# Edenzzzz/Stable-Diffusion-for-book-cover-generation

Measured on NVIDIA B200. Metric: unet_denoise_it_per_s, higher is better.
Workload: dtype bf16

## Files before the change

include/b200sd.h:

```cpp
#ifndef B200SD_H_
#define B200SD_H_

#include <stddef.h>
#include <stdint.h>

#ifdef __cplusplus
extern "C" {
#endif

#define B200SD_OK 0
#define B200SD_ERR_INVALID 1
#define B200SD_ERR_CUDA 2
#define B200SD_ERR_UNSUPPORTED 3

#define B200SD_F32 0
#define B200SD_BF16 1

typedef void* b200sd_stream_t;

const char* b200sd_last_error(void);
int b200sd_version(void);
int64_t b200sd_launch_count(void);

void b200sd_debug_set(int key, int value);
int b200sd_timer_reserve(int n);
int b200sd_timer_record(int i, b200sd_stream_t stream);
int b200sd_timer_elapsed_ms(int i, int j, float* ms);


int b200sd_cfg_ddim_step(const void* eps_u, const void* eps_c, const void* x, void* out, void* eps_out,
                         int64_t n, float guidance, float sa_t, float sb_t, float sa_p, float sb_p,
                         int eps_dtype, int x_dtype, b200sd_stream_t stream);

int b200sd_sampler_advance(const float* timesteps, int n_steps, int* cursor, float* in_t, int n_t, b200sd_stream_t stream);
int b200sd_cfg_ddim_step_table(const void* eps_u, const void* eps_c, const void* x, void* out, void* eps_out,
                               int64_t n, float guidance, const float* coef_table, const int* cursor,
                               int eps_dtype, int x_dtype, b200sd_stream_t stream);

int b200sd_cfg_plms_step_table(const float* eps_u, const float* eps_c, float* x, float* saved, float* ring, int64_t n,
                               float guidance, const float* table, const int* cursor, b200sd_stream_t stream);

int b200sd_cfg_plms_step(const void* eps_u, const void* eps_c, const void* x, void* out, void* eps_out,
                         const void* hist0, const void* hist1, const void* hist2, const void* hist3,
                         int nhist, const float* w_host5, int64_t n, float guidance, float cx, float ce,
                         int eps_dtype, int x_dtype, b200sd_stream_t stream);

int b200sd_add_noise(const void* x0, const void* noise, const int64_t* timesteps, const float* sa_table,
                     const float* sb_table, void* out, int batch, int64_t per_sample, int num_train_timesteps,
                     int dtype, b200sd_stream_t stream);

int b200sd_mse_workspace_floats(void);
int b200sd_mse_loss_fwd(const void* pred, const void* target, float* loss_out, float* workspace, int64_t n,
                        int pred_dtype, int target_dtype, b200sd_stream_t stream);
int b200sd_mse_loss_bwd(const void* pred, const void* target, const float* grad_loss, void* grad_pred, int64_t n,
                        int pred_dtype, int target_dtype, b200sd_stream_t stream);


int b200sd_timestep_embedding(const float* timesteps, float* out, int batch, int dim, b200sd_stream_t stream);

int b200sd_small_linear(const float* in, const void* w_bf16, const float* bias, float* out, int batch, int N, int K,
                        int silu_in, int silu_out, b200sd_stream_t stream);

#define B200SD_EPI_LINEAR 0
#define B200SD_EPI_GEGLU 1

typedef struct b200sd_gemm_args {
    const void* a0;
    const void* a1;
    const void* w;
    const float* bias;
    const float* rowbias;
    const void* residual;
    void* out;
    int M, N, K;
    int C0, C1;
    int lda0, lda1;
    int ldc, ldr;
    int ldrb;
    int conv_taps;
    int batch, H, W;
    int rows_per_image;
    int epilogue;
    int out_dtype;
    int residual_dtype;
    int block_n;
    int split_k;
    void* workspace;
    size_t workspace_bytes;
    int pair;
    float* gn_part;
} b200sd_gemm_args;

size_t b200sd_gemm_workspace_bytes(void);
int b200sd_geglu_tile(int N);
int b200sd_gemm(const b200sd_gemm_args* args, b200sd_stream_t stream);
int b200sd_gemm_gn_layout(const b200sd_gemm_args* args, int hw, int* parts_per_image, int* total_parts);

typedef struct b200sd_dgrad_args {
    const void* dy;
    const void* w;
    const void* residual;
    void* out;
    int M, Cout, Cin;
    int conv_taps;
    int batch, H, W;
    int ldy, ldc, ldr;
    int out_dtype, residual_dtype;
    int block_n;
    int pair;
} b200sd_dgrad_args;
int b200sd_gemm_dgrad(const b200sd_dgrad_args* args, b200sd_stream_t stream);

typedef struct b200sd_wgrad_args {
    const void* dy;
    const void* x;
    float* dw;
    int rows, Cout, Cin;
    int conv_taps;
    int batch, H, W;
    int ldy, ldx, lddw;
    int block_n, split_k;
} b200sd_wgrad_args;
int b200sd_gemm_wgrad(const b200sd_wgrad_args* args, b200sd_stream_t stream);

int b200sd_conv_in(const float* x_nchw, const float* w, const float* bias, void* out_nhwc, int batch, int Cin,
                   int Cout, int H, int W, int out_dtype, b200sd_stream_t stream);
int b200sd_conv_out(const void* x_nhwc, const float* w, const float* bias, float* out_nchw, int batch, int Cin,
                    int Cout, int H, int W, b200sd_stream_t stream);
int b200sd_nhwc_bias_to_nchw(const float* x, const float* bias, float* out_nchw, int batch, int C, int hw, int ld,
                             b200sd_stream_t stream);

int b200sd_groupnorm_silu(const void* x0, const void* x1, int C0, int C1, const float* gamma, const float* beta,
                          void* out, void* raw_out, float* stats_ws, int batch, int hw, int groups, float eps,
                          int silu, int in_dtype, b200sd_stream_t stream);

int b200sd_groupnorm_silu_stats(const void* x0, const void* x1, int C0, int C1, const float* gamma, const float* beta,
                                void* out, void* raw_out, float* stats_ws, float* stats_out, int batch, int hw, int groups,
                                float eps, int silu, int in_dtype, b200sd_stream_t stream);

int b200sd_groupnorm_silu_parts(const void* x0, const void* x1, int C0, int C1, const float* part0, int ppi0, int ld0,
                                const float* part1, int ppi1, int ld1, const float* gamma, const float* beta, void* out,
                                void* raw_out, float* stats_out, int batch, int hw, int groups, float eps, int silu,
                                int in_dtype, b200sd_stream_t stream);

int b200sd_groupnorm_workspace_floats(int batch);
int b200sd_layernorm(const void* x, const float* gamma, const float* beta, void* out, int rows, int C, float eps,
                     int in_dtype, b200sd_stream_t stream);

size_t b200sd_attention_workspace_bytes(int batch, int heads, int Skv, int d);
int b200sd_attention(const void* q, const void* k, const void* v, void* out, int batch, int heads, int Sq, int Skv,
                     int d, int ldq, int ldk, int ldv, int ldo, float scale, void* workspace, size_t workspace_bytes,
                     b200sd_stream_t stream);

int b200sd_attention_lse(const void* q, const void* k, const void* v, void* out, float* lse, int batch, int heads, int Sq,
                         int Skv, int d, int ldq, int ldk, int ldv, int ldo, float scale, void* workspace,
                         size_t workspace_bytes, b200sd_stream_t stream);

size_t b200sd_attention_bwd_workspace_bytes(int batch, int heads, int Sq);
int b200sd_attention_bwd(const void* q, const void* k, const void* v, const void* out, const void* dout,
                         const float* lse, void* dq, void* dk, void* dv, int batch, int heads, int Sq, int Skv, int d,
                         int ldq, int ldk, int ldv, int ldo, int lddo, int lddq, int lddk, int lddv, float scale,
                         void* workspace, size_t workspace_bytes, b200sd_stream_t stream);


int b200sd_clip_embed(const int64_t* ids, const float* tok, const float* pos, float* out, int batch, int S, int C, int vocab,
                      b200sd_stream_t stream);
int b200sd_clip_embed_bwd(const int64_t* ids, const float* dx, float* dtok, float* dpos, int batch, int S, int C, int vocab,
                          b200sd_stream_t stream);
int b200sd_quick_gelu_fwd(const void* u, void* out, int64_t n, b200sd_stream_t stream);
int b200sd_quick_gelu_bwd(const void* u, const void* dg, void* du, int64_t n, b200sd_stream_t stream);
int b200sd_layernorm_f32out(const float* x, const float* gamma, const float* beta, float* out, int rows, int C, float eps,
                            b200sd_stream_t stream);
int b200sd_causal_attention(const void* qkv, void* out, int batch, int heads, int S, int d, int ld, int ldo, int q_off,
                            int k_off, int v_off, float scale, b200sd_stream_t stream);
int b200sd_causal_attention_bwd(const void* qkv, const void* dout, void* dqkv, int batch, int heads, int S, int d, int ld,
                                int lddo, int ldd, int q_off, int k_off, int v_off, float scale, b200sd_stream_t stream);


int b200sd_im2col_s2_pad(const void* x, void* out, int batch, int H, int W, int C, int in_dtype, int pad,
                         b200sd_stream_t stream);
int b200sd_softmax_rows(const float* x, void* out_bf16, int rows, int L, int ldx, int ldo, float scale, b200sd_stream_t stream);
int b200sd_conv1x1_small(const float* x_nchw, const float* w, const float* bias, float* out_nchw, int batch, int Cin, int Cout,
                         int hw, b200sd_stream_t stream);
int b200sd_gaussian_sample(const float* moments, const float* noise, float* out, int batch, int C, int hw, float out_scale,
                           b200sd_stream_t stream);


int b200sd_grad_prep(const void* in, int in_dtype, void* out_bf16, float* colsum, int rows, int N, int ld,
                     int rows_per_image, int ldcs, b200sd_stream_t stream);

int b200sd_groupnorm_bwd_workspace_floats(int batch);
int b200sd_groupnorm_silu_bwd(const void* x0, const void* x1, int C0, int C1, int in_dtype, const float* gamma,
                              const float* beta, const void* dy, const float* add_src, void* out0, void* out1,
                              int out_dtype, int accumulate0, int accumulate1, float* dgamma, float* dbeta,
                              const float* mean_rstd, float* workspace, int batch, int hw, int groups, float eps, int silu,
                              b200sd_stream_t stream);

int b200sd_layernorm_bwd(const void* x, int in_dtype, const float* gamma, const void* dy, float* dres, float* dgamma,
                         float* dbeta, int rows, int C, float eps, b200sd_stream_t stream);

int b200sd_geglu_fwd(const void* u, void* out, int64_t rows, int C_half, b200sd_stream_t stream);
int b200sd_geglu_bwd(const void* u, const void* dff, void* du, int64_t rows, int C_half, b200sd_stream_t stream);

int b200sd_upsample2x_bwd(const void* dy, float* dx, int batch, int H, int W, int C, int accumulate, b200sd_stream_t stream);
int b200sd_col2im_s2(const void* dcol, float* dx, int batch, int H, int W, int C, int accumulate, b200sd_stream_t stream);

int b200sd_conv_out_bwd(const float* dout_nchw, const void* x_nhwc, const float* w, void* dx_nhwc, float* dw,
                        float* dbias, int batch, int Cin, int Cout, int H, int W, b200sd_stream_t stream);
int b200sd_conv_in_wgrad(const void* dy_nhwc, int dy_dtype, const float* x_nchw, float* dw, int batch, int Cin, int Cout,
                         int H, int W, b200sd_stream_t stream);

int b200sd_cast_act(const float* in, void* out_bf16, int64_t n, int silu, b200sd_stream_t stream);
int b200sd_silu_bwd_mul(const float* pre, float* grad, int64_t n, b200sd_stream_t stream);

int b200sd_split_hi_lo(const float* x, void* hi_bf16, void* lo_bf16, int64_t n, b200sd_stream_t stream);
int b200sd_groupnorm_silu_split(const void* x0, const void* x1, int C0, int C1, const float* gamma, const float* beta,
                                void* out, void* out_lo, void* raw_out, void* raw_lo, float* stats_ws, float* stats_out,
                                int batch, int hw, int groups, float eps, int silu, int in_dtype, b200sd_stream_t stream);
int b200sd_layernorm_split(const void* x, const float* gamma, const float* beta, void* out, void* out_lo, int rows, int C,
                           float eps, int in_dtype, b200sd_stream_t stream);
int b200sd_geglu_f32(const float* u, void* hi_bf16, void* lo_bf16, int64_t rows, int C_half, b200sd_stream_t stream);
int b200sd_attention_f32(const float* q, const float* k, const float* v, float* out, int batch, int heads, int Sq, int Skv,
                         int d, int ldq, int ldk, int ldv, int ldo, float scale, b200sd_stream_t stream);
int b200sd_small_linear_f32(const float* in, const float* w, const float* bias, float* out, int batch, int N, int K,
                            int silu_in, int silu_out, b200sd_stream_t stream);

int b200sd_cast_flat(const float* in, void* out_bf16, int64_t n, b200sd_stream_t stream);
int b200sd_adamw_step(float* param, float* grad, float* exp_avg, float* exp_avg_sq, void* weights_bf16, int64_t n,
                      float lr, float beta1, float beta2, float eps, float weight_decay, int step, float grad_scale,
                      int zero_grad, b200sd_stream_t stream);

int b200sd_adamw8bit_step(float* param, float* grad, uint8_t* state1, uint8_t* state2, float* absmax1, float* absmax2,
                          const float* qmap1, const float* qmap2, const int32_t* chunk_mode, float* small_exp_avg,
                          float* small_exp_avg_sq, void* weights_bf16, int64_t n, float lr, float beta1, float beta2, float eps,
                          float weight_decay, int step, float grad_scale, int zero_grad, b200sd_stream_t stream);

int b200sd_upsample2x(const void* x, void* out, int batch, int H, int W, int C, int in_dtype, b200sd_stream_t stream);
int b200sd_im2col_s2(const void* x, void* out, int batch, int H, int W, int C, int in_dtype, b200sd_stream_t stream);

#ifdef __cplusplus
}
#endif
#endif
```

stable-diffusion-for-book-cover-generation_b200/_lib.py:

```python
from __future__ import annotations

import ctypes as C
import os

_HERE = os.path.dirname(os.path.abspath(__file__))
LIB_PATH = os.path.join(_HERE, "libb200sd.so")

_lib = None


class B200SDError(RuntimeError):
    pass


class GemmArgs(C.Structure):
    _fields_ = [
        ("a0", C.c_void_p), ("a1", C.c_void_p), ("w", C.c_void_p), ("bias", C.c_void_p), ("rowbias", C.c_void_p),
        ("residual", C.c_void_p), ("out", C.c_void_p),
        ("M", C.c_int), ("N", C.c_int), ("K", C.c_int), ("C0", C.c_int), ("C1", C.c_int),
        ("lda0", C.c_int), ("lda1", C.c_int), ("ldc", C.c_int), ("ldr", C.c_int), ("ldrb", C.c_int), ("conv_taps", C.c_int),
        ("batch", C.c_int), ("H", C.c_int), ("W", C.c_int), ("rows_per_image", C.c_int), ("epilogue", C.c_int),
        ("out_dtype", C.c_int), ("residual_dtype", C.c_int), ("block_n", C.c_int), ("split_k", C.c_int),
        ("workspace", C.c_void_p), ("workspace_bytes", C.c_size_t), ("pair", C.c_int), ("gn_part", C.c_void_p),
    ]


class DgradArgs(C.Structure):
    _fields_ = [
        ("dy", C.c_void_p), ("w", C.c_void_p), ("residual", C.c_void_p), ("out", C.c_void_p),
        ("M", C.c_int), ("Cout", C.c_int), ("Cin", C.c_int), ("conv_taps", C.c_int),
        ("batch", C.c_int), ("H", C.c_int), ("W", C.c_int), ("ldy", C.c_int), ("ldc", C.c_int), ("ldr", C.c_int),
        ("out_dtype", C.c_int), ("residual_dtype", C.c_int), ("block_n", C.c_int), ("pair", C.c_int),
    ]


class WgradArgs(C.Structure):
    _fields_ = [
        ("dy", C.c_void_p), ("x", C.c_void_p), ("dw", C.c_void_p),
        ("rows", C.c_int), ("Cout", C.c_int), ("Cin", C.c_int), ("conv_taps", C.c_int),
        ("batch", C.c_int), ("H", C.c_int), ("W", C.c_int), ("ldy", C.c_int), ("ldx", C.c_int), ("lddw", C.c_int),
        ("block_n", C.c_int), ("split_k", C.c_int),
    ]


_vp, _i, _i64, _f, _sz = C.c_void_p, C.c_int, C.c_int64, C.c_float, C.c_size_t

SIGNATURES = {
    "b200sd_last_error": (C.c_char_p, []),
    "b200sd_version": (_i, []),
    "b200sd_launch_count": (_i64, []),
    "b200sd_debug_set": (None, [_i, _i]),
    "b200sd_timer_reserve": (_i, [_i]),
    "b200sd_timer_record": (_i, [_i, _vp]),
    "b200sd_timer_elapsed_ms": (_i, [_i, _i, C.POINTER(C.c_float)]),
    "b200sd_cfg_ddim_step": (_i, [_vp, _vp, _vp, _vp, _vp, _i64, _f, _f, _f, _f, _f, _i, _i, _vp]),
    "b200sd_clip_embed": (_i, [_vp, _vp, _vp, _vp, _i, _i, _i, _i, _vp]),
    "b200sd_clip_embed_bwd": (_i, [_vp, _vp, _vp, _vp, _i, _i, _i, _i, _vp]),
    "b200sd_quick_gelu_fwd": (_i, [_vp, _vp, _i64, _vp]),
    "b200sd_quick_gelu_bwd": (_i, [_vp, _vp, _vp, _i64, _vp]),
    "b200sd_layernorm_f32out": (_i, [_vp, _vp, _vp, _vp, _i, _i, _f, _vp]),
    "b200sd_causal_attention": (_i, [_vp, _vp, _i, _i, _i, _i, _i, _i, _i, _i, _i, _f, _vp]),
    "b200sd_causal_attention_bwd": (_i, [_vp, _vp, _vp, _i, _i, _i, _i, _i, _i, _i, _i, _i, _i, _f, _vp]),
    "b200sd_im2col_s2_pad": (_i, [_vp, _vp, _i, _i, _i, _i, _i, _i, _vp]),
    "b200sd_softmax_rows": (_i, [_vp, _vp, _i, _i, _i, _i, _f, _vp]),
    "b200sd_conv1x1_small": (_i, [_vp, _vp, _vp, _vp, _i, _i, _i, _i, _vp]),
    "b200sd_gaussian_sample": (_i, [_vp, _vp, _vp, _i, _i, _i, _f, _vp]),
    "b200sd_sampler_advance": (_i, [_vp, _i, _vp, _vp, _i, _vp]),
    "b200sd_cfg_plms_step_table": (_i, [_vp, _vp, _vp, _vp, _vp, _i64, _f, _vp, _vp, _vp]),
    "b200sd_cfg_ddim_step_table": (_i, [_vp, _vp, _vp, _vp, _vp, _i64, _f, _vp, _vp, _i, _i, _vp]),
    "b200sd_cfg_plms_step": (_i, [_vp, _vp, _vp, _vp, _vp, _vp, _vp, _vp, _vp, _i, C.POINTER(C.c_float), _i64, _f, _f,
                                  _f, _i, _i, _vp]),
    "b200sd_add_noise": (_i, [_vp, _vp, _vp, _vp, _vp, _vp, _i, _i64, _i, _i, _vp]),
    "b200sd_mse_workspace_floats": (_i, []),
    "b200sd_mse_loss_fwd": (_i, [_vp, _vp, _vp, _vp, _i64, _i, _i, _vp]),
    "b200sd_mse_loss_bwd": (_i, [_vp, _vp, _vp, _vp, _i64, _i, _i, _vp]),
    "b200sd_timestep_embedding": (_i, [_vp, _vp, _i, _i, _vp]),
    "b200sd_small_linear": (_i, [_vp, _vp, _vp, _vp, _i, _i, _i, _i, _i, _vp]),
    "b200sd_gemm_workspace_bytes": (_sz, []),
    "b200sd_geglu_tile": (_i, [_i]),
    "b200sd_gemm": (_i, [C.POINTER(GemmArgs), _vp]),
    "b200sd_gemm_gn_layout": (_i, [C.POINTER(GemmArgs), _i, C.POINTER(C.c_int), C.POINTER(C.c_int)]),
    "b200sd_groupnorm_silu_parts": (_i, [_vp, _vp, _i, _i, _vp, _i, _i, _vp, _i, _i, _vp, _vp, _vp, _vp, _vp, _i, _i, _i, _f, _i,
                                         _i, _vp]),
    "b200sd_gemm_dgrad": (_i, [C.POINTER(DgradArgs), _vp]),
    "b200sd_gemm_wgrad": (_i, [C.POINTER(WgradArgs), _vp]),
    "b200sd_conv_in": (_i, [_vp, _vp, _vp, _vp, _i, _i, _i, _i, _i, _i, _vp]),
    "b200sd_conv_out": (_i, [_vp, _vp, _vp, _vp, _i, _i, _i, _i, _i, _vp]),
    "b200sd_nhwc_bias_to_nchw": (_i, [_vp, _vp, _vp, _i, _i, _i, _i, _vp]),
    "b200sd_groupnorm_silu": (_i, [_vp, _vp, _i, _i, _vp, _vp, _vp, _vp, _vp, _i, _i, _i, _f, _i, _i, _vp]),
    "b200sd_groupnorm_silu_stats": (_i, [_vp, _vp, _i, _i, _vp, _vp, _vp, _vp, _vp, _vp, _i, _i, _i, _f, _i, _i, _vp]),
    "b200sd_groupnorm_workspace_floats": (_i, [_i]),
    "b200sd_layernorm": (_i, [_vp, _vp, _vp, _vp, _i, _i, _f, _i, _vp]),
    "b200sd_attention_workspace_bytes": (_sz, [_i, _i, _i, _i]),
    "b200sd_attention": (_i, [_vp, _vp, _vp, _vp, _i, _i, _i, _i, _i, _i, _i, _i, _i, _f, _vp, _sz, _vp]),
    "b200sd_attention_lse": (_i, [_vp, _vp, _vp, _vp, _vp, _i, _i, _i, _i, _i, _i, _i, _i, _i, _f, _vp, _sz, _vp]),
    "b200sd_attention_bwd_workspace_bytes": (_sz, [_i, _i, _i]),
    "b200sd_attention_bwd": (_i, [_vp] * 9 + [_i] * 13 + [_f, _vp, _sz, _vp]),
    "b200sd_grad_prep": (_i, [_vp, _i, _vp, _vp, _i, _i, _i, _i, _i, _vp]),
    "b200sd_groupnorm_bwd_workspace_floats": (_i, [_i]),
    "b200sd_groupnorm_silu_bwd": (_i, [_vp, _vp, _i, _i, _i, _vp, _vp, _vp, _vp, _vp, _vp, _i, _i, _i, _vp, _vp, _vp, _vp, _i,
                                       _i, _i, _f, _i, _vp]),
    "b200sd_layernorm_bwd": (_i, [_vp, _i, _vp, _vp, _vp, _vp, _vp, _i, _i, _f, _vp]),
    "b200sd_geglu_fwd": (_i, [_vp, _vp, _i64, _i, _vp]),
    "b200sd_geglu_bwd": (_i, [_vp, _vp, _vp, _i64, _i, _vp]),
    "b200sd_upsample2x_bwd": (_i, [_vp, _vp, _i, _i, _i, _i, _i, _vp]),
    "b200sd_col2im_s2": (_i, [_vp, _vp, _i, _i, _i, _i, _i, _vp]),
    "b200sd_conv_out_bwd": (_i, [_vp, _vp, _vp, _vp, _vp, _vp, _i, _i, _i, _i, _i, _vp]),
    "b200sd_conv_in_wgrad": (_i, [_vp, _i, _vp, _vp, _i, _i, _i, _i, _i, _vp]),
    "b200sd_cast_act": (_i, [_vp, _vp, _i64, _i, _vp]),
    "b200sd_silu_bwd_mul": (_i, [_vp, _vp, _i64, _vp]),
    "b200sd_split_hi_lo": (_i, [_vp, _vp, _vp, _i64, _vp]),
    "b200sd_groupnorm_silu_split": (_i, [_vp, _vp, _i, _i, _vp, _vp, _vp, _vp, _vp, _vp, _vp, _vp, _i, _i, _i, _f, _i, _i, _vp]),
    "b200sd_layernorm_split": (_i, [_vp, _vp, _vp, _vp, _vp, _i, _i, _f, _i, _vp]),
    "b200sd_geglu_f32": (_i, [_vp, _vp, _vp, _i64, _i, _vp]),
    "b200sd_attention_f32": (_i, [_vp, _vp, _vp, _vp, _i, _i, _i, _i, _i, _i, _i, _i, _i, _f, _vp]),
    "b200sd_small_linear_f32": (_i, [_vp, _vp, _vp, _vp, _i, _i, _i, _i, _i, _vp]),
    "b200sd_cast_flat": (_i, [_vp, _vp, _i64, _vp]),
    "b200sd_adamw_step": (_i, [_vp, _vp, _vp, _vp, _vp, _i64, _f, _f, _f, _f, _f, _i, _f, _i, _vp]),
    "b200sd_adamw8bit_step": (_i, [_vp] * 12 + [_i64, _f, _f, _f, _f, _f, _i, _f, _i, _vp]),
    "b200sd_upsample2x": (_i, [_vp, _vp, _i, _i, _i, _i, _i, _vp]),
    "b200sd_im2col_s2": (_i, [_vp, _vp, _i, _i, _i, _i, _i, _vp]),
}


def lib() -> C.CDLL:
    global _lib
    if _lib is None:
        if not os.path.exists(LIB_PATH):
            raise B200SDError(
                f"{LIB_PATH} is missing: build it with `python -c 'import __graft_entry__ as g; g.build()'` "
                "(b200sd has no CPU / eager fallback)")
        L = C.CDLL(LIB_PATH)
        for name, (res, args) in SIGNATURES.items():
            fn = getattr(L, name)
            fn.restype = res
            fn.argtypes = args
        _lib = L
    return _lib


def check(rc: int, what: str = "") -> None:
    if rc != 0:
        msg = lib().b200sd_last_error().decode("utf-8", "replace")
        raise B200SDError(f"{what or 'b200sd call'} failed (code {rc}): {msg}")
```

stable-diffusion-for-book-cover-generation_b200/csrc/api.cu:

```cuda
#include <atomic>
#include <cstdarg>
#include <cstdio>
#include <mutex>

#include "common.cuh"

static thread_local char g_err[512] = "";
std::atomic<long long> g_b200sd_launches{0};

void b200sd_set_error(const char* fmt, ...) {
    va_list ap;
    va_start(ap, fmt);
    vsnprintf(g_err, sizeof(g_err), fmt, ap);
    va_end(ap);
}

extern "C" const char* b200sd_last_error(void) { return g_err; }

#include <map>
#include <utility>
cudaError_t b200sd_opt_in_smem_impl(const void* kernel, int bytes, bool max_carveout) {
    static std::mutex mu;
    static std::map<std::pair<const void*, int>, int> configured;
    int dev = 0;
    cudaError_t e = cudaGetDevice(&dev);
    if (e != cudaSuccess) return e;
    std::lock_guard<std::mutex> lock(mu);
    auto key = std::make_pair(kernel, dev);
    auto it = configured.find(key);
    if (it != configured.end() && it->second >= bytes) return cudaSuccess;
    e = cudaFuncSetAttribute(kernel, cudaFuncAttributeMaxDynamicSharedMemorySize, bytes);
    if (e != cudaSuccess) return e;
    if (max_carveout) {
        e = cudaFuncSetAttribute(kernel, cudaFuncAttributePreferredSharedMemoryCarveout, 100);
        if (e != cudaSuccess) return e;
    }
    configured[key] = bytes;
    return cudaSuccess;
}
extern "C" int b200sd_version(void) { return 101; }
extern "C" int64_t b200sd_launch_count(void) { return g_b200sd_launches.load(); }

#include <vector>
static std::vector<cudaEvent_t> g_timers;
extern "C" int b200sd_timer_reserve(int n) {
    B200SD_REQUIRE(n >= 0 && n <= (1 << 20), "timer_reserve: bad count %d", n);
    while ((int)g_timers.size() < n) {
        cudaEvent_t e;
        B200SD_CUDA(cudaEventCreate(&e));
        g_timers.push_back(e);
    }
    return B200SD_OK;
}
extern "C" int b200sd_timer_record(int i, b200sd_stream_t stream) {
    B200SD_REQUIRE(i >= 0 && i < (int)g_timers.size(), "timer_record: index %d not reserved", i);
    cudaStream_t s = static_cast<cudaStream_t>(stream);
    cudaStreamCaptureStatus st = cudaStreamCaptureStatusNone;
    B200SD_CUDA(cudaStreamIsCapturing(s, &st));
    B200SD_CUDA(cudaEventRecordWithFlags(g_timers[i], s, st == cudaStreamCaptureStatusActive ? cudaEventRecordExternal : cudaEventRecordDefault));
    return B200SD_OK;
}
extern "C" int b200sd_timer_elapsed_ms(int i, int j, float* ms) {
    B200SD_REQUIRE(ms && i >= 0 && j >= 0 && i < (int)g_timers.size() && j < (int)g_timers.size(), "timer_elapsed: bad index");
    B200SD_CUDA(cudaEventElapsedTime(ms, g_timers[i], g_timers[j]));
    return B200SD_OK;
}

int b200sd_num_sms() {
    static int sms = 0;
    if (sms == 0) {
        int dev = 0;
        if (cudaGetDevice(&dev) != cudaSuccess) return 148;
        if (cudaDeviceGetAttribute(&sms, cudaDevAttrMultiProcessorCount, dev) != cudaSuccess || sms <= 0) sms = 148;
    }
    return sms;
}

typedef CUresult (*encode_tiled_fn)(CUtensorMap*, CUtensorMapDataType, cuuint32_t, void*, const cuuint64_t*,
                                    const cuuint64_t*, const cuuint32_t*, const cuuint32_t*, CUtensorMapInterleave,
                                    CUtensorMapSwizzle, CUtensorMapL2promotion, CUtensorMapFloatOOBfill);

static encode_tiled_fn get_encode_fn() {
    static encode_tiled_fn fn = nullptr;
    static std::once_flag once;
    std::call_once(once, [] {
        void* p = nullptr;
        cudaDriverEntryPointQueryResult q;
        if (cudaGetDriverEntryPoint("cuTensorMapEncodeTiled", &p, cudaEnableDefault, &q) == cudaSuccess &&
            q == cudaDriverEntryPointSuccess)
            fn = reinterpret_cast<encode_tiled_fn>(p);
    });
    return fn;
}

int b200sd_make_tmap(CUtensorMap* out, const void* base, int rank, const uint64_t* dims,
                     const uint64_t* strides_bytes, const uint32_t* box, CUtensorMapSwizzle swizzle,
                     CUtensorMapDataType dtype) {
    encode_tiled_fn fn = get_encode_fn();
    B200SD_REQUIRE(fn != nullptr, "cuTensorMapEncodeTiled driver entry point unavailable");
    cuuint64_t gdim[5];
    cuuint64_t gstr[5];
    cuuint32_t bdim[5];
    cuuint32_t estr[5];
    for (int i = 0; i < rank; ++i) {
        gdim[i] = dims[i];
        bdim[i] = box[i];
        estr[i] = 1;
        if (i > 0) gstr[i - 1] = strides_bytes[i];
    }
    CUresult r = fn(out, dtype, (cuuint32_t)rank, const_cast<void*>(base), gdim, gstr, bdim, estr,
                    CU_TENSOR_MAP_INTERLEAVE_NONE, swizzle, CU_TENSOR_MAP_L2_PROMOTION_L2_256B,
                    CU_TENSOR_MAP_FLOAT_OOB_FILL_NONE);
    B200SD_REQUIRE(r == CUDA_SUCCESS,
                   "cuTensorMapEncodeTiled failed (%d): rank %d dims [%llu %llu %llu %llu] box [%u %u %u %u] base %p",
                   (int)r, rank, (unsigned long long)dims[0], (unsigned long long)(rank > 1 ? dims[1] : 0),
                   (unsigned long long)(rank > 2 ? dims[2] : 0), (unsigned long long)(rank > 3 ? dims[3] : 0), box[0],
                   rank > 1 ? box[1] : 0, rank > 2 ? box[2] : 0, rank > 3 ? box[3] : 0, base);
    return B200SD_OK;
}
```

stable-diffusion-for-book-cover-generation_b200/csrc/common.cuh:

```cuda
#pragma once

#include <cuda.h>
#include <cuda_bf16.h>
#include <cuda_runtime.h>
#include <stdint.h>
#include <stdio.h>

#include "../../include/b200sd.h"

typedef __nv_bfloat16 bf16;

void b200sd_set_error(const char* fmt, ...);

#define B200SD_REQUIRE(cond, ...)                       \
    do {                                                \
        if (!(cond)) {                                  \
            b200sd_set_error(__VA_ARGS__);              \
            return B200SD_ERR_INVALID;                  \
        }                                               \
    } while (0)

#define B200SD_CUDA(call)                                                                   \
    do {                                                                                    \
        cudaError_t e__ = (call);                                                           \
        if (e__ != cudaSuccess) {                                                           \
            b200sd_set_error("%s:%d CUDA error %s", __FILE__, __LINE__, cudaGetErrorString(e__)); \
            return B200SD_ERR_CUDA;                                                         \
        }                                                                                   \
    } while (0)

#define B200SD_LAUNCH_CHECK() B200SD_CUDA(cudaGetLastError())

static inline int ceil_div(int a, int b) { return (a + b - 1) / b; }

int b200sd_num_sms();

int b200sd_make_tmap(CUtensorMap* out, const void* base, int rank, const uint64_t* dims,
                     const uint64_t* strides_bytes, const uint32_t* box, CUtensorMapSwizzle swizzle,
                     CUtensorMapDataType dtype = CU_TENSOR_MAP_DATA_TYPE_BFLOAT16);

#ifdef __CUDACC__
cudaError_t b200sd_opt_in_smem_impl(const void* kernel, int bytes, bool max_carveout);
template <typename K>
static inline cudaError_t b200sd_opt_in_smem(K kernel, int bytes, bool max_carveout = false) {
    return b200sd_opt_in_smem_impl(reinterpret_cast<const void*>(kernel), bytes, max_carveout);
}

namespace ptx {

__device__ __forceinline__ uint32_t smem_u32(const void* p) {
    return static_cast<uint32_t>(__cvta_generic_to_shared(p));
}

__device__ __forceinline__ bool elect_one() {
    uint32_t pred;
    asm volatile(
        "{\n\t.reg .pred p;\n\t"
        "elect.sync _|p, 0xffffffff;\n\t"
        "selp.u32 %0, 1, 0, p;\n\t}\n"
        : "=r"(pred));
    return pred != 0;
}

__device__ __forceinline__ void mbar_init(uint64_t* bar, uint32_t count) {
    asm volatile("mbarrier.init.shared::cta.b64 [%0], %1;" ::"r"(smem_u32(bar)), "r"(count));
}
__device__ __forceinline__ void fence_barrier_init() {
    asm volatile("fence.mbarrier_init.release.cluster;" ::: "memory");
}
__device__ __forceinline__ void fence_proxy_async() {
    asm volatile("fence.proxy.async.shared::cta;" ::: "memory");
}
__device__ __forceinline__ void fence_proxy_async_global() {
    asm volatile("fence.proxy.async.global;" ::: "memory");
}
__device__ __forceinline__ void mbar_expect_tx(uint64_t* bar, uint32_t bytes) {
    asm volatile("mbarrier.arrive.expect_tx.shared::cta.b64 _, [%0], %1;" ::"r"(smem_u32(bar)), "r"(bytes)
                 : "memory");
}
__device__ __forceinline__ void mbar_arrive(uint64_t* bar) {
    asm volatile("mbarrier.arrive.shared::cta.b64 _, [%0];" ::"r"(smem_u32(bar)) : "memory");
}
__device__ __forceinline__ bool mbar_try_wait(uint64_t* bar, uint32_t parity) {
    uint32_t ok;
    asm volatile(
        "{\n\t.reg .pred p;\n\t"
        "mbarrier.try_wait.parity.shared::cta.b64 p, [%1], %2;\n\t"
        "selp.u32 %0, 1, 0, p;\n\t}\n"
        : "=r"(ok)
        : "r"(smem_u32(bar)), "r"(parity)
        : "memory");
    return ok != 0;
}
__device__ __forceinline__ void mbar_wait(uint64_t* bar, uint32_t parity) {
    if (mbar_try_wait(bar, parity)) return;
    long long t0 = clock64();
    while (!mbar_try_wait(bar, parity)) {
        if (clock64() - t0 > 4000000000LL) {
            printf("b200sd: mbarrier wait timed out (block %d,%d thread %d)\n", blockIdx.x, blockIdx.y,
                   threadIdx.x);
            __trap();
        }
    }
}

__device__ __forceinline__ void prefetch_tmap(const CUtensorMap* m) {
    asm volatile("prefetch.tensormap [%0];" ::"l"(reinterpret_cast<uint64_t>(m)) : "memory");
}
__device__ __forceinline__ void tma_load_2d(void* dst, const CUtensorMap* m, uint64_t* bar, int c0, int c1) {
    asm volatile(
        "cp.async.bulk.tensor.2d.shared::cluster.global.mbarrier::complete_tx::bytes [%0], [%1, {%3, %4}], [%2];"
        ::"r"(smem_u32(dst)), "l"(reinterpret_cast<uint64_t>(m)), "r"(smem_u32(bar)), "r"(c0), "r"(c1)
        : "memory");
}
__device__ __forceinline__ void tma_load_3d(void* dst, const CUtensorMap* m, uint64_t* bar, int c0, int c1, int c2) {
    asm volatile(
        "cp.async.bulk.tensor.3d.shared::cluster.global.mbarrier::complete_tx::bytes [%0], [%1, {%3, %4, %5}], [%2];"
        ::"r"(smem_u32(dst)), "l"(reinterpret_cast<uint64_t>(m)), "r"(smem_u32(bar)), "r"(c0), "r"(c1), "r"(c2)
        : "memory");
}
__device__ __forceinline__ void tma_load_4d(void* dst, const CUtensorMap* m, uint64_t* bar, int c0, int c1, int c2,
                                            int c3) {
    asm volatile(
        "cp.async.bulk.tensor.4d.shared::cluster.global.mbarrier::complete_tx::bytes [%0], [%1, {%3, %4, %5, %6}], "
        "[%2];" ::"r"(smem_u32(dst)),
        "l"(reinterpret_cast<uint64_t>(m)), "r"(smem_u32(bar)), "r"(c0), "r"(c1), "r"(c2), "r"(c3)
        : "memory");
}

__device__ __forceinline__ void tma_store_2d(const CUtensorMap* m, const void* src, int c0, int c1) {
    asm volatile("cp.async.bulk.tensor.2d.global.shared::cta.bulk_group [%0, {%2, %3}], [%1];" ::"l"(reinterpret_cast<uint64_t>(m)),
                 "r"(smem_u32(src)), "r"(c0), "r"(c1)
                 : "memory");
}
__device__ __forceinline__ void tma_store_commit() { asm volatile("cp.async.bulk.commit_group;" ::: "memory"); }
template <int N>
__device__ __forceinline__ void tma_store_wait_read() { asm volatile("cp.async.bulk.wait_group.read %0;" ::"n"(N) : "memory"); }
template <int N>
__device__ __forceinline__ void tma_store_wait() { asm volatile("cp.async.bulk.wait_group %0;" ::"n"(N) : "memory"); }

__device__ __forceinline__ uint32_t mapa_u32(uint32_t local_smem_addr, uint32_t cta_rank) {
    uint32_t r;
    asm volatile("mapa.shared::cluster.u32 %0, %1, %2;" : "=r"(r) : "r"(local_smem_addr), "r"(cta_rank));
    return r;
}
__device__ __forceinline__ void tma_load_2d_cg2(void* dst, const CUtensorMap* m, uint32_t bar_cluster_addr, int c0, int c1) {
    asm volatile(
        "cp.async.bulk.tensor.2d.cta_group::2.shared::cluster.global.mbarrier::complete_tx::bytes [%0], [%1, {%3, %4}], [%2];"
        ::"r"(smem_u32(dst)), "l"(reinterpret_cast<uint64_t>(m)), "r"(bar_cluster_addr), "r"(c0), "r"(c1)
        : "memory");
}
__device__ __forceinline__ void tma_load_3d_cg2(void* dst, const CUtensorMap* m, uint32_t bar_cluster_addr, int c0, int c1, int c2) {
    asm volatile(
        "cp.async.bulk.tensor.3d.cta_group::2.shared::cluster.global.mbarrier::complete_tx::bytes [%0], [%1, {%3, %4, %5}], [%2];"
        ::"r"(smem_u32(dst)), "l"(reinterpret_cast<uint64_t>(m)), "r"(bar_cluster_addr), "r"(c0), "r"(c1), "r"(c2)
        : "memory");
}
__device__ __forceinline__ void tma_load_4d_cg2(void* dst, const CUtensorMap* m, uint32_t bar_cluster_addr, int c0, int c1, int c2,
                                                int c3) {
    asm volatile(
        "cp.async.bulk.tensor.4d.cta_group::2.shared::cluster.global.mbarrier::complete_tx::bytes [%0], [%1, {%3, %4, %5, %6}], "
        "[%2];" ::"r"(smem_u32(dst)),
        "l"(reinterpret_cast<uint64_t>(m)), "r"(bar_cluster_addr), "r"(c0), "r"(c1), "r"(c2), "r"(c3)
        : "memory");
}
__device__ __forceinline__ void tmem_alloc_cg2(uint32_t* dst_smem, uint32_t ncols) {
    asm volatile("tcgen05.alloc.cta_group::2.sync.aligned.shared::cta.b32 [%0], %1;" ::"r"(smem_u32(dst_smem)), "r"(ncols) : "memory");
}
__device__ __forceinline__ void tmem_relinquish_cg2() {
    asm volatile("tcgen05.relinquish_alloc_permit.cta_group::2.sync.aligned;" ::: "memory");
}
__device__ __forceinline__ void tmem_dealloc_cg2(uint32_t taddr, uint32_t ncols) {
    asm volatile("tcgen05.dealloc.cta_group::2.sync.aligned.b32 %0, %1;" ::"r"(taddr), "r"(ncols) : "memory");
}
__device__ __forceinline__ void umma_bf16_ss_cg2(uint32_t tmem_d, uint64_t desc_a, uint64_t desc_b, uint32_t idesc,
                                                 uint32_t accumulate) {
    asm volatile(
        "{\n\t.reg .pred p;\n\t"
        "setp.ne.b32 p, %4, 0;\n\t"
        "tcgen05.mma.cta_group::2.kind::f16 [%0], %1, %2, %3, p;\n\t}\n" ::"r"(tmem_d),
        "l"(desc_a), "l"(desc_b), "r"(idesc), "r"(accumulate)
        : "memory");
}
__device__ __forceinline__ void umma_commit_cg2(uint64_t* bar, uint16_t cta_mask) {
    asm volatile("tcgen05.commit.cta_group::2.mbarrier::arrive::one.shared::cluster.multicast::cluster.b64 [%0], %1;" ::"r"(smem_u32(bar)),
                 "h"(cta_mask)
                 : "memory");
}
// ... 156 lines not shown
```

stable-diffusion-for-book-cover-generation_b200/csrc/gemm_tcgen05.cu:

```cuda
#include <atomic>
#include <cstring>
#include <mutex>
#include <cstdio>

#include "common.cuh"

extern std::atomic<long long> g_b200sd_launches;

static int g_persist = -1;
extern "C" void b200sd_debug_set(int key, int value) { if (key == 0) g_persist = value; }

namespace {

constexpr int BLOCK_M = 128;
constexpr size_t kWsPartialBytes = (size_t)160 * 128 * 256 * sizeof(float);
constexpr size_t kWsCounterBytes = 4096;
constexpr int BLOCK_K = 64;
constexpr int UMMA_K = 16;
constexpr int kNumThreads = 192;
constexpr int kMaxStages = 8;
constexpr int kABytes = BLOCK_M * BLOCK_K * 2;


struct KParams {
    CUtensorMap tmA0, tmA1, tmB;
    const float* bias;
    const float* rowbias;
    const void* residual;
    void* out;
    int M, N;
    int num_k_blocks;
    int kb_per_split;
    int split_k;
    int block_n;
    int stages;
    int conv;
    int cblocks0;
    int cblocks;
    int tile_w, tile_h, tile_n;
    int tiles_y;
    int tiles_x;
    int rows_valid;
    int a_bytes;
    int ldc, ldr, ldrb;
    int rows_per_image;
    int epilogue;
    int out_f32;
    int res_f32;
    uint32_t tmem_cols;
    int a_mn;
    int b_mode;
    int conv_sign;
    int n_valid;
    int tiles_per_tap;
    int atomic_out;
    int pair;
    int persist;
    int psplit;
    float* gn_part;
};

__device__ __forceinline__ void cluster_sync_all() {
    asm volatile("barrier.cluster.arrive.release.aligned;\n\tbarrier.cluster.wait.acquire.aligned;" ::: "memory");
}
__device__ __forceinline__ uint32_t cluster_ctarank() {
    uint32_t r;
    asm volatile("mov.u32 %0, %%cluster_ctarank;" : "=r"(r));
    return r;
}
__device__ __forceinline__ float4 ld_dsmem_v4(uint32_t local_smem_addr, uint32_t cta_rank) {
    uint32_t raddr;
    asm volatile("mapa.shared::cluster.u32 %0, %1, %2;" : "=r"(raddr) : "r"(local_smem_addr), "r"(cta_rank));
    float4 v;
    asm volatile("ld.shared::cluster.v4.f32 {%0, %1, %2, %3}, [%4];" : "=f"(v.x), "=f"(v.y), "=f"(v.z), "=f"(v.w) : "r"(raddr) : "memory");
    return v;
}

__device__ __forceinline__ void red_add_v4(float* dst, float a, float b, float c, float d) {
    asm volatile("red.global.add.v4.f32 [%0], {%1, %2, %3, %4};" ::"l"(dst), "f"(a), "f"(b), "f"(c), "f"(d) : "memory");
}

struct EpiCtx {
    uint32_t stage_u32;
    int pitch_f, row_end, R, cb, half, m0, col_out, img0, n0cb;
    const float* s_rb;
    bool multi_img, rb_smem;
};
__device__ __forceinline__ void lds8(uint32_t addr, float (&v)[8]) {
    asm volatile("ld.shared.v4.f32 {%0, %1, %2, %3}, [%4];" : "=f"(v[0]), "=f"(v[1]), "=f"(v[2]), "=f"(v[3]) : "r"(addr));
    asm volatile("ld.shared.v4.f32 {%0, %1, %2, %3}, [%4];" : "=f"(v[4]), "=f"(v[5]), "=f"(v[6]), "=f"(v[7]) : "r"(addr + 16));
}
template <int OUT, int RES, bool SPLIT, bool GEGLU, bool STATS = false>
__device__ __forceinline__ void epilogue_rows(const KParams& p, const EpiCtx& e, int row0, const float (&b)[8], const float (&bg)[8],
                                              float* cs = nullptr, float* cq = nullptr) {
    constexpr int U = 4;
    for (int row = row0; row < e.row_end; row += e.R * U) {
        float v[U][8], r[U][8];
#pragma unroll
        for (int u = 0; u < U; ++u) {
            const int rl = min(row + u * e.R, e.row_end - 1);
            const uint32_t addr = e.stage_u32 + (uint32_t)(rl * e.pitch_f + e.cb) * 4u;
            if constexpr (SPLIT) {
#pragma unroll
                for (int i = 0; i < 8; ++i) v[u][i] = 0.f;
                for (int sp = 0; sp < p.split_k; ++sp) {
                    const float4 a0 = ld_dsmem_v4(addr, sp), a1 = ld_dsmem_v4(addr + 16, sp);
                    v[u][0] += a0.x; v[u][1] += a0.y; v[u][2] += a0.z; v[u][3] += a0.w;
                    v[u][4] += a1.x; v[u][5] += a1.y; v[u][6] += a1.z; v[u][7] += a1.w;
                }
            } else {
                lds8(addr, v[u]);
            }
            if constexpr (GEGLU) lds8(addr + (uint32_t)e.half * 4u, r[u]);
            else if constexpr (RES == 2) ld8<B200SD_F32>(p.residual, (size_t)(e.m0 + rl) * p.ldr + e.col_out, r[u]);
            else if constexpr (RES == 1) ld8<B200SD_BF16>(p.residual, (size_t)(e.m0 + rl) * p.ldr + e.col_out, r[u]);
        }
#pragma unroll
        for (int u = 0; u < U; ++u) {
            const int rl = row + u * e.R;
            if (rl >= e.row_end) break;
            const int grow = e.m0 + rl;
            float o[8];
            if constexpr (GEGLU) {
#pragma unroll
                for (int i = 0; i < 8; ++i) o[i] = (v[u][i] + b[i]) * gelu_erf_f(r[u][i] + bg[i]);
                st8<B200SD_BF16>(p.out, (size_t)grow * p.ldc + e.col_out, o);
            } else {
#pragma unroll
                for (int i = 0; i < 8; ++i) o[i] = v[u][i] + b[i];
                if constexpr (RES != 0) {
#pragma unroll
                    for (int i = 0; i < 8; ++i) o[i] += r[u][i];
                }
                if (e.multi_img) {
                    const int img = grow / p.rows_per_image;
                    if (e.rb_smem) {
                        const float* rb = e.s_rb + (img == e.img0 ? 0 : 256) + e.cb;
#pragma unroll
                        for (int i = 0; i < 8; ++i) o[i] += rb[i];
                    } else {
                        float t[8];
                        ld8<B200SD_F32>(p.rowbias, (size_t)img * p.ldrb + e.n0cb, t);
#pragma unroll
                        for (int i = 0; i < 8; ++i) o[i] += t[i];
                    }
                }
                if constexpr (STATS) {
#pragma unroll
                    for (int i = 0; i < 8; ++i) { cs[i] += o[i]; cq[i] = fmaf(o[i], o[i], cq[i]); }
                }
                if constexpr (OUT == 2) {
                    float* dst = static_cast<float*>(p.out) + (size_t)grow * p.ldc + e.col_out;
                    red_add_v4(dst, o[0], o[1], o[2], o[3]);
                    red_add_v4(dst + 4, o[4], o[5], o[6], o[7]);
                } else if constexpr (OUT == 1) st8<B200SD_F32>(p.out, (size_t)grow * p.ldc + e.col_out, o);
                else st8<B200SD_BF16>(p.out, (size_t)grow * p.ldc + e.col_out, o);
            }
        }
    }
}

template <bool PAIR, int OP>
__global__ void __launch_bounds__(kNumThreads, 1) gemm_tcgen05_kernel(const __grid_constant__ KParams p) {
    constexpr bool a_mn = OP >= 2;
    constexpr int b_mode = OP;
    extern __shared__ uint8_t smem_raw[];
    uint8_t* smem = reinterpret_cast<uint8_t*>((reinterpret_cast<uintptr_t>(smem_raw) + 1023) & ~uintptr_t(1023));
    constexpr bool pair = PAIR;
    const uint32_t crank = pair ? cluster_ctarank() : 0;
    const int b_bytes = (p.block_n * BLOCK_K * 2) >> (pair ? 1 : 0);
    uint8_t* smem_a = smem;
    uint8_t* smem_b = smem + (size_t)p.stages * kABytes;
    uint64_t* bars = reinterpret_cast<uint64_t*>(smem_b + (size_t)p.stages * b_bytes);
    uint64_t* full_bar = bars;
    uint64_t* empty_bar = bars + kMaxStages;
    uint64_t* tmem_full_bar = bars + 2 * kMaxStages;
    uint32_t* tmem_slot = reinterpret_cast<uint32_t*>(bars + 2 * kMaxStages + 1);

    const int warp = threadIdx.x >> 5;
    const int lane = threadIdx.x & 31;
    const int m_tile = blockIdx.x;
    const int n_tile = blockIdx.y;
    const int split = blockIdx.z;
    const int kb_begin = split * p.kb_per_split;
    const int kb_end = min(kb_begin + p.kb_per_split, p.num_k_blocks);
    const int w_tap = b_mode == 3 ? n_tile / p.tiles_per_tap : 0;
    const int n0 = (b_mode == 3 ? n_tile - w_tap * p.tiles_per_tap : n_tile) * p.block_n;
    const int col_base = w_tap * p.n_valid + n0;
    const int col_valid = min(p.block_n, p.n_valid - n0);
    const int m0 = m_tile * p.rows_valid;

    if (warp == 0 && lane == 0) {
        ptx::prefetch_tmap(&p.tmA0);
        ptx::prefetch_tmap(&p.tmB);
        if (p.cblocks0 != p.cblocks) ptx::prefetch_tmap(&p.tmA1);
        for (int s = 0; s < p.stages; ++s) {
            ptx::mbar_init(&full_bar[s], 1);
            ptx::mbar_init(&empty_bar[s], 1);
        }
        ptx::mbar_init(tmem_full_bar, 1);
        ptx::fence_barrier_init();
    }
    if (warp == 1) {
        if constexpr (pair) { ptx::tmem_alloc_cg2(tmem_slot, p.tmem_cols); ptx::tmem_relinquish_cg2(); }
        else { ptx::tmem_alloc(tmem_slot, p.tmem_cols); ptx::tmem_relinquish(); }
    }
    ptx::tc_fence_before();
    __syncthreads();
    if constexpr (pair) cluster_sync_all();
    ptx::tc_fence_after();
    const uint32_t tmem_base = *tmem_slot;

    const int epi_tid = threadIdx.x - 64;
    const int pitch_f = p.block_n + 4;
    float* stage = reinterpret_cast<float*>(smem);
    float* s_bias = reinterpret_cast<float*>(bars + 32);
    float* s_rb = s_bias + 256;
    int img0 = 0, img1 = 0;
    bool rb_smem = false;
    if (p.rowbias && m0 < p.M) {
        img0 = m0 / p.rows_per_image;
        img1 = (min(m0 + p.rows_valid, p.M) - 1) / p.rows_per_image;
        rb_smem = (img1 - img0) <= 1;
    }

    if (warp == 0) {
        if (ptx::elect_one()) {
            int stage = 0;
            uint32_t phase = 0;
            int img = 0, y0 = 0, x0 = 0;
            if (p.conv) {
                if (p.tile_n > 1) { img = m_tile * p.tile_n; y0 = 0; }
                else {
                    int mt = m_tile;
                    if (p.tiles_x > 1) { x0 = (mt % p.tiles_x) * p.tile_w; mt /= p.tiles_x; }
                    img = mt / p.tiles_y; y0 = (mt % p.tiles_y) * p.tile_h;
                }
            }
            const int nbox_live = (b_mode != 0 && !pair) ? (col_valid + 63) >> 6 : (p.block_n >> 6);
            const int nboxb = nbox_live >> (pair ? 1 : 0);
            const int nb0 = n0 + (pair ? (int)crank * (p.block_n >> 1) : 0);
            const uint32_t stage_tx = (b_mode != 0 && !pair) ? (uint32_t)(p.a_bytes + nbox_live * 8192)
                                                             : ((uint32_t)(p.a_bytes + b_bytes) << (pair ? 1 : 0));
            for (int kb = kb_begin; kb < kb_end; ++kb) {
                ptx::mbar_wait(&empty_bar[stage], phase ^ 1);
                if (!pair || crank == 0) ptx::mbar_expect_tx(&full_bar[stage], stage_tx);
                uint8_t* dst_a = smem_a + (size_t)stage * kABytes;
                uint8_t* dst_b = smem_b + (size_t)stage * b_bytes;
                uint64_t* fb = &full_bar[stage];
                const uint32_t fbc = pair ? ptx::mapa_u32(ptx::smem_u32(fb), 0) : 0;
#define LD2(dst, tm, c0, c1) do { if constexpr (pair) ptx::tma_load_2d_cg2(dst, tm, fbc, c0, c1); else ptx::tma_load_2d(dst, tm, fb, c0, c1); } while (0)
#define LD3(dst, tm, c0, c1, c2) do { if constexpr (pair) ptx::tma_load_3d_cg2(dst, tm, fbc, c0, c1, c2); else ptx::tma_load_3d(dst, tm, fb, c0, c1, c2); } while (0)
#define LD4(dst, tm, c0, c1, c2, c3) do { if constexpr (pair) ptx::tma_load_4d_cg2(dst, tm, fbc, c0, c1, c2, c3); else ptx::tma_load_4d(dst, tm, fb, c0, c1, c2, c3); } while (0)
                if (a_mn) {
                    LD2(dst_a, &p.tmA0, m0, kb * BLOCK_K);
                    LD2(dst_a + kABytes / 2, &p.tmA0, m0 + 64, kb * BLOCK_K);
                } else if (!p.conv) {
                    if (kb < p.cblocks0) LD2(dst_a, &p.tmA0, kb * BLOCK_K, m0);
                    else LD2(dst_a, &p.tmA1, (kb - p.cblocks0) * BLOCK_K, m0);
                } else {
                    const int tap = kb / p.cblocks;
                    const int cb = kb - tap * p.cblocks;
                    const int dy = (tap / 3 - 1) * p.conv_sign, dx = (tap % 3 - 1) * p.conv_sign;
                    if (cb < p.cblocks0) LD4(dst_a, &p.tmA0, cb * BLOCK_K, x0 + dx, y0 + dy, img);
                    else LD4(dst_a, &p.tmA1, (cb - p.cblocks0) * BLOCK_K, x0 + dx, y0 + dy, img);
                }
                if (b_mode == 0) {
                    LD2(dst_b, &p.tmB, kb * BLOCK_K, nb0);
                } else if (b_mode == 1) {
                    if (!p.conv) {
                        for (int j = 0; j < nboxb; ++j) LD2(dst_b + j * 8192, &p.tmB, nb0 + j * 64, kb * BLOCK_K);
                    } else {
                        const int tap = kb / p.cblocks;
                        const int cb = kb - tap * p.cblocks;
                        for (int j = 0; j < nboxb; ++j) LD3(dst_b + j * 8192, &p.tmB, nb0 + j * 64, tap, cb * BLOCK_K);
                    }
                } else if (b_mode == 2) {
                    for (int j = 0; j < nboxb; ++j) LD2(dst_b + j * 8192, &p.tmB, nb0 + j * 64, kb * BLOCK_K);
                } else {
                    int bimg, by0;
                    if (p.tile_n > 1) { bimg = kb * p.tile_n; by0 = 0; }
                    else { bimg = kb / p.tiles_y; by0 = (kb - bimg * p.tiles_y) * p.tile_h; }
                    const int dy = w_tap / 3 - 1, dx = w_tap % 3 - 1;
                    for (int j = 0; j < nboxb; ++j) LD4(dst_b + j * 8192, &p.tmB, nb0 + j * 64, dx, by0 + dy, bimg);
                }
#undef LD2
#undef LD3
#undef LD4
                if (++stage == p.stages) { stage = 0; phase ^= 1; }
            }
        }
    } else if (warp == 1) {
        if ((!pair || crank == 0) && ptx::elect_one()) {
            const uint32_t b_mn = b_mode != 0;
            const uint32_t mma_n = (b_mode != 0 && !pair) ? (uint32_t)(((col_valid + 63) >> 6) << 6) : (uint32_t)p.block_n;
            const uint32_t idesc = ptx::umma_idesc_bf16(pair ? 2 * BLOCK_M : BLOCK_M, mma_n) | ((uint32_t)a_mn << 15) | (b_mn << 16);
            const uint32_t a_step = a_mn ? (2048 >> 4) : 2, b_step = b_mn ? (2048 >> 4) : 2;
            int stage = 0;
            uint32_t phase = 0;
            for (int kb = kb_begin; kb < kb_end; ++kb) {
                ptx::mbar_wait(&full_bar[stage], phase);
                ptx::tc_fence_after();
                const uint32_t sa = ptx::smem_u32(smem_a + (size_t)stage * kABytes), sb = ptx::smem_u32(smem_b + (size_t)stage * b_bytes);
                const uint64_t da = a_mn ? ptx::umma_desc_mn_sw128(sa, 8192) : ptx::umma_desc_k_sw128(sa);
                const uint64_t db = b_mn ? ptx::umma_desc_mn_sw128(sb, 8192) : ptx::umma_desc_k_sw128(sb);
#pragma unroll
                for (int k = 0; k < BLOCK_K / UMMA_K; ++k) {
                    const uint32_t accum = (kb > kb_begin || k > 0) ? 1u : 0u;
                    if constexpr (pair) ptx::umma_bf16_ss_cg2(tmem_base, da + a_step * k, db + b_step * k, idesc, accum);
                    else ptx::umma_bf16_ss(tmem_base, da + a_step * k, db + b_step * k, idesc, accum);
                }
                if constexpr (pair) ptx::umma_commit_cg2(&empty_bar[stage], 3); else ptx::umma_commit(&empty_bar[stage]);
                if (++stage == p.stages) { stage = 0; phase ^= 1; }
            }
            if constexpr (pair) ptx::umma_commit_cg2(tmem_full_bar, 3); else ptx::umma_commit(tmem_full_bar);
        }
    } else {
        const int q = warp & 3;
        const int r_in_tile = q * 32 + lane;
        const uint32_t taddr = tmem_base + ((uint32_t)(q * 32) << 16);
        for (int c = epi_tid; c < p.block_n; c += 128) {
            s_bias[c] = (p.bias && c < col_valid) ? __ldg(p.bias + n0 + c) : 0.f;
            if (rb_smem) {
                s_rb[c] = __ldg(p.rowbias + (size_t)img0 * p.ldrb + n0 + c);
                s_rb[256 + c] = __ldg(p.rowbias + (size_t)img1 * p.ldrb + n0 + c);
            }
        }
        ptx::mbar_wait(tmem_full_bar, 0);
        ptx::tc_fence_after();
        {
            float4* my_row = reinterpret_cast<float4*>(stage + (size_t)r_in_tile * pitch_f);
            for (int c = 0; c < p.block_n; c += 32) {
                uint32_t r0[16], r1[16];
                const bool two = (c + 16 < p.block_n);
                ptx::tmem_ld_32x32b_x16(taddr + c, r0);
                if (two) ptx::tmem_ld_32x32b_x16(taddr + c + 16, r1);
                ptx::tmem_ld_wait();
#pragma unroll
                for (int i = 0; i < 4; ++i)
                    my_row[c / 4 + i] = make_float4(__uint_as_float(r0[4 * i]), __uint_as_float(r0[4 * i + 1]),
                                                    __uint_as_float(r0[4 * i + 2]), __uint_as_float(r0[4 * i + 3]));
                if (two) {
#pragma unroll
                    for (int i = 0; i < 4; ++i)
                        my_row[c / 4 + 4 + i] = make_float4(__uint_as_float(r1[4 * i]), __uint_as_float(r1[4 * i + 1]),
                                                            __uint_as_float(r1[4 * i + 2]), __uint_as_float(r1[4 * i + 3]));
                }
            }
        }
        ptx::tc_fence_before();
        ptx::named_bar_sync(1, 128);
    }

    if (p.split_k > 1) cluster_sync_all(); else __syncthreads();

    {
        const int rank = p.split_k > 1 ? (int)cluster_ctarank() : 0;
        const int rows_per_cta = BLOCK_M / p.split_k;
        const int row_begin = rank * rows_per_cta;
        int valid = min(p.rows_valid, p.M - m0) - row_begin;
        valid = max(0, min(valid, rows_per_cta));
        const bool geglu = p.epilogue == B200SD_EPI_GEGLU;
        const int half = p.block_n / 2;
        const int groups = (geglu ? half : p.block_n) / 8;
        const int R = kNumThreads / groups;
        const int tid = threadIdx.x;
        float cs[8], cq[8];
#pragma unroll
        for (int i = 0; i < 8; ++i) { cs[i] = 0.f; cq[i] = 0.f; }
        if (tid < R * groups && valid > 0) {
            const int c8 = tid % groups, r0 = tid / groups;
            const int cb = c8 * 8;
            if (geglu || cb < col_valid) {
                float b[8], bg[8];
#pragma unroll
                for (int i = 0; i < 8; ++i) { b[i] = s_bias[cb + i]; bg[i] = geglu ? s_bias[half + cb + i] : 0.f; }
                const bool multi_img = p.rowbias != nullptr && img1 != img0;
                if (p.rowbias != nullptr && !multi_img) {
#pragma unroll
                    for (int i = 0; i < 8; ++i) b[i] += s_rb[cb + i];
                }
                EpiCtx e;
                e.stage_u32 = ptx::smem_u32(stage);
                e.pitch_f = pitch_f; e.row_end = row_begin + valid; e.R = R; e.cb = cb; e.half = half; e.m0 = m0;
                e.col_out = geglu ? n_tile * half + cb : col_base + cb;
                e.s_rb = s_rb; e.img0 = img0; e.multi_img = multi_img; e.rb_smem = rb_smem; e.n0cb = n0 + cb;
                const int row0 = row_begin + r0;
                const int ok = p.atomic_out ? 2 : (p.out_f32 ? 1 : 0);
                const int rk = p.residual ? (p.res_f32 ? 2 : 1) : 0;
                if (geglu) epilogue_rows<0, 0, false, true>(p, e, row0, b, bg);
                else if (p.split_k > 1) {
                    if (ok == 1 && p.gn_part) { if (rk == 2) epilogue_rows<1, 2, true, false, true>(p, e, row0, b, bg, cs, cq); else epilogue_rows<1, 0, true, false, true>(p, e, row0, b, bg, cs, cq); }
                    else if (ok == 1) { if (rk == 2) epilogue_rows<1, 2, true, false>(p, e, row0, b, bg); else if (rk == 1) epilogue_rows<1, 1, true, false>(p, e, row0, b, bg); else epilogue_rows<1, 0, true, false>(p, e, row0, b, bg); }
                    else { if (rk == 2) epilogue_rows<0, 2, true, false>(p, e, row0, b, bg); else if (rk == 1) epilogue_rows<0, 1, true, false>(p, e, row0, b, bg); else epilogue_rows<0, 0, true, false>(p, e, row0, b, bg); }
                } else if (ok == 2) epilogue_rows<2, 0, false, false>(p, e, row0, b, bg);
                else if (ok == 1 && p.gn_part) { if (rk == 2) epilogue_rows<1, 2, false, false, true>(p, e, row0, b, bg, cs, cq); else epilogue_rows<1, 0, false, false, true>(p, e, row0, b, bg, cs, cq); }
                else if (ok == 1) { if (rk == 2) epilogue_rows<1, 2, false, false>(p, e, row0, b, bg); else if (rk == 1) epilogue_rows<1, 1, false, false>(p, e, row0, b, bg); else epilogue_rows<1, 0, false, false>(p, e, row0, b, bg); }
                else { if (rk == 2) epilogue_rows<0, 2, false, false>(p, e, row0, b, bg); else if (rk == 1) epilogue_rows<0, 1, false, false>(p, e, row0, b, bg); else epilogue_rows<0, 0, false, false>(p, e, row0, b, bg); }
            }
        }
        if (p.gn_part != nullptr) {
            if (p.split_k > 1) cluster_sync_all(); else __syncthreads();
            float* s_gn = reinterpret_cast<float*>(stage);
#pragma unroll
            for (int i = 0; i < 8; ++i) { s_gn[tid * 16 + i] = cs[i]; s_gn[tid * 16 + 8 + i] = cq[i]; }
            __syncthreads();
            float* dst = p.gn_part + (size_t)(m_tile * p.split_k + rank) * 2 * p.N;
            for (int idx = tid; idx < groups * 16; idx += kNumThreads) {
                const int c8 = idx >> 4, k = idx & 15, col = c8 * 8 + (k & 7);
                float a = 0.f;
                for (int r = 0; r < R; ++r) a += s_gn[(r * groups + c8) * 16 + k];
                if (col < col_valid) dst[(size_t)(k >> 3) * p.N + n0 + col] = a;
            }
        }
    }
    if (p.split_k > 1 && p.gn_part == nullptr) cluster_sync_all();

    ptx::tc_fence_before();
    __syncthreads();
    if constexpr (pair) cluster_sync_all();
    if (warp == 1) {
        ptx::tc_fence_after();
        if constexpr (pair) ptx::tmem_dealloc_cg2(tmem_base, p.tmem_cols); else ptx::tmem_dealloc(tmem_base, p.tmem_cols);
    }
}

constexpr int kEpiWarps = 8;
constexpr int kPersistThreads = 64 + 32 * kEpiWarps + 32;
constexpr int kMaxDepth = 3;

struct PParams {
    CUtensorMap tmA0, tmA1, tmB, tmOut, tmRes;
    const float* bias;
    const float* rowbias;
    float* gn_part;
    int M, N;
    int num_k_blocks, block_n, stages;
    int conv, cblocks0, cblocks, tile_h, tile_n, tiles_y;
    int tile_w, tiles_x;
    int n_tiles, num_tiles;
    int ldrb, rows_per_image;
    int geglu, out_f32, res_kind;
    int depth;
    int chunk_bytes;
    uint32_t tmem_cols, acc_stride;
    uint32_t off_b, off_epi, off_bias, off_stat, off_bars;
    int split, kb_per_split;
    CUtensorMap tmWs;
    float* ws;
    int* cnt;
    const void* residual;
    void* out;
    int ldc, ldr;
};

template <bool OUT_F32, int RES, bool GEGLU, bool STATS>
__device__ __forceinline__ void persist_chunk(const PParams& p, uint32_t taddr, int ch, const float* sbv, const float* sbg, uint8_t* cb,
                                              int lane, bool last_chunk, uint64_t* tempty_bar, uint64_t* rfull_bar, uint32_t rparity,
                                              float* gn_dst, int nrows) {
    uint32_t r0[16], r1[16], g0[16], g1[16];
    ptx::tmem_ld_32x32b_x16(taddr + ch * 32, r0);
    ptx::tmem_ld_32x32b_x16(taddr + ch * 32 + 16, r1);
    const int half = p.block_n >> 1;
    if constexpr (GEGLU) {
        ptx::tmem_ld_32x32b_x16(taddr + half + ch * 32, g0);
        ptx::tmem_ld_32x32b_x16(taddr + half + ch * 32 + 16, g1);
    }
    if constexpr (RES != 0) ptx::mbar_wait(rfull_bar, rparity);
    ptx::tmem_ld_wait();
    if (last_chunk) {
        ptx::tc_fence_before();
        __syncwarp();
        if (lane == 0) ptx::mbar_arrive(tempty_bar);
    }
    float v[32];
    const float4* sb4 = reinterpret_cast<const float4*>(sbv);
#pragma unroll
    for (int j = 0; j < 8; ++j) {
        const float4 b = sb4[j];
        const uint32_t* r = j < 4 ? r0 : r1;
        const int o = (j & 3) * 4;
        v[4 * j + 0] = __uint_as_float(r[o + 0]) + b.x;
        v[4 * j + 1] = __uint_as_float(r[o + 1]) + b.y;
        v[4 * j + 2] = __uint_as_float(r[o + 2]) + b.z;
        v[4 * j + 3] = __uint_as_float(r[o + 3]) + b.w;
    }
    if constexpr (GEGLU) {
        const float4* sg4 = reinterpret_cast<const float4*>(sbg);
#pragma unroll
        for (int j = 0; j < 8; ++j) {
            const float4 b = sg4[j];
            const uint32_t* r = j < 4 ? g0 : g1;
            const int o = (j & 3) * 4;
            v[4 * j + 0] *= gelu_erf_fast(__uint_as_float(r[o + 0]) + b.x);
            v[4 * j + 1] *= gelu_erf_fast(__uint_as_float(r[o + 1]) + b.y);
            v[4 * j + 2] *= gelu_erf_fast(__uint_as_float(r[o + 2]) + b.z);
            v[4 * j + 3] *= gelu_erf_fast(__uint_as_float(r[o + 3]) + b.w);
        }
    }
    uint8_t* row128 = cb + lane * 128;
    uint8_t* row64 = cb + lane * 64;
    const int x128 = lane & 7, x64 = (lane >> 1) & 3;
    if constexpr (RES == 2) {
#pragma unroll
        for (int j = 0; j < 8; ++j) {
            const float4 t = *reinterpret_cast<const float4*>(row128 + ((j ^ x128) << 4));
            v[4 * j + 0] += t.x; v[4 * j + 1] += t.y; v[4 * j + 2] += t.z; v[4 * j + 3] += t.w;
        }
    } else if constexpr (RES == 1) {
#pragma unroll
        for (int j = 0; j < 4; ++j) {
            const uint4 u = *reinterpret_cast<const uint4*>(row64 + ((j ^ x64) << 4));
            float2 f;
            f = unpack_bf16x2(u.x); v[8 * j + 0] += f.x; v[8 * j + 1] += f.y;
            f = unpack_bf16x2(u.y); v[8 * j + 2] += f.x; v[8 * j + 3] += f.y;
            f = unpack_bf16x2(u.z); v[8 * j + 4] += f.x; v[8 * j + 5] += f.y;
            f = unpack_bf16x2(u.w); v[8 * j + 6] += f.x; v[8 * j + 7] += f.y;
        }
    }
    if constexpr (RES != 0 && ((RES == 2) != OUT_F32)) __syncwarp();
    if constexpr (OUT_F32) {
#pragma unroll
        for (int j = 0; j < 8; ++j)
            *reinterpret_cast<float4*>(row128 + ((j ^ x128) << 4)) = make_float4(v[4 * j], v[4 * j + 1], v[4 * j + 2], v[4 * j + 3]);
    } else {
#pragma unroll
        for (int j = 0; j < 4; ++j) {
            uint4 u;
            u.x = pack_bf16x2(v[8 * j + 0], v[8 * j + 1]);
            u.y = pack_bf16x2(v[8 * j + 2], v[8 * j + 3]);
            u.z = pack_bf16x2(v[8 * j + 4], v[8 * j + 5]);
            u.w = pack_bf16x2(v[8 * j + 6], v[8 * j + 7]);
            *reinterpret_cast<uint4*>(row64 + ((j ^ x64) << 4)) = u;
        }
    }
    if constexpr (STATS) {
        __syncwarp();
        float s = 0.f, ss = 0.f;
        const uint8_t* colp = cb + ((lane & 3) << 2);
        const int piece = lane >> 2;
        for (int r = 0; r < nrows; ++r) {
            const float x = *reinterpret_cast<const float*>(colp + r * 128 + ((piece ^ (r & 7)) << 4));
            s += x;
            ss = fmaf(x, x, ss);
        }
        gn_dst[ch * 32 + lane] = s;
        gn_dst[256 + ch * 32 + lane] = ss;
    }
}

template <bool OUT_F32, int RES, bool GEGLU, bool STATS>
__device__ __forceinline__ void persist_epilogue(const PParams& p, uint8_t* smem, uint32_t tmem_base, int warp, int lane) {
    const int ew = warp - 2;
    const int q = warp & 3;
    const int h = ew >> 2;
    const int D = p.depth;
    const int kChunkBytes = p.chunk_bytes;
    uint8_t* my = smem + p.off_epi + (size_t)ew * D * kChunkBytes;
    float* sb = reinterpret_cast<float*>(smem + p.off_bias) + ew * 256;
    uint64_t* bars = reinterpret_cast<uint64_t*>(smem + p.off_bars);
    uint64_t* tfull = bars + 16;
    uint64_t* tempty = bars + 18;
    uint64_t* rfull = bars + 20 + ew * kMaxDepth;
    const int half = p.block_n >> 1;
    const int nch = (GEGLU ? half : p.block_n) >> 5;
    const int nl = nch > h ? (nch - h + 1) >> 1 : 0;
    const int my_tiles = ((int)blockIdx.x < p.num_tiles) ? (p.num_tiles - 1 - (int)blockIdx.x) / (int)gridDim.x + 1 : 0;
    const int total = my_tiles * nl;
    const int out_n = GEGLU ? half : p.block_n;

    auto issue_res = [&](int g) {
        const int itl = g / nl, ch = h + 2 * (g - itl * nl);
        const int tile = (int)blockIdx.x + itl * (int)gridDim.x;
        const int m_tile = tile / p.n_tiles, n_tile = tile - m_tile * p.n_tiles;
        const int buf = g % D;
        ptx::mbar_expect_tx(&rfull[buf], RES == 2 ? 4096u : 2048u);
        ptx::tma_load_2d(my + buf * kChunkBytes, &p.tmRes, &rfull[buf], n_tile * p.block_n + ch * 32, m_tile * BLOCK_M + q * 32);
    };
    if constexpr (RES != 0) {
        if (lane == 0)
            for (int g = 0; g < D && g < total; ++g) issue_res(g);
    }

    int g = 0;
    for (int it = 0; it < my_tiles; ++it) {
        const int tile = (int)blockIdx.x + it * (int)gridDim.x;
        const int m_tile = tile / p.n_tiles, n_tile = tile - m_tile * p.n_tiles;
        const int n0 = n_tile * p.block_n;
        const int row0 = m_tile * BLOCK_M + q * 32;
        __syncwarp();
        {
            const int img = p.rowbias ? min(row0, p.M - 1) / p.rows_per_image : 0;
            for (int l = 0; l < nl; ++l) {
                const int c = (h + 2 * l) * 32 + lane;
                float b = p.bias ? __ldg(p.bias + n0 + c) : 0.f;
                if (p.rowbias) b += __ldg(p.rowbias + (size_t)img * p.ldrb + n0 + c);
                sb[l * 32 + lane] = b;
                if constexpr (GEGLU) sb[128 + l * 32 + lane] = p.bias ? __ldg(p.bias + n0 + half + c) : 0.f;
            }
        }
        __syncwarp();
        const int acc = it & 1;
        ptx::mbar_wait(&tfull[acc], (uint32_t)(it >> 1) & 1u);
        ptx::tc_fence_after();
        const uint32_t taddr = tmem_base + (uint32_t)acc * p.acc_stride + ((uint32_t)(q * 32) << 16);
        const int nrows = max(0, min(32, p.M - row0));
        float* sstat = reinterpret_cast<float*>(smem + p.off_stat);
        float* gn_dst = STATS ? sstat + q * 512 : nullptr;
        if (nl == 0) {
            ptx::tc_fence_before();
            __syncwarp();
            if (lane == 0) ptx::mbar_arrive(&tempty[acc]);
        }
        for (int l = 0; l < nl; ++l, ++g) {
            const int ch = h + 2 * l;
            const int buf = g % D;
            uint8_t* cb = my + buf * kChunkBytes;
            if constexpr (RES == 0) {
                if (lane == 0) ptx::tma_store_wait_read<1>();
                __syncwarp();
            }
            persist_chunk<OUT_F32, RES, GEGLU, STATS>(p, taddr, ch, sb + l * 32, sb + 128 + l * 32, cb, lane, l == nl - 1, &tempty[acc],
                                                     &rfull[buf], (uint32_t)(g / D) & 1u, gn_dst, nrows);
            ptx::fence_proxy_async();
            __syncwarp();
            if (lane == 0) {
                ptx::tma_store_2d(&p.tmOut, cb, n_tile * out_n + ch * 32, row0);
                ptx::tma_store_commit();
                if constexpr (RES != 0) {
                    if (g >= 1 && g - 1 + D < total) {
                        ptx::tma_store_wait_read<1>();
                        issue_res(g - 1 + D);
                    }
                }
            }
        }
        if constexpr (STATS) {
            ptx::named_bar_sync(1, kEpiWarps * 32);
            const int te = ew * 32 + lane;
            if (te < p.block_n) {
                float s0 = 0.f, s1 = 0.f;
#pragma unroll
                for (int qq = 0; qq < 4; ++qq) { s0 += sstat[qq * 512 + te]; s1 += sstat[qq * 512 + 256 + te]; }
                float* dst = p.gn_part + (size_t)m_tile * 2 * p.N + n0 + te;
                dst[0] = s0;
                dst[p.N] = s1;
            }
            ptx::named_bar_sync(1, kEpiWarps * 32);
        }
    }
    if (lane == 0) ptx::tma_store_wait<0>();
    __syncwarp();
}

template <bool OUT_F32, int RES, bool STATS>
__device__ __forceinline__ void persist_epilogue_split(const PParams& p, uint8_t* smem, uint32_t tmem_base, int warp, int lane) {
    const int ew = warp - 2, q = warp & 3, h = ew >> 2;
    const int kChunkBytes = 4096;
    uint8_t* my = smem + p.off_epi + (size_t)ew * 2 * kChunkBytes;
    uint64_t* bars = reinterpret_cast<uint64_t*>(smem + p.off_bars);
    uint64_t* tfull = bars + 16;
    uint64_t* tempty = bars + 18;
    const int unit = blockIdx.x, tile = unit / p.split, s = unit - tile * p.split;
    const int m_tile = tile / p.n_tiles, n_tile = tile - m_tile * p.n_tiles;
    const int n0 = n_tile * p.block_n, m0 = m_tile * BLOCK_M;
    const int nch = p.block_n >> 5;
    const int nl = nch > h ? (nch - h + 1) >> 1 : 0;
    ptx::mbar_wait(&tfull[0], 0);
    ptx::tc_fence_after();
    const uint32_t taddr = tmem_base + ((uint32_t)(q * 32) << 16);
    for (int l = 0; l < nl; ++l) {
        const int ch = h + 2 * l;
        uint8_t* cb = my + (l & 1) * kChunkBytes;
        if (lane == 0) ptx::tma_store_wait_read<1>();
        __syncwarp();
        uint32_t r0[16], r1[16];
        ptx::tmem_ld_32x32b_x16(taddr + ch * 32, r0);
        ptx::tmem_ld_32x32b_x16(taddr + ch * 32 + 16, r1);
        ptx::tmem_ld_wait();
        uint8_t* row128 = cb + lane * 128;
        const int x128 = lane & 7;
#pragma unroll
        for (int j = 0; j < 8; ++j) {
            const uint32_t* r = j < 4 ? r0 : r1;
            const int o = (j & 3) * 4;
            *reinterpret_cast<uint4*>(row128 + ((j ^ x128) << 4)) = make_uint4(r[o], r[o + 1], r[o + 2], r[o + 3]);
        }
        ptx::fence_proxy_async();
        __syncwarp();
        if (lane == 0) {
            ptx::tma_store_2d(&p.tmWs, cb, ch * 32, unit * BLOCK_M + q * 32);
            ptx::tma_store_commit();
        }
    }
    ptx::tc_fence_before();
    __syncwarp();
    if (lane == 0) {
        ptx::mbar_arrive(&tempty[0]);
        ptx::tma_store_wait<0>();
        ptx::fence_proxy_async_global();
        __threadfence();
    }
    ptx::named_bar_sync(1, kEpiWarps * 32);
    const int te = ew * 32 + lane;
    int* cnt_in = p.cnt + tile;
    int* cnt_out = p.cnt + p.num_tiles + tile;
    if (te == 0) {
        atomicAdd(cnt_in, 1);
        int seen;
        long long t0 = clock64();
        do {
            asm volatile("ld.acquire.gpu.global.s32 %0, [%1];" : "=r"(seen) : "l"(cnt_in) : "memory");
            if (clock64() - t0 > 4000000000LL) { printf("b200sd: split-K arrival wait timed out (unit %d)\n", unit); __trap(); }
        } while (seen < p.split);
        __threadfence();
    }
    ptx::named_bar_sync(1, kEpiWarps * 32);
    const int rpc = BLOCK_M / p.split;
    const int groups = p.block_n >> 2;
    const int rslots = (kEpiWarps * 32) / groups < 4 ? (kEpiWarps * 32) / groups : 4;
    const int c4 = te % groups, rslot = te / groups;
    float* sstat = reinterpret_cast<float*>(smem + p.off_stat);
    float cs[4] = {0.f, 0.f, 0.f, 0.f}, cq[4] = {0.f, 0.f, 0.f, 0.f};
    if (rslot < rslots) {
        const int col = n0 + c4 * 4;
        float4 b4 = p.bias ? __ldg(reinterpret_cast<const float4*>(p.bias + col)) : make_float4(0.f, 0.f, 0.f, 0.f);
        for (int r = rslot; r < rpc; r += rslots) {
            const int trow = s * rpc + r;
            const int grow = m0 + trow;
            if (grow >= p.M) break;
            float4 v = make_float4(0.f, 0.f, 0.f, 0.f);
            const float* src = p.ws + ((size_t)(tile * p.split) * BLOCK_M + trow) * p.block_n + c4 * 4;
            for (int j = 0; j < p.split; ++j) {
                const float4 t = __ldcg(reinterpret_cast<const float4*>(src + (size_t)j * BLOCK_M * p.block_n));
                v.x += t.x; v.y += t.y; v.z += t.z; v.w += t.w;
            }
            v.x += b4.x; v.y += b4.y; v.z += b4.z; v.w += b4.w;
            if (p.rowbias) {
                const float4 t = __ldg(reinterpret_cast<const float4*>(p.rowbias + (size_t)(grow / p.rows_per_image) * p.ldrb + col));
                v.x += t.x; v.y += t.y; v.z += t.z; v.w += t.w;
            }
            if constexpr (RES == 2) {
                const float4 t = __ldcg(reinterpret_cast<const float4*>(static_cast<const float*>(p.residual) + (size_t)grow * p.ldr + col));
                v.x += t.x; v.y += t.y; v.z += t.z; v.w += t.w;
            } else if constexpr (RES == 1) {
                const uint2 u = __ldcg(reinterpret_cast<const uint2*>(static_cast<const bf16*>(p.residual) + (size_t)grow * p.ldr + col));
                const float2 f0 = unpack_bf16x2(u.x), f1 = unpack_bf16x2(u.y);
                v.x += f0.x; v.y += f0.y; v.z += f1.x; v.w += f1.y;
            }
            if constexpr (STATS) {
                cs[0] += v.x; cs[1] += v.y; cs[2] += v.z; cs[3] += v.w;
                cq[0] = fmaf(v.x, v.x, cq[0]); cq[1] = fmaf(v.y, v.y, cq[1]); cq[2] = fmaf(v.z, v.z, cq[2]); cq[3] = fmaf(v.w, v.w, cq[3]);
            }
            if constexpr (OUT_F32) {
                *reinterpret_cast<float4*>(static_cast<float*>(p.out) + (size_t)grow * p.ldc + col) = v;
            } else {
                uint2 u;
                u.x = pack_bf16x2(v.x, v.y);
                u.y = pack_bf16x2(v.z, v.w);
                *reinterpret_cast<uint2*>(static_cast<bf16*>(p.out) + (size_t)grow * p.ldc + col) = u;
            }
        }
    }
    if constexpr (STATS) {
        if (rslot < 4) {
#pragma unroll
            for (int i = 0; i < 4; ++i) { sstat[rslot * 512 + c4 * 4 + i] = cs[i]; sstat[rslot * 512 + 256 + c4 * 4 + i] = cq[i]; }
        }
        ptx::named_bar_sync(1, kEpiWarps * 32);
        if (te < p.block_n) {
            float s0 = 0.f, s1 = 0.f;
            for (int rs = 0; rs < rslots; ++rs) { s0 += sstat[rs * 512 + te]; s1 += sstat[rs * 512 + 256 + te]; }
            float* dst = p.gn_part + (size_t)(m_tile * p.split + s) * 2 * p.N + n0 + te;
            dst[0] = s0;
            dst[p.N] = s1;
        }
    }
    ptx::named_bar_sync(1, kEpiWarps * 32);
    if (te == 0) {
        __threadfence();
        if (atomicAdd(cnt_out, 1) == p.split - 1) {
            *cnt_out = 0;
            *cnt_in = 0;
            __threadfence();
        }
    }
}

__global__ void __launch_bounds__(kPersistThreads, 1) gemm_persist_kernel(const __grid_constant__ PParams p) {
    extern __shared__ uint8_t smem_raw[];
    uint8_t* smem = reinterpret_cast<uint8_t*>((reinterpret_cast<uintptr_t>(smem_raw) + 1023) & ~uintptr_t(1023));
    uint8_t* smem_a = smem;
    uint8_t* smem_b = smem + p.off_b;
    uint64_t* bars = reinterpret_cast<uint64_t*>(smem + p.off_bars);
    uint64_t* full_bar = bars;
    uint64_t* empty_bar = bars + 8;
    uint64_t* tfull = bars + 16;
    uint64_t* tempty = bars + 18;
    uint64_t* rfull = bars + 20;
    uint32_t* tmem_slot = reinterpret_cast<uint32_t*>(bars + 20 + kEpiWarps * kMaxDepth);
    const int warp = threadIdx.x >> 5;
    const int lane = threadIdx.x & 31;
    const int b_bytes = p.block_n * BLOCK_K * 2;

    const bool splitk = p.split > 1;
    const int sk_tile = splitk ? (int)blockIdx.x / p.split : 0, sk_s = splitk ? (int)blockIdx.x - sk_tile * p.split : 0;
    const int sk_kb0 = splitk ? (sk_s * p.num_k_blocks) / p.split : 0;
    const int sk_kb1 = splitk ? ((sk_s + 1) * p.num_k_blocks) / p.split : p.num_k_blocks;
    int pr_stage = 0, pr_tile = splitk ? sk_tile : (int)blockIdx.x, pr_kb = sk_kb0, pr_m0 = 0, pr_n0 = 0, pr_img = 0, pr_y0 = 0, pr_x0 = 0, pr_tap = 0,
        pr_cb = 0;
    bool pr_new = true;
    uint32_t pr_phase = 0;
    auto produce = [&](int limit, const int what) {
        const bool load_a = what & 1, load_b = what & 2;
        while (limit > 0 && pr_tile < p.num_tiles) {
            if (pr_new) {
                pr_new = false;
                const int m_tile = pr_tile / p.n_tiles, n_tile = pr_tile - m_tile * p.n_tiles;
                pr_m0 = m_tile * BLOCK_M;
                pr_n0 = n_tile * p.block_n;
                if (p.conv) {
                    if (p.tile_n > 1) { pr_img = m_tile * p.tile_n; pr_y0 = 0; }
                    else {
                        int mt = m_tile;
                        if (p.tiles_x > 1) { pr_x0 = (mt % p.tiles_x) * p.tile_w; mt /= p.tiles_x; }
                        pr_img = mt / p.tiles_y; pr_y0 = (mt - pr_img * p.tiles_y) * p.tile_h;
                    }
                }
                pr_tap = pr_kb / p.cblocks;
                pr_cb = pr_kb - pr_tap * p.cblocks;
            }
            uint64_t* fb = &full_bar[pr_stage];
            if (what) ptx::mbar_wait(&empty_bar[pr_stage], pr_phase ^ 1);
            if (load_a) {
                ptx::mbar_expect_tx(fb, (uint32_t)kABytes);

                uint8_t* dst_a = smem_a + (size_t)pr_stage * kABytes;
                if (!p.conv) {
                    if (pr_kb < p.cblocks0) ptx::tma_load_2d(dst_a, &p.tmA0, fb, pr_kb * BLOCK_K, pr_m0);
                    else ptx::tma_load_2d(dst_a, &p.tmA1, fb, (pr_kb - p.cblocks0) * BLOCK_K, pr_m0);
                } else {
                    const int dy = pr_tap / 3 - 1, dx = pr_tap - (pr_tap / 3) * 3 - 1;
                    if (pr_cb < p.cblocks0) ptx::tma_load_4d(dst_a, &p.tmA0, fb, pr_cb * BLOCK_K, pr_x0 + dx, pr_y0 + dy, pr_img);
                    else ptx::tma_load_4d(dst_a, &p.tmA1, fb, (pr_cb - p.cblocks0) * BLOCK_K, pr_x0 + dx, pr_y0 + dy, pr_img);
                }
            }
            if (load_b) {
                ptx::mbar_expect_tx(fb, (uint32_t)b_bytes);
                ptx::tma_load_2d(smem_b + (size_t)pr_stage * b_bytes, &p.tmB, fb, pr_kb * BLOCK_K, pr_n0);
            }
            if (++pr_stage == p.stages) { pr_stage = 0; pr_phase ^= 1; }
            if (++pr_cb == p.cblocks) { pr_cb = 0; ++pr_tap; }
            if (++pr_kb == sk_kb1) { pr_kb = 0; pr_new = true; pr_tile = splitk ? p.num_tiles : pr_tile + (int)gridDim.x; }
            --limit;
        }
    };
    const bool is_prod_a = threadIdx.x == 0, is_prod_b = threadIdx.x == kPersistThreads - 32;

    if (warp == 0 && lane == 0) {
        ptx::prefetch_tmap(&p.tmA0);
        ptx::prefetch_tmap(&p.tmB);
        ptx::prefetch_tmap(&p.tmOut);
        if (p.cblocks0 != p.cblocks) ptx::prefetch_tmap(&p.tmA1);
        if (p.res_kind) ptx::prefetch_tmap(&p.tmRes);
        for (int s = 0; s < p.stages; ++s) {
            ptx::mbar_init(&full_bar[s], 2);
            ptx::mbar_init(&empty_bar[s], 1);
        }
        for (int s = 0; s < 2; ++s) {
            ptx::mbar_init(&tfull[s], 1);
            ptx::mbar_init(&tempty[s], kEpiWarps);
        }
        for (int s = 0; s < kEpiWarps * kMaxDepth; ++s) ptx::mbar_init(&rfull[s], 1);
        ptx::fence_barrier_init();
        produce(p.stages, 3);
    }
    if (warp == 1) {
        ptx::tmem_alloc(tmem_slot, p.tmem_cols);
        ptx::tmem_relinquish();
    }
    ptx::tc_fence_before();
    __syncthreads();
    ptx::tc_fence_after();
    const uint32_t tmem_base = *tmem_slot;

    if (warp == 0) {
        if (is_prod_a) produce(0x7fffffff, 1);
    } else if (warp == kPersistThreads / 32 - 1) {
        if (is_prod_b) {
            produce(p.stages, 0);
            produce(0x7fffffff, 2);
        }
    } else if (warp == 1) {
        if (ptx::elect_one()) {
            const uint32_t idesc = ptx::umma_idesc_bf16(BLOCK_M, (uint32_t)p.block_n);
            int stage = 0;
            uint32_t phase = 0;
            int it = 0;
            const int nkb = sk_kb1 - sk_kb0;
            for (int tile = splitk ? sk_tile : (int)blockIdx.x; tile < p.num_tiles; tile = splitk ? p.num_tiles : tile + (int)gridDim.x, ++it) {
                const int acc = it & 1;
                ptx::mbar_wait(&tempty[acc], ((uint32_t)(it >> 1) & 1u) ^ 1u);
                ptx::tc_fence_after();
                const uint32_t d_tmem = tmem_base + (uint32_t)acc * p.acc_stride;
                for (int kb = 0; kb < nkb; ++kb) {
                    ptx::mbar_wait(&full_bar[stage], phase);
                    ptx::tc_fence_after();
                    const uint64_t da = ptx::umma_desc_k_sw128(ptx::smem_u32(smem_a + (size_t)stage * kABytes));
                    const uint64_t db = ptx::umma_desc_k_sw128(ptx::smem_u32(smem_b + (size_t)stage * b_bytes));
#pragma unroll
                    for (int k = 0; k < BLOCK_K / UMMA_K; ++k)
                        ptx::umma_bf16_ss(d_tmem, da + 2 * k, db + 2 * k, idesc, (kb > 0 || k > 0) ? 1u : 0u);
                    ptx::umma_commit(&empty_bar[stage]);
                    if (++stage == p.stages) { stage = 0; phase ^= 1; }
                }
                ptx::umma_commit(&tfull[acc]);
            }
        }
    } else {
        const int variant = (p.geglu ? 100 : 0) + (p.out_f32 ? 10 : 0) + p.res_kind + (p.gn_part ? 1000 : 0);
        if (splitk) {
            switch (variant) {
                case 0: persist_epilogue_split<false, 0, false>(p, smem, tmem_base, warp, lane); break;
                case 1: persist_epilogue_split<false, 1, false>(p, smem, tmem_base, warp, lane); break;
                case 2: persist_epilogue_split<false, 2, false>(p, smem, tmem_base, warp, lane); break;
                case 10: persist_epilogue_split<true, 0, false>(p, smem, tmem_base, warp, lane); break;
                case 11: persist_epilogue_split<true, 1, false>(p, smem, tmem_base, warp, lane); break;
                case 12: persist_epilogue_split<true, 2, false>(p, smem, tmem_base, warp, lane); break;
                case 1010: persist_epilogue_split<true, 0, true>(p, smem, tmem_base, warp, lane); break;
                case 1012: persist_epilogue_split<true, 2, true>(p, smem, tmem_base, warp, lane); break;
                default: break;
            }
        } else
        switch (variant) {
            case 100: persist_epilogue<false, 0, true, false>(p, smem, tmem_base, warp, lane); break;
            case 0: persist_epilogue<false, 0, false, false>(p, smem, tmem_base, warp, lane); break;
            case 1: persist_epilogue<false, 1, false, false>(p, smem, tmem_base, warp, lane); break;
            case 2: persist_epilogue<false, 2, false, false>(p, smem, tmem_base, warp, lane); break;
            case 10: persist_epilogue<true, 0, false, false>(p, smem, tmem_base, warp, lane); break;
// ... 28 lines not shown
        for (int bn = 256; bn >= step; bn -= step)
            if (N % bn == 0) { best = bn; break; }
        return best;
    }
    if (epilogue == B200SD_EPI_LINEAR && !can_split && (long)m_tiles * (N / best) * 2 <= sms) {
        for (int bn = 80; bn < best; bn += step)
            if (N % bn == 0 && (long)m_tiles * (N / bn) <= sms) { best = bn; break; }
    }
    return best;
}


typedef void (*gemm_kernel_t)(const KParams);
gemm_kernel_t gemm_entry(int pair, int op) {
    switch ((op << 1) | (pair ? 1 : 0)) {
        case 0: return gemm_tcgen05_kernel<false, 0>;
        case 1: return gemm_tcgen05_kernel<true, 0>;
        case 2: return gemm_tcgen05_kernel<false, 1>;
        case 3: return gemm_tcgen05_kernel<true, 1>;
        case 4: return gemm_tcgen05_kernel<false, 2>;
        case 5: return gemm_tcgen05_kernel<true, 2>;
        case 6: return gemm_tcgen05_kernel<false, 3>;
        default: return gemm_tcgen05_kernel<true, 3>;
    }
}

int configure_gemm_kernels() {
    static std::mutex mu;
    static bool configured[64] = {};
    int dev = 0;
    B200SD_CUDA(cudaGetDevice(&dev));
    std::lock_guard<std::mutex> lock(mu);
    if (dev < 0 || dev >= 64 || configured[dev]) return B200SD_OK;
    for (int i = 0; i < 8; ++i) {
        B200SD_CUDA(cudaFuncSetAttribute(gemm_entry(i & 1, i >> 1), cudaFuncAttributeMaxDynamicSharedMemorySize, (int)(227 * 1024)));
        B200SD_CUDA(cudaFuncSetAttribute(gemm_entry(i & 1, i >> 1), cudaFuncAttributePreferredSharedMemoryCarveout, 100));
    }
    B200SD_CUDA(cudaFuncSetAttribute(gemm_persist_kernel, cudaFuncAttributeMaxDynamicSharedMemorySize, (int)(227 * 1024)));
    B200SD_CUDA(cudaFuncSetAttribute(gemm_persist_kernel, cudaFuncAttributePreferredSharedMemoryCarveout, 100));
    configured[dev] = true;
    return B200SD_OK;
}

bool persist_enabled() { return g_persist != 0; }
int pick_block_n_persist(int N, int m_tiles, bool geglu) {
    const int sms = b200sd_num_sms();
    const int step = geglu ? 64 : 32;
    long best_cost = 0;
    int best = 0;
    for (int bn = step; bn <= 256; bn += step) {
        if (N % bn) continue;
        const long tiles = (long)m_tiles * (N / bn);
        const long cost = ((tiles + sms - 1) / sms) * (BLOCK_M + bn);
        if (best == 0 || cost < best_cost || (cost == best_cost && bn > best)) { best = bn; best_cost = cost; }
    }
    return best;
}

int launch_persist(const b200sd_gemm_args* a, const KParams& k, int m_tiles, b200sd_stream_t stream) {
    PParams p;
    memset(&p, 0, sizeof(p));
    p.tmA0 = k.tmA0; p.tmA1 = k.tmA1; p.tmB = k.tmB;
    p.bias = k.bias; p.rowbias = k.rowbias; p.gn_part = k.gn_part;
    p.M = k.M; p.N = k.N;
    p.num_k_blocks = k.num_k_blocks; p.block_n = k.block_n;
    p.conv = k.conv; p.cblocks0 = k.cblocks0; p.cblocks = k.cblocks;
    p.tile_h = k.tile_h; p.tile_n = k.tile_n; p.tiles_y = k.tiles_y;
    p.tile_w = k.tile_w; p.tiles_x = k.tiles_x;
    p.n_tiles = k.N / k.block_n;
    p.num_tiles = m_tiles * p.n_tiles;
    p.ldrb = k.ldrb; p.rows_per_image = k.rows_per_image;
    p.geglu = k.epilogue == B200SD_EPI_GEGLU;
    p.out_f32 = k.out_f32;
    p.res_kind = k.residual ? (k.res_f32 ? 2 : 1) : 0;
    p.depth = p.res_kind ? kMaxDepth : 2;
    p.split = k.psplit > 1 ? k.psplit : 1;
    p.kb_per_split = ceil_div(k.num_k_blocks, p.split);
    p.residual = k.residual; p.out = k.out; p.ldc = k.ldc; p.ldr = k.ldr;
    const int units = p.num_tiles * p.split;
    if (p.split > 1) {
        B200SD_REQUIRE(k.num_k_blocks >= p.split, "gemm(split-K): fewer K blocks (%d) than slices (%d)", k.num_k_blocks, p.split);
        B200SD_REQUIRE(units <= b200sd_num_sms() && (size_t)units * BLOCK_M * k.block_n * sizeof(float) <= kWsPartialBytes &&
                           (size_t)2 * p.num_tiles * sizeof(int) <= kWsCounterBytes,
                       "gemm(split-K): %d units do not fit the workspace / the machine", units);
        p.depth = 2;
        p.ws = static_cast<float*>(a->workspace);
        p.cnt = reinterpret_cast<int*>(static_cast<char*>(a->workspace) + kWsPartialBytes);
        const uint64_t dims[2] = {(uint64_t)k.block_n, (uint64_t)units * BLOCK_M};
        const uint64_t str[2] = {0, (uint64_t)k.block_n * 4};
        const uint32_t box[2] = {32, 32};
        const int rc = b200sd_make_tmap(&p.tmWs, a->workspace, 2, dims, str, box, CU_TENSOR_MAP_SWIZZLE_128B, CU_TENSOR_MAP_DATA_TYPE_FLOAT32);
        if (rc) return rc;
    }
    const int bn = k.block_n;
    p.acc_stride = bn <= 128 ? 128 : 256;
    p.tmem_cols = 2 * p.acc_stride;
    const int out_cols = p.geglu ? k.N / 2 : k.N;
    {
        const uint64_t dims[2] = {(uint64_t)out_cols, (uint64_t)k.M};
        const uint64_t str[2] = {0, (uint64_t)k.ldc * (k.out_f32 ? 4 : 2)};
        const uint32_t box[2] = {32, 32};
        const int rc = b200sd_make_tmap(&p.tmOut, k.out, 2, dims, str, box, k.out_f32 ? CU_TENSOR_MAP_SWIZZLE_128B : CU_TENSOR_MAP_SWIZZLE_64B,
                                        k.out_f32 ? CU_TENSOR_MAP_DATA_TYPE_FLOAT32 : CU_TENSOR_MAP_DATA_TYPE_BFLOAT16);
        if (rc) return rc;
    }
    if (p.res_kind) {
        const uint64_t dims[2] = {(uint64_t)k.N, (uint64_t)k.M};
        const uint64_t str[2] = {0, (uint64_t)k.ldr * (k.res_f32 ? 4 : 2)};
        const uint32_t box[2] = {32, 32};
        const int rc = b200sd_make_tmap(&p.tmRes, k.residual, 2, dims, str, box, k.res_f32 ? CU_TENSOR_MAP_SWIZZLE_128B : CU_TENSOR_MAP_SWIZZLE_64B,
                                        k.res_f32 ? CU_TENSOR_MAP_DATA_TYPE_FLOAT32 : CU_TENSOR_MAP_DATA_TYPE_BFLOAT16);
        if (rc) return rc;
    }
    const int stage_bytes = kABytes + bn * BLOCK_K * 2;
    p.chunk_bytes = (p.out_f32 || p.res_kind == 2 || k.psplit > 1) ? 4096 : 2048;
    const int epi_bytes = kEpiWarps * p.depth * p.chunk_bytes;
    const int bias_bytes = kEpiWarps * 256 * (int)sizeof(float);
    const int stat_bytes = k.gn_part ? 4 * 2 * 256 * (int)sizeof(float) : 0;
    const int bars_bytes = 512;
    const int budget = 227 * 1024 - 1024;
    int stages = (budget - epi_bytes - bias_bytes - stat_bytes - bars_bytes) / stage_bytes;
    if (stages > kMaxStages) stages = kMaxStages;
    B200SD_REQUIRE(stages >= 2, "gemm(persistent): smem budget leaves %d stages for block_n %d", stages, bn);
    p.stages = stages;
    p.off_b = (uint32_t)stages * kABytes;
    p.off_epi = (uint32_t)stages * stage_bytes;
    p.off_bias = p.off_epi + epi_bytes;
    p.off_stat = p.off_bias + bias_bytes;
    p.off_bars = p.off_stat + stat_bytes;
    const size_t smem_bytes = (size_t)p.off_bars + bars_bytes + 1024;
    {
        const int rc = configure_gemm_kernels();
        if (rc) return rc;
    }
    const int sms = b200sd_num_sms();
    cudaLaunchConfig_t cfg = {};
    cfg.gridDim = dim3(p.split > 1 ? units : (p.num_tiles < sms ? p.num_tiles : sms));
    cfg.blockDim = dim3(kPersistThreads);
    cfg.dynamicSmemBytes = smem_bytes;
    cfg.stream = static_cast<cudaStream_t>(stream);
    cudaLaunchAttribute attr[1];
    if (p.split > 1) {
        attr[0].id = cudaLaunchAttributeCooperative;
        attr[0].val.cooperative = 1;
        cfg.attrs = attr;
        cfg.numAttrs = 1;
    }
    B200SD_CUDA(cudaLaunchKernelEx(&cfg, gemm_persist_kernel, p));
    g_b200sd_launches.fetch_add(1, std::memory_order_relaxed);
    B200SD_LAUNCH_CHECK();
    return B200SD_OK;
}

int launch_gemm(KParams& p, int m_tiles, int n_tiles, int grid_z, bool cluster, b200sd_stream_t stream) {
    const int sms = b200sd_num_sms();
    const int bn = p.block_n;
    if (p.pair) m_tiles = (m_tiles + 1) & ~1;
    const int stage_bytes = kABytes + ((bn * BLOCK_K * 2) >> (p.pair ? 1 : 0));
    const long total_ctas = (long)m_tiles * n_tiles * grid_z;
    int stages;
    if (total_ctas <= sms || bn > 160) stages = (200 * 1024) / stage_bytes;
    else stages = (108 * 1024) / stage_bytes;
    if (stages > kMaxStages) stages = kMaxStages;
    if (stages > p.kb_per_split && total_ctas <= sms) stages = p.kb_per_split;
    const int min_stages = ceil_div(BLOCK_M * (bn + 4) * (int)sizeof(float), stage_bytes);
    if (stages < min_stages) stages = min_stages;
    if (stages < 2) stages = 2;
    p.stages = stages;
    B200SD_REQUIRE((size_t)stages * stage_bytes >= (size_t)BLOCK_M * (bn + 4) * sizeof(float), "gemm: smem ring smaller than the epilogue staging tile");
    const size_t smem_bytes = (size_t)stages * stage_bytes + 1024  + 256  + 3072 ;
    B200SD_REQUIRE(smem_bytes <= 227 * 1024, "gemm: smem budget exceeded (%zu B)", smem_bytes);

    {
        const int rc = configure_gemm_kernels();
        if (rc) return rc;
    }
    cudaLaunchConfig_t cfg = {};
    cfg.gridDim = dim3(m_tiles, n_tiles, grid_z);
    cfg.blockDim = dim3(kNumThreads);
    cfg.dynamicSmemBytes = smem_bytes;
    cfg.stream = static_cast<cudaStream_t>(stream);
    cudaLaunchAttribute attr[1];
    if ((cluster && grid_z > 1) || p.pair) {
        attr[0].id = cudaLaunchAttributeClusterDimension;
        attr[0].val.clusterDim.x = p.pair ? 2 : 1;
        attr[0].val.clusterDim.y = 1;
        attr[0].val.clusterDim.z = p.pair ? 1 : grid_z;
        cfg.attrs = attr;
        cfg.numAttrs = 1;
    }
    B200SD_CUDA(cudaLaunchKernelEx(&cfg, gemm_entry(p.pair, p.b_mode), p));
    g_b200sd_launches.fetch_add(1, std::memory_order_relaxed);
    B200SD_LAUNCH_CHECK();
    return B200SD_OK;
}

bool want_pair(int request, int split, int m_tiles, int n_tiles, int k_blocks) {
    if (request < 0 || split != 1) return false;
    if (request > 0) return true;
    return m_tiles >= 2 && k_blocks >= 32 && (long)m_tiles * n_tiles >= b200sd_num_sms();
}

int pick_block_n_mn(int N, int m_tiles, int kind) {
    int best;
    if (N <= 64) best = 64;
    else if (N <= 128) best = 128;
    else if (kind == 1) best = N <= 192 ? 192 : ((N % 192 == 0 || N % 128 != 0) ? 192 : (N % 256 == 0 ? 256 : 128));
    else best = (N % 192 == 0 && N % 128 != 0) ? 192 : 128;
    while (best > 64 && (long)m_tiles * ceil_div(N, best) * 2 <= b200sd_num_sms()) best -= 64;
    return best;
}

int conv_m_tiling(KParams& p, int NB, int H, int W, int M, int* m_tiles) {
    B200SD_REQUIRE(NB > 0 && H > 0 && W > 0 && M == NB * H * W, "gemm(conv): M=%d != batch*H*W", M);
    p.tiles_x = 1;
    if (W > BLOCK_M) {
        B200SD_REQUIRE(W % BLOCK_M == 0, "gemm(conv): W=%d > 128 must be a multiple of 128", W);
        p.tile_w = BLOCK_M; p.tile_h = 1; p.tile_n = 1;
        p.tiles_x = W / BLOCK_M; p.tiles_y = H;
        p.rows_valid = BLOCK_M;
        p.a_bytes = p.rows_valid * BLOCK_K * 2;
        *m_tiles = NB * H * p.tiles_x;
        return B200SD_OK;
    }
    const int max_h = BLOCK_M / W;
    if (H <= max_h) {
        p.tile_h = H;
        p.tile_n = max_h / H;
        if (p.tile_n < 1) p.tile_n = 1;
        if (p.tile_n > NB) p.tile_n = NB;
    } else {
        p.tile_n = 1;
        p.tile_h = 1;
        for (int h = max_h; h >= 1; --h)
            if (H % h == 0) { p.tile_h = h; break; }
    }
    p.tile_w = W;
    p.tiles_y = H / p.tile_h;
    p.rows_valid = p.tile_w * p.tile_h * p.tile_n;
    p.a_bytes = p.rows_valid * BLOCK_K * 2;
    *m_tiles = (p.tile_n > 1) ? ceil_div(NB, p.tile_n) : NB * p.tiles_y;
    return B200SD_OK;
}

}

extern "C" size_t b200sd_gemm_workspace_bytes(void) { return kWsPartialBytes + kWsCounterBytes; }

extern "C" int b200sd_geglu_tile(int N) {
    if (persist_enabled() && N < 10240) {
        if (N % 256 == 0) return 256;
        if (N % 128 == 0) return 128;
        if (N % 64 == 0) return 64;
    }
    return pick_block_n(N, 1, B200SD_EPI_GEGLU);
}

static int gemm_tiling(const b200sd_gemm_args* a, KParams& p, int* m_tiles_out, int* n_tiles_out) {
    const int C0 = a->C0, C1 = a->a1 ? a->C1 : 0, C = C0 + C1;
    (void)C;
    if (!p.conv) {
        p.rows_valid = BLOCK_M;
        p.a_bytes = kABytes;
        p.tile_w = p.tile_h = p.tile_n = 1;
        p.tiles_x = 1;
        p.tiles_y = 1;
        *m_tiles_out = ceil_div(a->M, BLOCK_M);
    } else {
        const int rc = conv_m_tiling(p, a->batch, a->H, a->W, a->M, m_tiles_out);
        if (rc) return rc;
    }

    const int m_tiles = *m_tiles_out;

    const bool can_split = a->split_k <= 0 && a->epilogue == B200SD_EPI_LINEAR && p.num_k_blocks >= 16;
    int bn = a->block_n > 0 ? a->block_n : pick_block_n(a->N, m_tiles, a->epilogue, can_split);
    B200SD_REQUIRE(bn >= 16 && bn <= 256 && bn % 16 == 0 && a->N % bn == 0, "gemm: bad block_n %d for N=%d", bn, a->N);
    B200SD_REQUIRE(a->epilogue != B200SD_EPI_GEGLU || bn % 32 == 0, "gemm: GEGLU needs block_n %% 32 == 0");
    p.block_n = bn;
    int n_tiles = a->N / bn;
    p.tmem_cols = pow2_cols(bn);

    const int sms = b200sd_num_sms();
    int split = a->split_k;
    if (split <= 0) {
        split = 1;
        const int tiles = m_tiles * n_tiles;
        if (a->epilogue == B200SD_EPI_LINEAR && tiles * 2 <= sms && p.num_k_blocks >= 16) {
            while (split < 8 && tiles * split * 2 <= sms && p.num_k_blocks / (split * 2) >= 8) split *= 2;
        }
    }
    int n_tiles_f = n_tiles;
    if (a->split_k <= 0 && a->block_n <= 0 && can_split) {
        const int tiles = m_tiles * n_tiles;
        if (split == 8 && tiles > 8) split = 4;
        if (split <= 4 && tiles * split * 2 <= sms && bn % 32 == 0 && bn / 2 >= 80) {
            bn /= 2;
            p.block_n = bn;
            n_tiles_f = a->N / bn;
            p.tmem_cols = pow2_cols(bn);
        }
    }
    B200SD_REQUIRE(split == 1 || a->epilogue == B200SD_EPI_LINEAR, "gemm: split-K only with the linear epilogue");
    B200SD_REQUIRE(split == 1 || split == 2 || split == 4 || split == 8, "gemm: split_k must be 1, 2, 4 or 8 (cluster size)");
    p.kb_per_split = ceil_div(p.num_k_blocks, split);
    B200SD_REQUIRE((split - 1) * p.kb_per_split < p.num_k_blocks, "gemm: split_k=%d leaves an empty split for K=%d", split, a->K);
    *n_tiles_out = n_tiles_f;
    p.split_k = split;
    p.pair = want_pair(a->pair, split, m_tiles, n_tiles_f, p.num_k_blocks) && bn % 32 == 0;
    p.persist = 0;
    p.psplit = 0;
    const bool geglu = a->epilogue == B200SD_EPI_GEGLU;
    if (persist_enabled() && a->split_k <= 0 && a->block_n <= 0 && split > 1 && !geglu && p.rows_valid == BLOCK_M &&
        a->N % 32 == 0 && a->workspace != nullptr && a->workspace_bytes >= kWsPartialBytes + kWsCounterBytes &&
        (reinterpret_cast<uintptr_t>(a->workspace) & 127) == 0 && a->ldc % 4 == 0 && (!a->residual || a->ldr % 4 == 0)) {
        int bnp = 0;
        for (int cand : {160, 128, 256, 192, 96, 64, 32})
            if (a->N % cand == 0) { bnp = cand; break; }
        const int sms_s = b200sd_num_sms();
        const long tiles = bnp ? (long)m_tiles * (a->N / bnp) : sms_s + 1;
        int S = 1;
        while (S < 16 && tiles * (S * 2) <= sms_s && p.num_k_blocks / (S * 2) >= 4) S *= 2;
        if (S == 16 && p.num_k_blocks >= 128) {
            p.persist = 1;
            p.psplit = S;
            p.block_n = bnp;
            p.split_k = 1;
            p.pair = 0;
            *n_tiles_out = a->N / bnp;
            return B200SD_OK;
        }
    }
    if (persist_enabled() && split == 1 && !p.pair && p.rows_valid == BLOCK_M && a->N % 32 == 0 &&
        (!a->rowbias || (a->rows_per_image > 0 && a->rows_per_image % 32 == 0)) &&
        !(a->residual && a->residual == a->out && a->residual_dtype != a->out_dtype)) {
        const int bnp = a->block_n > 0 ? a->block_n : pick_block_n_persist(a->N, m_tiles, geglu);
        const long ptiles = bnp > 0 ? (long)m_tiles * (a->N / bnp) : 0;
        const bool multi = ptiles >= 2L * b200sd_num_sms();
        if (bnp > 0 && bnp <= 256 && bnp % (geglu ? 64 : 32) == 0 && a->N % bnp == 0 && (multi || g_persist > 0)) {
            p.persist = 1;
            p.block_n = bnp;
            *n_tiles_out = a->N / bnp;
        }
    }
    return B200SD_OK;
}

extern "C" int b200sd_gemm(const b200sd_gemm_args* a, b200sd_stream_t stream) {
    B200SD_REQUIRE(a != nullptr, "gemm: null args");
    B200SD_REQUIRE(a->a0 && a->w && a->out, "gemm: null operand pointer");
    B200SD_REQUIRE(a->M > 0 && a->N > 0 && a->K > 0, "gemm: non-positive dims M=%d N=%d K=%d", a->M, a->N, a->K);
    B200SD_REQUIRE(a->conv_taps == 1 || a->conv_taps == 9, "gemm: conv_taps must be 1 or 9");
    const int C0 = a->C0, C1 = a->a1 ? a->C1 : 0, C = C0 + C1;
    B200SD_REQUIRE(C0 > 0 && C0 % BLOCK_K == 0 && C1 % BLOCK_K == 0, "gemm: channel counts must be multiples of 64 (C0=%d C1=%d)", C0, C1);
    B200SD_REQUIRE(a->K == a->conv_taps * C, "gemm: K=%d != taps*C=%d", a->K, a->conv_taps * C);
    B200SD_REQUIRE(a->N % 16 == 0, "gemm: N=%d must be a multiple of 16", a->N);
    B200SD_REQUIRE(a->epilogue == B200SD_EPI_LINEAR || a->epilogue == B200SD_EPI_GEGLU, "gemm: bad epilogue");
    B200SD_REQUIRE(a->epilogue != B200SD_EPI_GEGLU || (a->bias && !a->residual && !a->rowbias && a->out_dtype == B200SD_BF16),
                   "gemm: GEGLU epilogue needs bias, bf16 out and no residual/rowbias");
    B200SD_REQUIRE(a->out_dtype == B200SD_BF16 || a->out_dtype == B200SD_F32, "gemm: bad out dtype");
    B200SD_REQUIRE(a->residual_dtype == B200SD_BF16 || a->residual_dtype == B200SD_F32, "gemm: bad residual dtype");
    B200SD_REQUIRE(a->ldc % 8 == 0 && (!a->residual || a->ldr % 8 == 0), "gemm: ldc/ldr must be multiples of 8");
    B200SD_REQUIRE((reinterpret_cast<uintptr_t>(a->out) & 15) == 0 && (reinterpret_cast<uintptr_t>(a->a0) & 15) == 0 &&
                       (reinterpret_cast<uintptr_t>(a->w) & 15) == 0 && (reinterpret_cast<uintptr_t>(a->a1) & 15) == 0 &&
                       (reinterpret_cast<uintptr_t>(a->residual) & 15) == 0 && (reinterpret_cast<uintptr_t>(a->bias) & 15) == 0 &&
                       (reinterpret_cast<uintptr_t>(a->rowbias) & 15) == 0,
                   "gemm: pointers must be 16-byte aligned");
    B200SD_REQUIRE(!a->rowbias || (a->rows_per_image > 0 && a->ldrb % 4 == 0), "gemm: rowbias needs rows_per_image and ldrb %% 4 == 0");

    KParams p;
    memset(&p, 0, sizeof(p));
    p.M = a->M;
    p.N = a->N;
    p.num_k_blocks = a->K / BLOCK_K;
    p.conv = a->conv_taps == 9;
    p.cblocks0 = C0 / BLOCK_K;
    p.cblocks = C / BLOCK_K;
    p.bias = a->bias;
    p.rowbias = a->rowbias;
    p.residual = a->residual;
    p.res_f32 = a->residual_dtype == B200SD_F32;
    p.out = a->out;
    p.ldc = a->ldc;
    p.ldr = a->ldr;
    p.ldrb = a->ldrb > 0 ? a->ldrb : a->N;
    p.rows_per_image = a->rows_per_image > 0 ? a->rows_per_image : 1;
    p.epilogue = a->epilogue;
    p.out_f32 = a->out_dtype == B200SD_F32;
    p.conv_sign = 1;
    p.n_valid = a->N;
    p.tiles_per_tap = 1;

    int m_tiles = 0, n_tiles = 0;
    {
        const int rc = gemm_tiling(a, p, &m_tiles, &n_tiles);
        if (rc) return rc;
    }
    const int bn = p.block_n, split = p.split_k;
    p.gn_part = a->gn_part;
    B200SD_REQUIRE(!a->gn_part || (a->out_dtype == B200SD_F32 && a->epilogue == B200SD_EPI_LINEAR &&
                                   (!a->residual || a->residual_dtype == B200SD_F32)),
                   "gemm: gn_part needs fp32 output, the linear epilogue and no bf16 residual");

    if (!p.conv) {
        const uint64_t dimsA[2] = {(uint64_t)C0, (uint64_t)a->M};
        const uint64_t strA[2] = {0, (uint64_t)(a->lda0 > 0 ? a->lda0 : C0) * 2};
        const uint32_t boxA[2] = {BLOCK_K, BLOCK_M};
        int rc = b200sd_make_tmap(&p.tmA0, a->a0, 2, dimsA, strA, boxA, CU_TENSOR_MAP_SWIZZLE_128B);
        if (rc) return rc;
        if (C1 > 0) {
            const uint64_t dimsA1[2] = {(uint64_t)C1, (uint64_t)a->M};
            const uint64_t strA1[2] = {0, (uint64_t)(a->lda1 > 0 ? a->lda1 : C1) * 2};
            rc = b200sd_make_tmap(&p.tmA1, a->a1, 2, dimsA1, strA1, boxA, CU_TENSOR_MAP_SWIZZLE_128B);
            if (rc) return rc;
        }
    } else {
        const uint32_t boxA[4] = {BLOCK_K, (uint32_t)p.tile_w, (uint32_t)p.tile_h, (uint32_t)p.tile_n};
        const uint64_t dims0[4] = {(uint64_t)C0, (uint64_t)a->W, (uint64_t)a->H, (uint64_t)a->batch};
        const uint64_t str0[4] = {0, (uint64_t)C0 * 2, (uint64_t)a->W * C0 * 2, (uint64_t)a->H * a->W * C0 * 2};
        int rc = b200sd_make_tmap(&p.tmA0, a->a0, 4, dims0, str0, boxA, CU_TENSOR_MAP_SWIZZLE_128B);
        if (rc) return rc;
        if (C1 > 0) {
            const uint64_t dims1[4] = {(uint64_t)C1, (uint64_t)a->W, (uint64_t)a->H, (uint64_t)a->batch};
            const uint64_t str1[4] = {0, (uint64_t)C1 * 2, (uint64_t)a->W * C1 * 2, (uint64_t)a->H * a->W * C1 * 2};
            rc = b200sd_make_tmap(&p.tmA1, a->a1, 4, dims1, str1, boxA, CU_TENSOR_MAP_SWIZZLE_128B);
            if (rc) return rc;
        }
    }
    {
        const uint64_t dimsB[2] = {(uint64_t)a->K, (uint64_t)a->N};
        const uint64_t strB[2] = {0, (uint64_t)a->K * 2};
        const uint32_t boxB[2] = {BLOCK_K, (uint32_t)(p.pair ? bn / 2 : bn)};
        int rc = b200sd_make_tmap(&p.tmB, a->w, 2, dimsB, strB, boxB, CU_TENSOR_MAP_SWIZZLE_128B);
        if (rc) return rc;
    }

    if (p.persist) return launch_persist(a, p, m_tiles, stream);
    return launch_gemm(p, m_tiles, n_tiles, split, true, stream);
}

extern "C" int b200sd_gemm_gn_layout(const b200sd_gemm_args* a, int hw, int* parts_per_image, int* total_parts) {
    B200SD_REQUIRE(a && parts_per_image && total_parts && hw > 0, "gemm_gn_layout: bad arguments");
    KParams p;
    memset(&p, 0, sizeof(p));
    p.M = a->M;
    p.N = a->N;
    p.num_k_blocks = a->K / BLOCK_K;
    p.conv = a->conv_taps == 9;
    int m_tiles = 0, n_tiles = 0;
    const int rc = gemm_tiling(a, p, &m_tiles, &n_tiles);
    if (rc) return rc;
    *parts_per_image = 0;
    *total_parts = 0;
    if (a->out_dtype != B200SD_F32 || a->epilogue != B200SD_EPI_LINEAR || (a->residual && a->residual_dtype != B200SD_F32)) return B200SD_OK;
    if (p.persist && p.psplit > 1) {
        const int rpc = BLOCK_M / p.psplit;
        if (a->M % hw != 0 || hw % rpc != 0 || (p.conv && a->H * a->W != hw)) return B200SD_OK;
        *parts_per_image = hw / rpc;
        *total_parts = m_tiles * p.psplit;
        return B200SD_OK;
    }
    if (p.persist) {
        if (a->M % hw != 0 || hw % BLOCK_M != 0 || (p.conv && a->H * a->W != hw)) return B200SD_OK;
        *parts_per_image = hw / BLOCK_M;
        *total_parts = m_tiles;
        return B200SD_OK;
    }
    const int rpp = BLOCK_M / p.split_k;
    int ppi;
    if (p.conv) {
        if (a->H * a->W != hw) return B200SD_OK;
        if (p.tile_n == 1) ppi = p.tiles_y * p.tiles_x * p.split_k;
        else if (p.rows_valid == BLOCK_M && hw % rpp == 0) ppi = hw / rpp;
        else return B200SD_OK;
    } else {
        if (a->M % hw != 0 || hw % rpp != 0) return B200SD_OK;
        ppi = hw / rpp;
    }
    if (p.pair) m_tiles = (m_tiles + 1) & ~1;
    *parts_per_image = ppi;
    *total_parts = m_tiles * p.split_k;
    return B200SD_OK;
}

extern "C" int b200sd_gemm_dgrad(const b200sd_dgrad_args* a, b200sd_stream_t stream) {
    B200SD_REQUIRE(a != nullptr && a->dy && a->w && a->out, "dgrad: null pointer");
    B200SD_REQUIRE(a->conv_taps == 1 || a->conv_taps == 9, "dgrad: conv_taps must be 1 or 9");
    B200SD_REQUIRE(a->M > 0 && a->Cout > 0 && a->Cout % BLOCK_K == 0, "dgrad: Cout=%d must be a positive multiple of 64", a->Cout);
    B200SD_REQUIRE(a->Cin > 0 && a->Cin % 8 == 0, "dgrad: Cin=%d must be a multiple of 8", a->Cin);
    B200SD_REQUIRE(a->out_dtype == B200SD_BF16 || a->out_dtype == B200SD_F32, "dgrad: bad out dtype");
    const int ldy = a->ldy > 0 ? a->ldy : a->Cout;
    const int ldc = a->ldc > 0 ? a->ldc : a->Cin;
    const int ldr = a->ldr > 0 ? a->ldr : a->Cin;
    B200SD_REQUIRE(ldc % 8 == 0 && ldr % 8 == 0 && ldy % 8 == 0, "dgrad: pitches must be multiples of 8");
    B200SD_REQUIRE(((reinterpret_cast<uintptr_t>(a->dy) | reinterpret_cast<uintptr_t>(a->w) | reinterpret_cast<uintptr_t>(a->out) |
                     reinterpret_cast<uintptr_t>(a->residual)) & 15) == 0, "dgrad: pointers must be 16-byte aligned");
    KParams p;
    memset(&p, 0, sizeof(p));
    p.M = a->M;
    p.N = a->Cin;
    p.n_valid = a->Cin;
    p.tiles_per_tap = 1;
    p.conv = a->conv_taps == 9;
    p.conv_sign = -1;
    p.b_mode = 1;
    p.cblocks0 = p.cblocks = a->Cout / BLOCK_K;
    p.num_k_blocks = a->conv_taps * p.cblocks;
    p.residual = a->residual;
    p.res_f32 = a->residual_dtype == B200SD_F32;
    p.out = a->out;
    p.ldc = ldc;
    p.ldr = ldr;
    p.ldrb = a->Cin;
    p.rows_per_image = 1;
    p.epilogue = B200SD_EPI_LINEAR;
    p.out_f32 = a->out_dtype == B200SD_F32;
    int m_tiles;
    if (!p.conv) {
        p.rows_valid = BLOCK_M;
        p.a_bytes = kABytes;
        p.tile_w = p.tile_h = p.tile_n = p.tiles_y = 1;
        p.tiles_x = 1;
        m_tiles = ceil_div(a->M, BLOCK_M);
    } else {
        B200SD_REQUIRE(ldy == a->Cout, "dgrad(conv): dy must be dense NHWC");
        const int rc = conv_m_tiling(p, a->batch, a->H, a->W, a->M, &m_tiles);
        if (rc) return rc;
    }
    int bn = a->block_n > 0 ? a->block_n : pick_block_n_mn(a->Cin, m_tiles, 0);
    B200SD_REQUIRE(bn % 64 == 0 && bn >= 64 && bn <= 256, "dgrad: block_n %d must be 64, 128, 192 or 256", bn);
    p.pair = want_pair(a->pair, 1, m_tiles, ceil_div(a->Cin, bn), p.num_k_blocks);
    if (p.pair && bn % 128 != 0) {
        if (a->block_n > 0) p.pair = 0;
        else bn = (ceil_div(a->Cin, 256) * 256 <= ceil_div(a->Cin, 128) * 128) ? 256 : 128;
    }
    p.block_n = bn;
    const int n_tiles = ceil_div(a->Cin, bn);
    p.tmem_cols = pow2_cols(bn);
    int split = 1;
    {
        const int sms = b200sd_num_sms();
        const int tiles = m_tiles * n_tiles;
        if (!p.pair && tiles * 2 <= sms && p.num_k_blocks >= 16) {
            while (split < 8 && tiles * split * 2 <= sms && p.num_k_blocks / (split * 2) >= 8) split *= 2;
            if (split == 8 && tiles > 8) split = 4;
        }
    }
    p.split_k = split;
    p.kb_per_split = ceil_div(p.num_k_blocks, split);
    while (split > 1 && (split - 1) * p.kb_per_split >= p.num_k_blocks) {
        split /= 2;
        p.split_k = split;
        p.kb_per_split = ceil_div(p.num_k_blocks, split);
    }
    int rc;
// ... 105 lines not shown
```

stable-diffusion-for-book-cover-generation_b200/csrc/norm.cu:

```cuda
#include <atomic>

#include <algorithm>


#include "common.cuh"

extern std::atomic<long long> g_b200sd_launches;
#define COUNT_LAUNCH() g_b200sd_launches.fetch_add(1, std::memory_order_relaxed)

namespace {

__device__ __forceinline__ void st8_lo(bf16* lo, size_t i, const float (&y)[8]) {
    float r[8];
#pragma unroll
    for (int j = 0; j < 8; ++j) r[j] = y[j] - __bfloat162float(__float2bfloat16(y[j]));
    st8<B200SD_BF16>(lo, i, r);
}

constexpr int kGnThreads = 256;
constexpr int kMaxSlabs = 128;
constexpr int kCounterFloats = 1024;
constexpr int kMaxGroups = 32;

template <int DT>
// ... 407 lines not shown
                                           int silu, int in_dtype, b200sd_stream_t stream) {
    B200SD_REQUIRE(raw_lo == nullptr || raw_out != nullptr, "groupnorm: raw_lo needs raw_out");
    B200SD_REQUIRE(x0 && gamma && beta && out && stats_ws, "groupnorm: null pointer");
    if (!x1) C1 = 0;
    const int C = C0 + C1;
    B200SD_REQUIRE(batch > 0 && hw > 0 && batch <= kCounterFloats, "groupnorm: bad batch/hw");
    B200SD_REQUIRE(groups > 0 && groups <= kMaxGroups && C % groups == 0 && (C / groups) % 2 == 0,
                   "groupnorm: C=%d groups=%d unsupported (channels per group must be even)", C, groups);
    B200SD_REQUIRE(C0 % 8 == 0 && C1 % 8 == 0, "groupnorm: channel counts must be multiples of 8");
    B200SD_REQUIRE(C * sizeof(float2) <= 48 * 1024, "groupnorm: C=%d too large", C);
    cudaStream_t s = static_cast<cudaStream_t>(stream);
    B200SD_REQUIRE(in_dtype == B200SD_BF16 || in_dtype == B200SD_F32, "groupnorm: bad input dtype");
    {
        const int cpg = C / groups;
        int G = 1;
        while ((G * cpg) % 8 != 0 && G < groups) G *= 2;
        while (G * 2 <= groups && groups % (G * 2) == 0 && G * cpg < 32) G *= 2;
        const int Cg = G * cpg;
        if ((Cg % 8) == 0 && groups % G == 0 && Cg / 8 <= 512 && (long)hw * C <= 3000000L) {
            const int VC = Cg / 8;
            const int sets = groups / G;
            int CL = 1;
            while (CL < 8 && (long)batch * sets * CL < b200sd_num_sms() && hw / (CL * 2) >= 32) CL *= 2;
            const int ppc = ceil_div(hw, CL);
            int R = 256 / VC;
            if (R < 1) R = 1;
            if (R > ppc) R = ppc;
            int threads = ((VC * R + 31) / 32) * 32;
            if (threads < 32) threads = 32;
            const size_t smem = ((size_t)2 * R * Cg + 2 * Cg + threads) * sizeof(float);
            cudaLaunchConfig_t cfg = {};
            cfg.gridDim = dim3(CL, sets, batch);
            cfg.blockDim = dim3(threads);
            cfg.dynamicSmemBytes = smem;
            cfg.stream = s;
            cudaLaunchAttribute attr[1];
            if (CL > 1) {
                attr[0].id = cudaLaunchAttributeClusterDimension;
                attr[0].val.clusterDim.x = CL;
                attr[0].val.clusterDim.y = 1;
                attr[0].val.clusterDim.z = 1;
                cfg.attrs = attr;
                cfg.numAttrs = 1;
            }
            if (in_dtype == B200SD_F32)
                B200SD_CUDA(cudaLaunchKernelEx(&cfg, gn_fused_kernel<B200SD_F32>, x0, x1, C0, C1, gamma, beta, static_cast<bf16*>(out),
                                               static_cast<bf16*>(raw_out), static_cast<bf16*>(out_lo), static_cast<bf16*>(raw_lo), hw, groups, G, CL, ppc, R, eps,
                                               silu, stats_out));
            else
                B200SD_CUDA(cudaLaunchKernelEx(&cfg, gn_fused_kernel<B200SD_BF16>, x0, x1, C0, C1, gamma, beta, static_cast<bf16*>(out),
                                               static_cast<bf16*>(raw_out), static_cast<bf16*>(out_lo), static_cast<bf16*>(raw_lo), hw, groups, G, CL, ppc, R, eps,
                                               silu, stats_out));
            COUNT_LAUNCH();
            B200SD_LAUNCH_CHECK();
            return B200SD_OK;
        }
    }
    const int C8 = C / 8;
    B200SD_REQUIRE(C8 <= 1024, "groupnorm: C=%d too large", C);
    const int rows_per_pass = (C8 >= 256) ? 1 : 256 / C8;
    int threads = ((C8 * rows_per_pass + 31) / 32) * 32;
    if (threads < 256) threads = 256;
    unsigned int* counters = reinterpret_cast<unsigned int*>(stats_ws);
    float* mean_rstd = stats_ws + kCounterFloats;
    float* partial = mean_rstd + 2 * (size_t)batch * kMaxGroups;
    int slabs = ceil_div(b200sd_num_sms() * 2, batch);
    if (slabs > kMaxSlabs) slabs = kMaxSlabs;
    int pps = ceil_div(hw, slabs);
    pps = ceil_div(pps, rows_per_pass) * rows_per_pass;
    slabs = ceil_div(hw, pps);
    const size_t st_smem = (size_t)2 * rows_per_pass * C * sizeof(float);
    if (in_dtype == B200SD_F32)
        gn_stats_kernel<B200SD_F32><<<dim3(slabs, batch), dim3(threads), st_smem, s>>>(x0, x1, C0, C1, partial,
                                  mean_rstd, counters, hw, groups, pps, rows_per_pass, eps);
    else
        gn_stats_kernel<B200SD_BF16><<<dim3(slabs, batch), dim3(threads), st_smem, s>>>(x0, x1, C0, C1, partial,
                                  mean_rstd, counters, hw, groups, pps, rows_per_pass, eps);
    COUNT_LAUNCH();
    B200SD_LAUNCH_CHECK();
    if (stats_out != nullptr)
        B200SD_CUDA(cudaMemcpyAsync(stats_out, mean_rstd, (size_t)2 * batch * groups * sizeof(float), cudaMemcpyDeviceToDevice, s));
    int blocks = ceil_div(b200sd_num_sms() * 4, batch);
    int ppb = ceil_div(hw, blocks);
    const int min_ppb = ceil_div(kGnThreads * 4, C / 8);
    if (ppb < min_ppb) ppb = min_ppb;
    blocks = ceil_div(hw, ppb);
    if (in_dtype == B200SD_F32)
        gn_apply_kernel<B200SD_F32><<<dim3(blocks, batch), dim3(kGnThreads), C * sizeof(float2), s>>>(x0, x1, C0, C1,
                                  gamma, beta, static_cast<bf16*>(out), static_cast<bf16*>(raw_out), static_cast<bf16*>(out_lo), static_cast<bf16*>(raw_lo),
                                  mean_rstd, hw, groups, silu, ppb);
    else
        gn_apply_kernel<B200SD_BF16><<<dim3(blocks, batch), dim3(kGnThreads), C * sizeof(float2), s>>>(x0, x1, C0, C1,
                                  gamma, beta, static_cast<bf16*>(out), static_cast<bf16*>(raw_out), static_cast<bf16*>(out_lo), static_cast<bf16*>(raw_lo),
                                  mean_rstd, hw, groups, silu, ppb);
    COUNT_LAUNCH();
    B200SD_LAUNCH_CHECK();
    return B200SD_OK;
}

extern "C" int b200sd_groupnorm_silu(const void* x0, const void* x1, int C0, int C1, const float* gamma,
                                     const float* beta, void* out, void* raw_out, float* stats_ws, int batch, int hw,
                                     int groups, float eps, int silu, int in_dtype, b200sd_stream_t stream) {
    return b200sd_groupnorm_silu_split(x0, x1, C0, C1, gamma, beta, out, nullptr, raw_out, nullptr, stats_ws, nullptr, batch, hw,
                                       groups, eps, silu, in_dtype, stream);
}

extern "C" int b200sd_groupnorm_silu_stats(const void* x0, const void* x1, int C0, int C1, const float* gamma,
                                           const float* beta, void* out, void* raw_out, float* stats_ws, float* stats_out,
                                           int batch, int hw, int groups, float eps, int silu, int in_dtype,
                                           b200sd_stream_t stream) {
    return b200sd_groupnorm_silu_split(x0, x1, C0, C1, gamma, beta, out, nullptr, raw_out, nullptr, stats_ws, stats_out, batch, hw,
                                       groups, eps, silu, in_dtype, stream);
}

extern "C" int b200sd_groupnorm_workspace_floats(int batch) {
    return kCounterFloats + 2 * batch * kMaxGroups + 2 * batch * kMaxSlabs * kMaxGroups;
}

extern "C" int b200sd_layernorm_split(const void* x, const float* gamma, const float* beta, void* out, void* out_lo, int rows,
                                      int C, float eps, int in_dtype, b200sd_stream_t stream) {
    B200SD_REQUIRE(x && gamma && beta && out, "layernorm: null pointer");
    B200SD_REQUIRE(rows > 0, "layernorm: rows must be positive");
    B200SD_REQUIRE(C % 64 == 0 && C >= 64 && C <= 1280, "layernorm: C=%d unsupported (multiple of 64, <= 1280)", C);
    cudaStream_t s = static_cast<cudaStream_t>(stream);
    const int blocks = ceil_div(rows, 8);
    const void* xi = x;
    B200SD_REQUIRE(in_dtype == B200SD_BF16 || in_dtype == B200SD_F32, "layernorm: bad input dtype");
    bf16* xo = static_cast<bf16*>(out);
    bf16* xl = static_cast<bf16*>(out_lo);
#define LN_CASE(P)                                                                                     \
    case P:                                                                                            \
        if (in_dtype == B200SD_F32)                                                                         \
            layernorm_kernel<P, B200SD_F32><<<dim3(blocks), dim3(256), 0, s>>>(xi, gamma, beta, xo, xl, rows, C, eps); \
        else                                                                                                \
            layernorm_kernel<P, B200SD_BF16><<<dim3(blocks), dim3(256), 0, s>>>(xi, gamma, beta, xo, xl, rows, C, eps); \
        break;
    switch (C / 64) {
        LN_CASE(1) LN_CASE(2) LN_CASE(3) LN_CASE(4) LN_CASE(5) LN_CASE(6) LN_CASE(7) LN_CASE(8) LN_CASE(9) LN_CASE(10)
        LN_CASE(11) LN_CASE(12) LN_CASE(13) LN_CASE(14) LN_CASE(15) LN_CASE(16) LN_CASE(17) LN_CASE(18) LN_CASE(19) LN_CASE(20)
        default:
            B200SD_REQUIRE(false, "layernorm: C=%d unsupported", C);
    }
#undef LN_CASE
    COUNT_LAUNCH();
    B200SD_LAUNCH_CHECK();
    return B200SD_OK;
}

extern "C" int b200sd_layernorm(const void* x, const float* gamma, const float* beta, void* out, int rows, int C,
                                float eps, int in_dtype, b200sd_stream_t stream) {
    return b200sd_layernorm_split(x, gamma, beta, out, nullptr, rows, C, eps, in_dtype, stream);
}

extern "C" int b200sd_groupnorm_silu_parts(const void* x0, const void* x1, int C0, int C1, const float* part0, int ppi0, int ld0,
                                           const float* part1, int ppi1, int ld1, const float* gamma, const float* beta, void* out,
                                           void* raw_out, float* stats_out, int batch, int hw, int groups, float eps, int silu,
                                           int in_dtype, b200sd_stream_t stream) {
    B200SD_REQUIRE(x0 && part0 && gamma && beta && out && ppi0 > 0, "groupnorm_parts: null pointer");
    if (!x1) C1 = 0;
    B200SD_REQUIRE(C1 == 0 || (part1 && ppi1 > 0), "groupnorm_parts: x1 without its statistics");
    const int C = C0 + C1;
    B200SD_REQUIRE(batch > 0 && hw > 0 && groups > 0 && groups <= kMaxGroups && C % groups == 0, "groupnorm_parts: bad shape");
    B200SD_REQUIRE(C0 % 8 == 0 && C1 % 8 == 0, "groupnorm_parts: channel counts must be multiples of 8");
    B200SD_REQUIRE(in_dtype == B200SD_BF16 || in_dtype == B200SD_F32, "groupnorm_parts: bad input dtype");
    const int cpg = C / groups;
    int G = 1;
    while ((G * cpg) % 8 != 0 && G < groups) G *= 2;
    while (G * 2 <= groups && groups % (G * 2) == 0 && G * cpg < 32) G *= 2;
    const int Cg = G * cpg;
    if ((Cg % 8) != 0 || groups % G != 0 || Cg / 8 > 512) return B200SD_ERR_UNSUPPORTED;
    const int VC = Cg / 8, sets = groups / G;
    int slabs = ceil_div(b200sd_num_sms() * 2, batch * sets);
    if (slabs > hw / 32) slabs = hw / 32;
    if (slabs < 1) slabs = 1;
    const int ppc = ceil_div(hw, slabs);
    slabs = ceil_div(hw, ppc);
    int R = 256 / VC;
    if (R < 1) R = 1;
    if (R > ppc) R = ppc;
    int threads = ((VC * R + 31) / 32) * 32;
    if (threads < 64) threads = 64;
    const size_t smem = ((size_t)4 * Cg + (size_t)std::max(threads, 2 * Cg)) * sizeof(float);
    cudaStream_t s = static_cast<cudaStream_t>(stream);
    if (in_dtype == B200SD_F32)
        gn_parts_kernel<B200SD_F32><<<dim3(slabs, sets, batch), dim3(threads), smem, s>>>(x0, x1, C0, C1, part0, ppi0,
                                  ld0, part1, ppi1, ld1, gamma, beta, static_cast<bf16*>(out), static_cast<bf16*>(raw_out), hw, groups, G,
                                  ppc, R, eps, silu, stats_out);
    else
        gn_parts_kernel<B200SD_BF16><<<dim3(slabs, sets, batch), dim3(threads), smem, s>>>(x0, x1, C0, C1, part0, ppi0,
                                  ld0, part1, ppi1, ld1, gamma, beta, static_cast<bf16*>(out), static_cast<bf16*>(raw_out), hw, groups, G,
                                  ppc, R, eps, silu, stats_out);
    COUNT_LAUNCH();
    B200SD_LAUNCH_CHECK();
    return B200SD_OK;
}
```

stable-diffusion-for-book-cover-generation_b200/engine.py:

```python
from __future__ import annotations

import torch

from . import ops
from .plan import Builder, ContextKey, Plan, Pool, capture, profile_plan, run_plan


class Engine(Builder):
    def __init__(self, model, N, H, W, S_ctx, device, io=None):
        super().__init__(device)
        self.model, self.N, self.H, self.W, self.S = model, N, H, W, S_ctx
        self._io = io
        cfg = model.config
        self.heads = cfg.attention_head_dim
        self.ctx_dim = cfg.cross_attention_dim
        self.plan = Plan()
        self.ctx_plan = Plan()
        self.graph = None
        self._ctx_key = ContextKey()
        self.debug = False
        self.debug_out = {}
        with torch.cuda.device(device):
            self._build()

    def _tap(self, name, t, h, w):
        def op():
            if self.debug:
                self.debug_out[name] = t.float().reshape(self.N, h, w, -1).permute(0, 3, 1, 2).clone()
        self.plan.append(op, "tap")

    def _build(self):
        m, Wp, N, dev = self.model, self.model._packed, self.N, self.device
        cfg = m.config
        boc = cfg.block_out_channels
        P, pool = self.plan, Pool(dev)
        self.pool = pool
        f32 = dict(dtype=torch.float32, device=dev)

        if self._io is not None:
            self.in_sample, self.in_t, self.out = self._io
        else:
            self.in_sample = torch.zeros(N, cfg.in_channels, self.H, self.W, **f32)
            self.in_t = torch.zeros(N, **f32)
            self.out = torch.zeros(N, cfg.out_channels, self.H, self.W, **f32)
        self.in_ctx = torch.zeros(N * self.S, self.ctx_dim, dtype=torch.bfloat16, device=dev)

        temb_dim = boc[0] * 4
        t_sin = torch.empty(N, boc[0], **f32)
        t_h = torch.empty(N, temb_dim, **f32)
        t_emb = torch.empty(N, temb_dim, **f32)
        tp_off, n_tp = m._tproj_offsets()
        self.tproj = torch.empty(N, n_tp, **f32)
        te = Wp["temb"]
        P.append(lambda: ops.timestep_embedding(self.in_t, boc[0], out=t_sin), "time_embed")
        P.append(lambda: ops.small_linear(t_sin, te["w1"], te["b1"], silu_out=True, out=t_h), "time_embed")
        P.append(lambda: ops.small_linear(t_h, te["w2"], te["b2"], out=t_emb), "time_embed")
        self.large_batch = N >= 8
        if self.large_batch:
            a16 = torch.empty(N, temb_dim, dtype=torch.bfloat16, device=dev)
            P.append(lambda: ops.cast_act(t_emb, a16, silu=True), "time_embed")
            self.gemm(P, a16, Wp["tproj"]["w"], self.tproj, bias=Wp["tproj"]["b"], kind="time_embed",
                      name="time_emb_proj x22 (tensor cores)")
        else:
            P.append(lambda: ops.small_linear(t_emb, Wp["tproj"]["w"], Wp["tproj"]["b"], silu_in=True, out=self.tproj), "time_embed", 0, "time_emb_proj x22")

        self.attn_ws = torch.empty(ops.attention_workspace_bytes(N, self.heads, self.H * self.W, boc[0] // self.heads) + 256,
                                   dtype=torch.uint8, device=dev)

        h, w = self.H, self.W
        F32 = torch.float32
        x = pool.get(N * h * w, boc[0], F32)
        P.append(lambda x=x: ops.conv_in(self.in_sample, Wp["conv_in"]["w"], Wp["conv_in"]["b"], x), "conv_io", 0, "conv_in")
        self._tap("conv_in", x, h, w)

        def resnet(prefix, r, x, skip, h, w):
            wr = Wp[prefix]
            M = N * h * w
            cin, cout = r.cin, r.cout
            t1 = pool.get(M, cin)
            raw = pool.get(M, cin) if "wsc" in wr else None
            self.groupnorm(P, x, skip, wr["g1"], wr["b1"], t1, N, h * w, cfg.norm_eps, True, raw_out=raw)
            hbuf = pool.get(M, cout, F32)
            rb = (self.tproj.data_ptr() + tp_off[prefix] * 4, n_tp, h * w)
            self.gemm(P, t1, wr["w1"], hbuf, bias=wr["cb1"], conv=(N, h, w), rowbias_ptr=rb, gn_hw=h * w)
            pool.put(t1)
            t2 = pool.get(M, cout)
            self.groupnorm(P, hbuf, None, wr["g2"], wr["b2"], t2, N, h * w, cfg.norm_eps, True)
            pool.put(hbuf)
            if "wsc" in wr:
                sc = pool.get(M, cout, F32)
                self.gemm(P, raw, wr["wsc"], sc, bias=wr["bsc"])
                pool.put(raw)
            else:
                sc = x
            y = pool.get(M, cout, F32)
            self.gemm(P, t2, wr["w2"], y, bias=wr["cb2"], residual=sc, conv=(N, h, w), gn_hw=h * w)
            pool.put(t2)
            if sc is not x:
                pool.put(sc)
            self._tap(prefix, y, h, w)
            return y

        def xformer(prefix, a, x, h, w):
            wa = Wp[prefix]
            Cc = a.ch
            M = N * h * w
            d = Cc // self.heads
            scale = d ** -0.5
            kv = torch.empty(N * self.S, 2 * Cc, dtype=torch.bfloat16, device=dev)
            self.gemm(self.ctx_plan, self.in_ctx, wa["w_kv2"], kv)
            t = pool.get(M, Cc)
            self.groupnorm(P, x, None, wa["gn_g"], wa["gn_b"], t, N, h * w, 1e-6, False)
            hs = pool.get(M, Cc, F32)
            self.gemm(P, t, wa["w_in"], hs, bias=wa["b_in"])
            P.append(lambda: ops.layernorm(hs, wa["ln1_g"], wa["ln1_b"], t), "layernorm")
            qkv = pool.get(M, 3 * Cc)
            self.gemm(P, t, wa["w_qkv"], qkv)
            P.append(lambda: ops.attention(qkv, qkv, qkv, t, N, self.heads, h * w, h * w, d, scale, ldq=3 * Cc,
                                           ldk=3 * Cc, ldv=3 * Cc, ldo=Cc, q_off=0, k_off=Cc, v_off=2 * Cc, ws=self.attn_ws),
                     "attention", 4.0 * N * self.heads * (h * w) * (h * w) * d, f"self-attn S{h * w} d{d}")
            pool.put(qkv)
            self.gemm(P, t, wa["w_o1"], hs, bias=wa["b_o1"], residual=hs)
            P.append(lambda: ops.layernorm(hs, wa["ln2_g"], wa["ln2_b"], t), "layernorm")
            q = pool.get(M, Cc)
            self.gemm(P, t, wa["w_q2"], q)
            P.append(lambda: ops.attention(q, kv, kv, t, N, self.heads, h * w, self.S, d, scale, ldq=Cc, ldk=2 * Cc,
                                           ldv=2 * Cc, ldo=Cc, k_off=0, v_off=Cc, ws=self.attn_ws),
                     "attention", 4.0 * N * self.heads * (h * w) * self.S * d, f"cross-attn S{h * w} d{d}")
            pool.put(q)
            self.gemm(P, t, wa["w_o2"], hs, bias=wa["b_o2"], residual=hs)
            P.append(lambda: ops.layernorm(hs, wa["ln3_g"], wa["ln3_b"], t), "layernorm")
            ff = pool.get(M, 4 * Cc)
            self.gemm(P, t, wa["w_ff1"], ff, bias=wa["b_ff1"], epilogue=ops.EPI_GEGLU, block_n=wa["ff_tile"])
            self.gemm(P, ff, wa["w_ff2"], t, bias=wa["b_ff2"], residual=hs)
            pool.put(ff)
            y = pool.get(M, Cc, F32)
            self.gemm(P, t, wa["w_out"], y, bias=wa["b_out"], residual=x, gn_hw=h * w)
            pool.put(t)
            pool.put(hs)
            self._tap(prefix, y, h, w)
            return y

        def downsample(prefix, _s, x, h, w):
            Cc = x.shape[1]
            col = pool.get(N * (h // 2) * (w // 2), 9 * Cc)
            P.append(lambda x=x, col=col, h=h, w=w: ops.im2col_s2(x, col, N, h, w), "resample", 0, "im2col_s2")
            h, w = h // 2, w // 2
            y = pool.get(N * h * w, Cc, F32)
            self.gemm(P, col, Wp[prefix]["w"], y, bias=Wp[prefix]["b"], gn_hw=h * w)
            pool.put(col)
            self._tap(prefix, y, h, w)
            return y

        def upsample(prefix, _s, x, h, w):
            Cc = x.shape[1]
            up = pool.get(N * 4 * h * w, Cc)
            P.append(lambda x=x, up=up, h=h, w=w: ops.upsample2x(x, up, N, h, w), "resample", 0, "upsample2x")
            h, w = 2 * h, 2 * w
            y = pool.get(N * h * w, Cc, F32)
            self.gemm(P, up, Wp[prefix]["w"], y, bias=Wp[prefix]["b"], conv=(N, h, w), gn_hw=h * w)
            pool.put(up)
            self._tap(prefix, y, h, w)
            return y

        x, h, w = m._walk(x, h, w, resnet=resnet, xformer=xformer, downsample=downsample, upsample=upsample, release=pool.put)

        wo = Wp["conv_out"]
        t = pool.get(N * h * w, boc[0])
        self.groupnorm(P, x, None, wo["g"], wo["beta"], t, N, h * w, cfg.norm_eps, True)
        if self.large_batch and boc[0] % 64 == 0 and cfg.out_channels <= 4:
            tmp = pool.get(N * h * w, 32, F32)
            self.gemm(P, t, wo["w_tc"], tmp, a1=t, conv=(N, h, w), kind="conv_io", name="conv_out (tensor cores)")
            P.append(lambda tmp=tmp: ops.nhwc_bias_to_nchw(tmp, wo["b"], self.out), "conv_io", 0, "conv_out: bias + NCHW")
        else:
            P.append(lambda t=t: ops.conv_out(t, wo["w"], wo["b"], self.out), "conv_io", 0, "conv_out")
        self.activation_bytes = pool.total

    def set_context(self, ctx):
        if self._ctx_key.matches(ctx):
            return
        self.in_ctx.copy_(ctx.reshape(self.N * self.S, self.ctx_dim))
        run_plan(self.ctx_plan)
        self._ctx_key.set(ctx)

    def run(self, sample, timestep, ctx, use_graph=True):
        with torch.cuda.device(self.device):
            self.set_context(ctx)
            self.in_sample.copy_(sample)
            if torch.is_tensor(timestep):
                self.in_t.copy_(timestep.to(device=self.device, dtype=torch.float32).reshape(-1).expand(self.N))
            else:
                self.in_t.fill_(float(timestep))
            if not use_graph:
                run_plan(self.plan)
            elif self.graph is None:
                self.graph, self.kernels_per_graph = capture(self.plan)
            else:
                self.graph.replay()
            return self.out.clone()

    def profile(self, iters=5):
        return profile_plan(self.plan, self.device, iters)
```

stable-diffusion-for-book-cover-generation_b200/ops.py:

```python
from __future__ import annotations

import ctypes as C

import torch

from ._lib import DgradArgs, GemmArgs, WgradArgs, B200SDError, check, lib

F32, BF16 = 0, 1
EPI_LINEAR, EPI_GEGLU = 0, 1


def _up16(*ts):
    had = any(t is not None and t.dtype == torch.float16 for t in ts)
    return tuple(t.float() if (t is not None and t.dtype == torch.float16) else t for t in ts) + (had,)


def _dt(t: torch.Tensor) -> int:
    if t.dtype == torch.float32:
        return F32
    if t.dtype == torch.bfloat16:
        return BF16
    raise B200SDError(f"unsupported dtype {t.dtype} (float32 / bfloat16 only)")


def _chk(*ts):
    for t in ts:
        if t is None:
            continue
        if not t.is_cuda:
            raise B200SDError("b200sd ops need CUDA tensors (there is no CPU fallback)")
        if not t.is_contiguous():
            raise B200SDError("b200sd ops need contiguous tensors")


def _p(t):
    return None if t is None else t.data_ptr()


def _stream():
    return torch.cuda.current_stream().cuda_stream


_ws_cache: dict = {}
_ws_retired: list = []


def _workspace(key, nbytes, device, zero=True):
    k = (key, device.index if device.index is not None else torch.cuda.current_device())
    t = _ws_cache.get(k)
    if t is None or t.numel() < nbytes:
        if t is not None:
            _ws_retired.append(t)
        t = (torch.zeros if zero else torch.empty)(nbytes, dtype=torch.uint8, device=device)
        _ws_cache[k] = t
    return t


def attention_workspace_bytes(batch, heads, Skv, d) -> int:
    return int(lib().b200sd_attention_workspace_bytes(batch, heads, Skv, d))


def attention_bwd_workspace_bytes(batch, heads, Sq) -> int:
    return int(lib().b200sd_attention_bwd_workspace_bytes(batch, heads, Sq))


def launch_count() -> int:
    return int(lib().b200sd_launch_count())


def cfg_ddim_step(eps_u, eps_c, x, guidance, sa_t, sb_t, sa_p, sb_p, out=None, eps_out=None):
    eps_u, eps_c, x, half = _up16(eps_u, eps_c, x)
    if half:
        if eps_out is not None:
            raise B200SDError("cfg_ddim_step: eps_out is not supported with float16 inputs")
        r = cfg_ddim_step(eps_u.contiguous(), None if eps_c is None else eps_c.contiguous(), x.contiguous(), guidance, sa_t, sb_t,
                          sa_p, sb_p).half()
        return r if out is None else out.copy_(r)
    _chk(eps_u, eps_c, x, out, eps_out)
    if out is None:
        out = torch.empty_like(x)
    if eps_c is not None and eps_c.shape != eps_u.shape:
        raise ValueError("eps_u / eps_c shape mismatch")
    if eps_u.numel() != x.numel():
        raise ValueError(f"model_output {tuple(eps_u.shape)} and sample {tuple(x.shape)} sizes differ")
    check(lib().b200sd_cfg_ddim_step(_p(eps_u), _p(eps_c), _p(x), _p(out), _p(eps_out), x.numel(), float(guidance),
                                     float(sa_t), float(sb_t), float(sa_p), float(sb_p), _dt(eps_u), _dt(x), _stream()),
          "cfg_ddim_step")
    return out


def cfg_plms_step(eps_u, eps_c, x, hist, weights, guidance, cx, ce, out=None, eps_out=None):
    eps_u, eps_c, x, half = _up16(eps_u, eps_c, x)
    if half:
        r = cfg_plms_step(eps_u.contiguous(), None if eps_c is None else eps_c.contiguous(), x.contiguous(), hist, weights, guidance,
                          cx, ce, eps_out=eps_out).half()
        return r if out is None else out.copy_(r)
    _chk(eps_u, eps_c, x, out, eps_out, *hist)
    if out is None:
        out = torch.empty_like(x)
    if eps_u.numel() != x.numel():
        raise ValueError(f"model_output {tuple(eps_u.shape)} and sample {tuple(x.shape)} sizes differ")
    w = (C.c_float * 5)(*([float(v) for v in weights] + [0.0] * (5 - len(weights))))
    hp = [_p(h) for h in hist] + [None] * (4 - len(hist))
    check(lib().b200sd_cfg_plms_step(_p(eps_u), _p(eps_c), _p(x), _p(out), _p(eps_out), hp[0], hp[1], hp[2], hp[3],
                                     len(hist), w, x.numel(), float(guidance), float(cx), float(ce), _dt(eps_u), _dt(x),
                                     _stream()), "cfg_plms_step")
    return out


def sampler_advance(t_table, cursor, in_t):
    check(lib().b200sd_sampler_advance(_p(t_table), t_table.numel(), _p(cursor), _p(in_t), in_t.numel(), _stream()),
          "sampler_advance")


def cfg_ddim_step_table(eps_u, eps_c, x, out, guidance, coef_table, cursor):
    check(lib().b200sd_cfg_ddim_step_table(_p(eps_u), _p(eps_c), _p(x), _p(out), None, x.numel(), float(guidance), _p(coef_table),
                                           _p(cursor), F32, F32, _stream()), "cfg_ddim_step_table")


def cfg_plms_step_table(eps_u, eps_c, x, saved, ring, guidance, coef_table, cursor):
    check(lib().b200sd_cfg_plms_step_table(_p(eps_u), _p(eps_c), _p(x), _p(saved), _p(ring), x.numel(), float(guidance),
                                           _p(coef_table), _p(cursor), _stream()), "cfg_plms_step_table")


def add_noise(x0, noise, timesteps, sa_table, sb_table, out=None):
    x0, noise, half = _up16(x0, noise)
    if half:
        r = add_noise(x0.contiguous(), noise.contiguous(), timesteps, sa_table, sb_table).half()
        return r if out is None else out.copy_(r)
    _chk(x0, noise, timesteps, sa_table, sb_table, out)
    if x0.shape != noise.shape:
        raise ValueError("original_samples / noise shape mismatch")
    if timesteps.dtype != torch.int64 or timesteps.numel() != x0.shape[0]:
        raise ValueError("timesteps must be int64 of shape (batch,)")
    if noise.dtype != x0.dtype:
        noise = noise.to(x0.dtype)
    if out is None:
        out = torch.empty_like(x0)
    B = x0.shape[0]
    check(lib().b200sd_add_noise(_p(x0), _p(noise), _p(timesteps), _p(sa_table), _p(sb_table), _p(out), B,
                                 x0.numel() // max(B, 1), sa_table.numel(), _dt(x0), _stream()), "add_noise")
    return out


def mse_loss_fwd(pred, target):
    _chk(pred, target)
    if pred.shape != target.shape:
        raise ValueError("pred / target shape mismatch")
    ws = _workspace("mse", lib().b200sd_mse_workspace_floats() * 4, pred.device)
    out = torch.empty(1, dtype=torch.float32, device=pred.device)
    check(lib().b200sd_mse_loss_fwd(_p(pred), _p(target), _p(out), _p(ws), pred.numel(), _dt(pred), _dt(target),
                                    _stream()), "mse_loss_fwd")
    return out


def mse_loss_bwd(pred, target, grad_loss):
    _chk(pred, target, grad_loss)
    g = torch.empty_like(pred)
    gl = grad_loss.reshape(1).to(torch.float32)
    check(lib().b200sd_mse_loss_bwd(_p(pred), _p(target), _p(gl), _p(g), pred.numel(), _dt(pred), _dt(target),
                                    _stream()), "mse_loss_bwd")
    return g


class _MSELoss(torch.autograd.Function):
    @staticmethod
    def forward(ctx, pred, target):
        ctx.pred_dtype = pred.dtype
        pred, target, _ = _up16(pred, target)
        ctx.save_for_backward(pred, target)
        return mse_loss_fwd(pred.contiguous(), target.contiguous()).reshape(())

    @staticmethod
    def backward(ctx, grad):
        pred, target = ctx.saved_tensors
        return mse_loss_bwd(pred.contiguous(), target.contiguous(), grad.contiguous().float()).to(ctx.pred_dtype), None


def mse_loss(pred, target):
    return _MSELoss.apply(pred, target)


def timestep_embedding(t_f32, dim, out=None):
    _chk(t_f32, out)
    B = t_f32.numel()
    if out is None:
        out = torch.empty(B, dim, dtype=torch.float32, device=t_f32.device)
    check(lib().b200sd_timestep_embedding(_p(t_f32), _p(out), B, dim, _stream()), "timestep_embedding")
    return out


def small_linear(x, w_bf16, bias, silu_in=False, silu_out=False, out=None):
    _chk(x, w_bf16, bias, out)
    B, K = x.shape
    N = w_bf16.shape[0]
    if out is None:
        out = torch.empty(B, N, dtype=torch.float32, device=x.device)
    check(lib().b200sd_small_linear(_p(x), _p(w_bf16), _p(bias), _p(out), B, N, K, int(silu_in), int(silu_out),
                                    _stream()), "small_linear")
    return out


def gemm_workspace(device):
    return _workspace(("gemm", _stream()), max(16, lib().b200sd_gemm_workspace_bytes()), device)


def gemm(a0, w, out, *, a1=None, bias=None, rowbias=None, residual=None, conv=None, rows_per_image=0,
         epilogue=EPI_LINEAR, block_n=0, split_k=0, M=None, ldrb=0, launch=True, pair=0):
    _chk(a0, a1, w, bias, rowbias, residual, out)
    N, K = w.shape
    C0 = a0.shape[-1]
    C1 = a1.shape[-1] if a1 is not None else 0
    if M is None:
        M = a0.numel() // C0
    ws = gemm_workspace(a0.device)
    args = GemmArgs()
    args.a0, args.a1, args.w = _p(a0), _p(a1), _p(w)
    args.bias, args.rowbias, args.residual, args.out = _p(bias), _p(rowbias), _p(residual), _p(out)
    args.M, args.N, args.K, args.C0, args.C1 = M, N, K, C0, C1
    args.lda0, args.lda1 = C0, C1
    args.ldc = out.shape[-1]
    args.ldr = residual.shape[-1] if residual is not None else 0
    args.ldrb = ldrb
    if conv is not None:
        args.conv_taps = 9
        args.batch, args.H, args.W = conv
    else:
        args.conv_taps = 1
    args.rows_per_image = rows_per_image
    args.epilogue = epilogue
    args.out_dtype = _dt(out)
    args.residual_dtype = _dt(residual) if residual is not None else BF16
    args.block_n, args.split_k = block_n, split_k
    args.pair = pair
    args.workspace, args.workspace_bytes = _p(ws), ws.numel()
    if not launch:
        return args
    gemm_run(args)
    return out


def gemm_run(args):
    check(lib().b200sd_gemm(C.byref(args), _stream()), "gemm")


class GnParts:
    __slots__ = ("buf", "ppi", "ld")

    def __init__(self, buf, ppi, ld):
        self.buf, self.ppi, self.ld = buf, ppi, ld


def gemm_attach_gn_parts(args, hw, device):
    ppi, total = C.c_int(0), C.c_int(0)
    check(lib().b200sd_gemm_gn_layout(C.byref(args), int(hw), C.byref(ppi), C.byref(total)), "gemm_gn_layout")
    if ppi.value <= 0:
        return None
    buf = torch.zeros(total.value * 2 * args.N, dtype=torch.float32, device=device)
    args.gn_part = buf.data_ptr()
    return GnParts(buf, ppi.value, args.N)


def groupnorm_silu_parts(x0, x1, parts0, parts1, gamma, beta, out, batch, hw, groups=32, eps=1e-5, silu=True, raw_out=None,
                         stats_out=None):
    _chk(x0, x1, gamma, beta, out, raw_out, stats_out)
    C0 = x0.shape[-1]
    C1 = x1.shape[-1] if x1 is not None else 0
    rc = lib().b200sd_groupnorm_silu_parts(_p(x0), _p(x1), C0, C1, _p(parts0.buf), parts0.ppi, parts0.ld,
                                           _p(parts1.buf) if parts1 is not None else None, parts1.ppi if parts1 is not None else 0,
                                           parts1.ld if parts1 is not None else 0, _p(gamma), _p(beta), _p(out), _p(raw_out),
                                           _p(stats_out), batch, hw, groups, float(eps), int(silu), _dt(x0), _stream())
    check(rc, "groupnorm_silu_parts")
    return out


def gn_parts_supported(C, groups=32):
    if C % groups:
        return False
    cpg = C // groups
    G = 1
    while (G * cpg) % 8 != 0 and G < groups:
        G *= 2
    while G * 2 <= groups and groups % (G * 2) == 0 and G * cpg < 32:
        G *= 2
    Cg = G * cpg
    return Cg % 8 == 0 and groups % G == 0 and Cg // 8 <= 512


def gemm_dgrad(dy, w, out, *, residual=None, conv=None, Cin=None, block_n=0, launch=True, pair=0):
    _chk(dy, w, residual, out)
    Cout = w.shape[0]
    taps = 9 if conv is not None else 1
    if Cin is None:
        Cin = w.shape[1] // taps
    a = DgradArgs()
    a.dy, a.w, a.residual, a.out = _p(dy), _p(w), _p(residual), _p(out)
    a.M, a.Cout, a.Cin, a.conv_taps = dy.numel() // dy.shape[-1], Cout, Cin, taps
    if conv is not None:
        a.batch, a.H, a.W = conv
    a.ldy, a.ldc = dy.shape[-1], out.shape[-1]
    a.ldr = residual.shape[-1] if residual is not None else 0
    a.out_dtype = _dt(out)
    a.residual_dtype = _dt(residual) if residual is not None else BF16
    a.block_n = block_n
    a.pair = pair
    if not launch:
        return a
    gemm_dgrad_run(a)
    return out


def gemm_dgrad_run(args):
    check(lib().b200sd_gemm_dgrad(C.byref(args), _stream()), "gemm_dgrad")


def gemm_wgrad(dy, x, dw, *, conv=None, lddw=0, block_n=0, split_k=0, launch=True):
    _chk(dy, x, dw)
    if dw.dtype != torch.float32:
        raise B200SDError("gemm_wgrad: dw must be float32")
    a = WgradArgs()
    a.dy, a.x, a.dw = _p(dy), _p(x), _p(dw)
    a.rows, a.Cout, a.Cin = dy.numel() // dy.shape[-1], dy.shape[-1], x.shape[-1]
    a.conv_taps = 9 if conv is not None else 1
    if conv is not None:
        a.batch, a.H, a.W = conv
    a.ldy, a.ldx, a.lddw = dy.shape[-1], x.shape[-1], lddw
    a.block_n, a.split_k = block_n, split_k
    if not launch:
        return a
    gemm_wgrad_run(a)
    return dw


def gemm_wgrad_run(args):
    check(lib().b200sd_gemm_wgrad(C.byref(args), _stream()), "gemm_wgrad")


def geglu_tile(N):
    return int(lib().b200sd_geglu_tile(N))


def conv_in(x_nchw, w_packed, bias, out):
    _chk(x_nchw, w_packed, bias, out)
    B, Cin, H, W = x_nchw.shape
    check(lib().b200sd_conv_in(_p(x_nchw), _p(w_packed), _p(bias), _p(out), B, Cin, w_packed.shape[0], H, W, _dt(out), _stream()),
          "conv_in")
    return out


def conv_out(x_nhwc, w_packed, bias, out_nchw):
    _chk(x_nhwc, w_packed, bias, out_nchw)
    B, Cout, H, W = out_nchw.shape
    check(lib().b200sd_conv_out(_p(x_nhwc), _p(w_packed), _p(bias), _p(out_nchw), B, x_nhwc.shape[-1], Cout, H, W,
                                _stream()), "conv_out")
    return out_nchw


def nhwc_bias_to_nchw(x_f32, bias, out_nchw):
    _chk(x_f32, bias, out_nchw)
    B, C, H, W = out_nchw.shape
    check(lib().b200sd_nhwc_bias_to_nchw(_p(x_f32), _p(bias), _p(out_nchw), B, C, H * W, x_f32.shape[-1], _stream()), "nhwc_bias_to_nchw")
    return out_nchw


def groupnorm_silu(x0, x1, gamma, beta, out, batch, hw, groups=32, eps=1e-5, silu=True, raw_out=None, stats_out=None):
    _chk(x0, x1, gamma, beta, out, raw_out, stats_out)
    if x1 is not None and x1.dtype != x0.dtype:
        raise B200SDError("groupnorm: both sources must have the same dtype")
    ws = _workspace(("gn", _stream()), lib().b200sd_groupnorm_workspace_floats(batch) * 4, x0.device)
    C0 = x0.shape[-1]
    C1 = x1.shape[-1] if x1 is not None else 0
    check(lib().b200sd_groupnorm_silu_stats(_p(x0), _p(x1), C0, C1, _p(gamma), _p(beta), _p(out), _p(raw_out), _p(ws),
                                            _p(stats_out), batch, hw, groups, float(eps), int(silu), _dt(x0), _stream()),
          "groupnorm_silu")
    return out


def layernorm(x, gamma, beta, out, eps=1e-5):
    _chk(x, gamma, beta, out)
    Cc = x.shape[-1]
    check(lib().b200sd_layernorm(_p(x), _p(gamma), _p(beta), _p(out), x.numel() // Cc, Cc, float(eps), _dt(x), _stream()),
          "layernorm")
    return out


def attention(q, k, v, out, batch, heads, Sq, Skv, d, scale, ldq=None, ldk=None, ldv=None, ldo=None,
              q_off=0, k_off=0, v_off=0, ws=None):
    _chk(q, k, v, out)
    es = 2
    if ws is None:
        ws = _workspace("attn", lib().b200sd_attention_workspace_bytes(batch, heads, Skv, d) + 128, q.device, zero=False)
    check(lib().b200sd_attention(q.data_ptr() + q_off * es, k.data_ptr() + k_off * es, v.data_ptr() + v_off * es,
                                 _p(out), batch, heads, Sq, Skv, d, ldq or q.shape[-1], ldk or k.shape[-1],
                                 ldv or v.shape[-1], ldo or out.shape[-1], float(scale), _p(ws), ws.numel(), _stream()),
          "attention")
    return out


def upsample2x(x, out, batch, H, W):
    _chk(x, out)
    check(lib().b200sd_upsample2x(_p(x), _p(out), batch, H, W, x.shape[-1], _dt(x), _stream()), "upsample2x")
    return out


def im2col_s2(x, out, batch, H, W, pad=1):
    _chk(x, out)
    check(lib().b200sd_im2col_s2_pad(_p(x), _p(out), batch, H, W, x.shape[-1], _dt(x), int(pad), _stream()), "im2col_s2")
    return out


def attention_lse(q, k, v, out, lse, batch, heads, Sq, Skv, d, scale, ldq=None, ldk=None, ldv=None, ldo=None,
                  q_off=0, k_off=0, v_off=0, ws=None):
    _chk(q, k, v, out, lse)
    if ws is None:
        ws = _workspace("attn", lib().b200sd_attention_workspace_bytes(batch, heads, Skv, d) + 128, q.device, zero=False)
# ... 242 lines not shown
```

stable-diffusion-for-book-cover-generation_b200/plan.py:

```python
from __future__ import annotations

import ctypes as C
import weakref

import torch

from . import ops
from ._lib import check, lib


class Pool:

    def __init__(self, device):
        self.device, self.free, self.total = device, {}, 0

    def get(self, rows, cols, dtype=torch.bfloat16):
        lst = self.free.get((rows * cols, dtype))
        if lst:
            return lst.pop().view(rows, cols)
        self.total += rows * cols * (2 if dtype == torch.bfloat16 else 4)
        return torch.empty(rows, cols, dtype=dtype, device=self.device)

    def put(self, *ts):
        for t in ts:
            if t is not None:
                self.free.setdefault((t.numel(), t.dtype), []).append(t)


class Plan(list):

    def __init__(self):
        super().__init__()
        self.meta = []

    def append(self, fn, kind="other", flops=0.0, name=""):
        super().append(fn)
        self.meta.append((kind, float(flops), name))


def run_plan(plan):
    for op in plan:
        op()


def capture(plan, capture_error_mode="global"):
    run_plan(plan)
    torch.cuda.current_stream().synchronize()
    g = torch.cuda.CUDAGraph()
    before = ops.launch_count()
    with torch.cuda.graph(g, capture_error_mode=capture_error_mode):
        run_plan(plan)
    return g, ops.launch_count() - before


class ContextKey:

    def __init__(self):
        self.ref, self.version = None, None

    def matches(self, ctx):
        return self.ref is not None and self.ref() is ctx and self.version == ctx._version

    def set(self, ctx):
        self.ref, self.version = weakref.ref(ctx), ctx._version


class Builder:

    def __init__(self, device):
        self.device = device
        self._keep = []
        self._gn_parts = {}

    def gemm(self, plan, a0, w, out, *, rowbias_ptr=None, gn_hw=0, kind=None, name=None, **kw):
        args = ops.gemm(a0, w, out, launch=False, **kw)
        if rowbias_ptr is not None:
            args.rowbias, args.ldrb, args.rows_per_image = rowbias_ptr
        self._gn_parts.pop(id(out), None)
        if gn_hw > 0:
            parts = ops.gemm_attach_gn_parts(args, gn_hw, self.device)
            if parts is not None:
                self._gn_parts[id(out)] = parts
                self._keep.append(parts)
        self._keep.append((a0, w, out, kw))
        k = "conv3x3" if args.conv_taps == 9 else "gemm"
        plan.append(lambda a=args: ops.gemm_run(a), kind or k, 2.0 * args.M * args.N * args.K,
                    name or f"{k} M{args.M} N{args.N} K{args.K}")

    def dgrad(self, plan, dy, w, out, *, name=None, **kw):
        args = ops.gemm_dgrad(dy, w, out, launch=False, **kw)
        self._keep.append((dy, w, out, kw))
        plan.append(lambda a=args: ops.gemm_dgrad_run(a), "gemm", 2.0 * args.M * args.Cout * args.Cin * args.conv_taps,
                    name or f"dgrad M{args.M} N{args.Cin} K{args.Cout * args.conv_taps}")

    def wgrad(self, plan, dy, x, dw, **kw):
        if dw is None:
            return
        args = ops.gemm_wgrad(dy, x, dw, launch=False, **kw)
        self._keep.append((dy, x, dw, kw))
        plan.append(lambda a=args: ops.gemm_wgrad_run(a), "gemm", 2.0 * args.rows * args.Cout * args.Cin * args.conv_taps,
                    f"wgrad M{args.Cout} N{args.Cin * args.conv_taps} K{args.rows}")

    def groupnorm(self, plan, x, skip, g, b, out, batch, hw, eps, silu, *, groups=32, raw_out=None, stats_out=None):
        p0 = self._gn_parts.get(id(x))
        p1 = self._gn_parts.get(id(skip)) if skip is not None else None
        Cc = x.shape[-1] + (skip.shape[-1] if skip is not None else 0)
        if p0 is not None and (skip is None or p1 is not None) and ops.gn_parts_supported(Cc, groups):
            self._keep.append((p0, p1))
            plan.append(lambda: ops.groupnorm_silu_parts(x, skip, p0, p1, g, b, out, batch, hw, groups, eps, silu, raw_out=raw_out,
                                                         stats_out=stats_out), "groupnorm", 0, "groupnorm (stats from GEMM)")
        else:
            plan.append(lambda: ops.groupnorm_silu(x, skip, g, b, out, batch, hw, groups, eps, silu, raw_out=raw_out,
                                                   stats_out=stats_out), "groupnorm")


def profile_plan(plan, device, iters=5):
    with torch.cuda.device(device):
        entries = [(op, meta) for op, meta in zip(plan, plan.meta) if meta[0] != "tap"]
        n = len(entries)
        check(lib().b200sd_timer_reserve(n + 1), "timer_reserve")

        def run_all():
            for op, _m in entries:
                op()
        run_all()
        torch.cuda.synchronize()
        side = torch.cuda.Stream()
        g = torch.cuda.CUDAGraph()
        with torch.cuda.graph(g, stream=side):
            sh = torch.cuda.current_stream().cuda_stream
            for i, (op, _meta) in enumerate(entries):
                check(lib().b200sd_timer_record(i, sh), "timer_record")
                op()
            check(lib().b200sd_timer_record(n, sh), "timer_record")
        torch.cuda.synchronize()
        times = [0.0] * n
        total = 0.0
        ms = C.c_float(0.0)
        g.replay()
        torch.cuda.synchronize()
        for _ in range(iters):
            g.replay()
            torch.cuda.synchronize()
            for i in range(n):
                check(lib().b200sd_timer_elapsed_ms(i, i + 1, C.byref(ms)), "timer_elapsed")
                times[i] += ms.value / iters
            check(lib().b200sd_timer_elapsed_ms(0, n, C.byref(ms)), "timer_elapsed")
            total += ms.value / iters
        acc, per_op = {}, []
        for t, (op, (kind, flops, name)) in zip(times, entries):
            a = acc.setdefault(kind, [0.0, 0.0, 0])
            a[0] += t
            a[1] += flops
            a[2] += 1
            per_op.append((name or kind, t, flops))
        run_all()
        torch.cuda.synchronize()
    return acc, per_op, total
```

Baseline: 203.8.

## Fuse LayerNorm and GroupNorm into preceding GEMM epilogue with grid-wide stat sync

Adds a normalization epilogue to the tcgen05 GEMM. The epilogue keeps the output tile in shared memory, writes per-tile partial row or group statistics to global memory, and waits on a grid-wide arrival counter. It then reduces the statistics and writes the normalized bf16 output directly. The plan builder attaches this epilogue to the GEMM that feeds a layernorm, or a groupnorm without skip input, which removes a separate normalization launch and the re-read of the GEMM output. The cost is a spin-wait grid barrier that requires all dependent CTAs to be co-resident, plus extra shared-memory use that may reduce pipeline stages.

```diff
diff --git a/include/b200sd.h b/include/b200sd.h
--- a/include/b200sd.h
+++ b/include/b200sd.h
@@ -89,11 +89,25 @@
     size_t workspace_bytes;
     int pair;
     float* gn_part;
+    void* norm_out;
+    int ld_norm;
+    int norm_kind;
+    const float* gamma;
+    const float* beta;
+    float eps;
+    int silu;
+    int groups;
+    void* norm_ws;
 } b200sd_gemm_args;
+
+#define B200SD_NORM_NONE 0
+#define B200SD_NORM_LAYER 1
+#define B200SD_NORM_GROUP 2
 
 size_t b200sd_gemm_workspace_bytes(void);
 int b200sd_geglu_tile(int N);
 int b200sd_gemm(const b200sd_gemm_args* args, b200sd_stream_t stream);
+int b200sd_gemm_norm_query(const b200sd_gemm_args* args, int* supported, size_t* ws_bytes);
 int b200sd_gemm_gn_layout(const b200sd_gemm_args* args, int hw, int* parts_per_image, int* total_parts);
 
 typedef struct b200sd_dgrad_args {
diff --git a/stable-diffusion-for-book-cover-generation_b200/_lib.py b/stable-diffusion-for-book-cover-generation_b200/_lib.py
--- a/stable-diffusion-for-book-cover-generation_b200/_lib.py
+++ b/stable-diffusion-for-book-cover-generation_b200/_lib.py
@@ -22,6 +22,8 @@
         ("batch", C.c_int), ("H", C.c_int), ("W", C.c_int), ("rows_per_image", C.c_int), ("epilogue", C.c_int),
         ("out_dtype", C.c_int), ("residual_dtype", C.c_int), ("block_n", C.c_int), ("split_k", C.c_int),
         ("workspace", C.c_void_p), ("workspace_bytes", C.c_size_t), ("pair", C.c_int), ("gn_part", C.c_void_p),
+        ("norm_out", C.c_void_p), ("ld_norm", C.c_int), ("norm_kind", C.c_int), ("gamma", C.c_void_p), ("beta", C.c_void_p),
+        ("eps", C.c_float), ("silu", C.c_int), ("groups", C.c_int), ("norm_ws", C.c_void_p),
     ]
 
 
@@ -80,6 +82,7 @@
     "b200sd_geglu_tile": (_i, [_i]),
     "b200sd_gemm": (_i, [C.POINTER(GemmArgs), _vp]),
     "b200sd_gemm_gn_layout": (_i, [C.POINTER(GemmArgs), _i, C.POINTER(C.c_int), C.POINTER(C.c_int)]),
+    "b200sd_gemm_norm_query": (_i, [C.POINTER(GemmArgs), C.POINTER(C.c_int), C.POINTER(C.c_size_t)]),
     "b200sd_groupnorm_silu_parts": (_i, [_vp, _vp, _i, _i, _vp, _i, _i, _vp, _i, _i, _vp, _vp, _vp, _vp, _vp, _i, _i, _i, _f, _i,
                                          _i, _vp]),
     "b200sd_gemm_dgrad": (_i, [C.POINTER(DgradArgs), _vp]),
diff --git a/stable-diffusion-for-book-cover-generation_b200/csrc/api.cu b/stable-diffusion-for-book-cover-generation_b200/csrc/api.cu
--- a/stable-diffusion-for-book-cover-generation_b200/csrc/api.cu
+++ b/stable-diffusion-for-book-cover-generation_b200/csrc/api.cu
@@ -38,7 +38,7 @@
     configured[key] = bytes;
     return cudaSuccess;
 }
-extern "C" int b200sd_version(void) { return 101; }
+extern "C" int b200sd_version(void) { return 102; }
 extern "C" int64_t b200sd_launch_count(void) { return g_b200sd_launches.load(); }
 
 #include <vector>
diff --git a/stable-diffusion-for-book-cover-generation_b200/csrc/common.cuh b/stable-diffusion-for-book-cover-generation_b200/csrc/common.cuh
--- a/stable-diffusion-for-book-cover-generation_b200/csrc/common.cuh
+++ b/stable-diffusion-for-book-cover-generation_b200/csrc/common.cuh
@@ -34,6 +34,8 @@
 static inline int ceil_div(int a, int b) { return (a + b - 1) / b; }
 
 int b200sd_num_sms();
+
+bool b200sd_gn_parts_shape(int C, int groups, int batch, int hw, int* G, int* slabs, int* ppc, int* R, int* threads, int* fold_ways);
 
 int b200sd_make_tmap(CUtensorMap* out, const void* base, int rank, const uint64_t* dims,
                      const uint64_t* strides_bytes, const uint32_t* box, CUtensorMapSwizzle swizzle,
diff --git a/stable-diffusion-for-book-cover-generation_b200/csrc/gemm_tcgen05.cu b/stable-diffusion-for-book-cover-generation_b200/csrc/gemm_tcgen05.cu
--- a/stable-diffusion-for-book-cover-generation_b200/csrc/gemm_tcgen05.cu
+++ b/stable-diffusion-for-book-cover-generation_b200/csrc/gemm_tcgen05.cu
@@ -1,3 +1,4 @@
+#include <algorithm>
 #include <atomic>
 #include <cstring>
 #include <mutex>
@@ -20,6 +21,7 @@
 constexpr int kNumThreads = 192;
 constexpr int kMaxStages = 8;
 constexpr int kABytes = BLOCK_M * BLOCK_K * 2;
+constexpr int kMaxLnTiles = 16;
 
 
 struct KParams {
@@ -58,6 +60,22 @@
     int persist;
     int psplit;
     float* gn_part;
+    int norm_kind;
+    bf16* norm_out;
+    int ld_norm;
+    const float* gamma;
+    const float* beta;
+    float eps;
+    int silu;
+    int cpg;
+    int hw;
+    int gn_ppi;
+    int gn_fold;
+    int n_tiles;
+    float2* ln_part;
+    int* norm_cnt;
+    int dep_mtiles;
+    uint32_t norm_smem;
 };
 
 __device__ __forceinline__ void cluster_sync_all() {
@@ -78,6 +96,25 @@
 
 __device__ __forceinline__ void red_add_v4(float* dst, float a, float b, float c, float d) {
     asm volatile("red.global.add.v4.f32 [%0], {%1, %2, %3, %4};" ::"l"(dst), "f"(a), "f"(b), "f"(c), "f"(d) : "memory");
+}
+
+__device__ __forceinline__ void grid_arrive_wait(int* cnt_in, int expected, const char* what, int unit) {
+    atomicAdd(cnt_in, 1);
+    int seen;
+    const long long t0 = clock64();
+    do {
+        asm volatile("ld.acquire.gpu.global.s32 %0, [%1];" : "=r"(seen) : "l"(cnt_in) : "memory");
+        if (clock64() - t0 > 4000000000LL) { printf("b200sd: %s arrival wait timed out (unit %d)\n", what, unit); __trap(); }
+    } while (seen < expected);
+    __threadfence();
+}
+__device__ __forceinline__ void grid_depart(int* cnt_in, int* cnt_out, int expected) {
+    __threadfence();
+    if (atomicAdd(cnt_out, 1) == expected - 1) {
+        *cnt_out = 0;
+        *cnt_in = 0;
+        __threadfence();
+    }
 }
 
 struct EpiCtx {
@@ -90,7 +127,7 @@
     asm volatile("ld.shared.v4.f32 {%0, %1, %2, %3}, [%4];" : "=f"(v[0]), "=f"(v[1]), "=f"(v[2]), "=f"(v[3]) : "r"(addr));
     asm volatile("ld.shared.v4.f32 {%0, %1, %2, %3}, [%4];" : "=f"(v[4]), "=f"(v[5]), "=f"(v[6]), "=f"(v[7]) : "r"(addr + 16));
 }
-template <int OUT, int RES, bool SPLIT, bool GEGLU, bool STATS = false>
+template <int OUT, int RES, bool SPLIT, bool GEGLU, bool STATS = false, bool KEEP = false>
 __device__ __forceinline__ void epilogue_rows(const KParams& p, const EpiCtx& e, int row0, const float (&b)[8], const float (&bg)[8],
                                               float* cs = nullptr, float* cq = nullptr) {
     constexpr int U = 4;
@@ -149,6 +186,11 @@
 #pragma unroll
                     for (int i = 0; i < 8; ++i) { cs[i] += o[i]; cq[i] = fmaf(o[i], o[i], cq[i]); }
                 }
+                if constexpr (KEEP) {
+                    const uint32_t addr = e.stage_u32 + (uint32_t)(rl * e.pitch_f + e.cb) * 4u;
+                    asm volatile("st.shared.v4.f32 [%0], {%1, %2, %3, %4};" ::"r"(addr), "f"(o[0]), "f"(o[1]), "f"(o[2]), "f"(o[3]) : "memory");
+                    asm volatile("st.shared.v4.f32 [%0], {%1, %2, %3, %4};" ::"r"(addr + 16), "f"(o[4]), "f"(o[5]), "f"(o[6]), "f"(o[7]) : "memory");
+                }
                 if constexpr (OUT == 2) {
                     float* dst = static_cast<float*>(p.out) + (size_t)grow * p.ldc + e.col_out;
                     red_add_v4(dst, o[0], o[1], o[2], o[3]);
@@ -157,6 +199,139 @@
                 else st8<B200SD_BF16>(p.out, (size_t)grow * p.ldc + e.col_out, o);
             }
         }
+    }
+}
+
+template <bool SPLIT, bool STATS>
+__device__ __forceinline__ void epilogue_rows_keep(const KParams& p, const EpiCtx& e, int row0, const float (&b)[8], float* cs, float* cq) {
+    if (p.residual) epilogue_rows<1, 2, SPLIT, false, STATS, true>(p, e, row0, b, b, cs, cq);
+    else epilogue_rows<1, 0, SPLIT, false, STATS, true>(p, e, row0, b, b, cs, cq);
+}
+
+__device__ __forceinline__ void norm_epilogue(const KParams& p, float* stage, int pitch_f, int m0, int n0, int row_begin, int valid) {
+    const int tid = threadIdx.x;
+    const int bn = p.block_n;
+    const bool ln = p.norm_kind == B200SD_NORM_LAYER;
+    float* scr = reinterpret_cast<float*>(reinterpret_cast<uint8_t*>(stage) + p.norm_smem);
+    __syncthreads();
+    if (ln && tid < valid) {
+        const float4* row = reinterpret_cast<const float4*>(stage + (size_t)(row_begin + tid) * pitch_f);
+        float s = 0.f;
+        for (int c = 0; c < bn / 4; ++c) { const float4 v = row[c]; s += (v.x + v.y) + (v.z + v.w); }
+        const float mean = s / (float)bn;
+        float q = 0.f;
+        for (int c = 0; c < bn / 4; ++c) {
+            const float4 v = row[c];
+            const float a = v.x - mean, b = v.y - mean, d = v.z - mean, e = v.w - mean;
+            q += (a * a + b * b) + (d * d + e * e);
+        }
+        p.ln_part[(size_t)(m0 + row_begin + tid) * p.n_tiles + blockIdx.y] = make_float2(mean, q);
+    }
+    const int unit = blockIdx.x / p.dep_mtiles;
+    const int expected = p.dep_mtiles * gridDim.y * gridDim.z;
+    int* cnt_in = p.norm_cnt + unit;
+    __syncthreads();
+    if (tid == 0) {
+        __threadfence();
+        grid_arrive_wait(cnt_in, expected, "norm epilogue", unit);
+    }
+    __syncthreads();
+    const int depart_tid = kNumThreads - 1;
+    if (tid == depart_tid) grid_depart(cnt_in, p.norm_cnt + gridDim.x / p.dep_mtiles + unit, expected);
+    float2* s_mr = reinterpret_cast<float2*>(scr);
+    const int img_lo = (m0 + row_begin) / p.hw;
+    float2* s_ab = nullptr;
+    if (ln) {
+        if (tid < valid) {
+            const float2* pr = p.ln_part + (size_t)(m0 + row_begin + tid) * p.n_tiles;
+            float2 part[kMaxLnTiles];
+#pragma unroll
+            for (int t = 0; t < kMaxLnTiles; ++t)
+                if (t < p.n_tiles) part[t] = __ldcg(pr + t);
+            float n = 0.f, mean = 0.f, m2 = 0.f;
+#pragma unroll
+            for (int t = 0; t < kMaxLnTiles; ++t) {
+                if (t >= p.n_tiles) break;
+                const float2 v = part[t];
+                const float nab = n + (float)bn;
+                const float d = v.x - mean;
+                mean += d * ((float)bn / nab);
+                m2 += v.y + d * d * (n * (float)bn / nab);
+                n = nab;
+            }
+            s_mr[tid] = make_float2(mean, rsqrtf(m2 / (float)p.N + p.eps));
+        }
+    } else if (valid > 0) {
+        const int nimg = (m0 + row_begin + valid - 1) / p.hw - img_lo + 1;
+        const int nq = p.gn_fold, c4n = bn / 4, gpt = bn / p.cpg;
+        float* s_red = scr;
+        float* s_tot = s_red + 2 * nq * 2 * bn;
+        s_ab = reinterpret_cast<float2*>(s_tot + 2 * 2 * bn);
+        float2* s_gmr = s_ab + 2 * bn;
+        for (int it = tid; it < nimg * nq * 2 * c4n; it += kNumThreads) {
+            const int c4 = it % c4n, rest = it / c4n, which = rest & 1, q = (rest >> 1) % nq, il = (rest >> 1) / nq;
+            const float* src = p.gn_part + ((size_t)(img_lo + il) * p.gn_ppi * 2 + which) * p.N + n0 + c4 * 4;
+            float a0 = 0.f, a1 = 0.f, a2 = 0.f, a3 = 0.f;
+#pragma unroll 8
+            for (int k = q; k < p.gn_ppi; k += nq) {
+                const float4 v = __ldcg(reinterpret_cast<const float4*>(src + (size_t)k * 2 * p.N));
+                a0 += v.x; a1 += v.y; a2 += v.z; a3 += v.w;
+            }
+            *reinterpret_cast<float4*>(s_red + ((il * nq + q) * 2 + which) * bn + c4 * 4) = make_float4(a0, a1, a2, a3);
+        }
+        __syncthreads();
+        for (int t = tid; t < nimg * 2 * bn; t += kNumThreads) {
+            const int il = t / (2 * bn), v = t % (2 * bn), which = v / bn, c = v % bn;
+            float a = 0.f;
+            for (int q = 0; q < nq; ++q) a += s_red[((il * nq + q) * 2 + which) * bn + c];
+            s_tot[t] = a;
+        }
+        __syncthreads();
+        for (int t = tid; t < nimg * gpt; t += kNumThreads) {
+            const int il = t / gpt, g = t % gpt;
+            float s0 = 0.f, s1 = 0.f;
+            for (int j = 0; j < p.cpg; ++j) { s0 += s_tot[(il * 2) * bn + g * p.cpg + j]; s1 += s_tot[(il * 2 + 1) * bn + g * p.cpg + j]; }
+            const double cnt = (double)p.hw * p.cpg;
+            const double mean = (double)s0 / cnt;
+            double var = (double)s1 / cnt - mean * mean;
+            if (var < 0.0) var = 0.0;
+            s_gmr[t] = make_float2((float)mean, (float)(1.0 / sqrt(var + (double)p.eps)));
+        }
+        __syncthreads();
+        for (int t = tid; t < nimg * bn; t += kNumThreads) {
+            const int il = t / bn, c = t % bn;
+            const float2 mr = s_gmr[il * gpt + c / p.cpg];
+            const float a = mr.y * __ldg(p.gamma + n0 + c);
+            s_ab[t] = make_float2(a, __ldg(p.beta + n0 + c) - mr.x * a);
+        }
+    }
+    __syncthreads();
+    const int groups = bn / 8, R = kNumThreads / groups;
+    if (tid >= R * groups) return;
+    const int cb = (tid % groups) * 8, r0 = tid / groups;
+    float g[8], bb[8];
+    if (ln) {
+#pragma unroll
+        for (int i = 0; i < 8; ++i) { g[i] = __ldg(p.gamma + n0 + cb + i); bb[i] = __ldg(p.beta + n0 + cb + i); }
+    }
+    const uint32_t stage_u32 = ptx::smem_u32(stage);
+    for (int r = r0; r < valid; r += R) {
+        const int grow = m0 + row_begin + r;
+        float v[8], y[8];
+        lds8(stage_u32 + (uint32_t)((row_begin + r) * pitch_f + cb) * 4u, v);
+        if (ln) {
+            const float2 mr = s_mr[r];
+#pragma unroll
+            for (int i = 0; i < 8; ++i) y[i] = (v[i] - mr.x) * mr.y * g[i] + bb[i];
+        } else {
+            const float2* ab = s_ab + (grow / p.hw - img_lo) * bn + cb;
+#pragma unroll
+            for (int i = 0; i < 8; ++i) {
+                y[i] = v[i] * ab[i].x + ab[i].y;
+                if (p.silu) y[i] = silu_f(y[i]);
+            }
+        }
+        st8<B200SD_BF16>(p.norm_out, (size_t)grow * p.ld_norm + n0 + cb, y);
     }
 }
 
@@ -388,7 +563,13 @@
                 const int row0 = row_begin + r0;
                 const int ok = p.atomic_out ? 2 : (p.out_f32 ? 1 : 0);
                 const int rk = p.residual ? (p.res_f32 ? 2 : 1) : 0;
-                if (geglu) epilogue_rows<0, 0, false, true>(p, e, row0, b, bg);
+                if (p.norm_kind != 0) {
+                    if constexpr (OP == 0 && !PAIR) {
+                        if (p.split_k > 1) { if (p.gn_part) epilogue_rows_keep<true, true>(p, e, row0, b, cs, cq); else epilogue_rows_keep<true, false>(p, e, row0, b, cs, cq); }
+                        else if (p.gn_part) epilogue_rows_keep<false, true>(p, e, row0, b, cs, cq);
+                        else epilogue_rows_keep<false, false>(p, e, row0, b, cs, cq);
+                    }
+                } else if (geglu) epilogue_rows<0, 0, false, true>(p, e, row0, b, bg);
                 else if (p.split_k > 1) {
                     if (ok == 1 && p.gn_part) { if (rk == 2) epilogue_rows<1, 2, true, false, true>(p, e, row0, b, bg, cs, cq); else epilogue_rows<1, 0, true, false, true>(p, e, row0, b, bg, cs, cq); }
                     else if (ok == 1) { if (rk == 2) epilogue_rows<1, 2, true, false>(p, e, row0, b, bg); else if (rk == 1) epilogue_rows<1, 1, true, false>(p, e, row0, b, bg); else epilogue_rows<1, 0, true, false>(p, e, row0, b, bg); }
@@ -401,7 +582,7 @@
         }
         if (p.gn_part != nullptr) {
             if (p.split_k > 1) cluster_sync_all(); else __syncthreads();
-            float* s_gn = reinterpret_cast<float*>(stage);
+            float* s_gn = stage + BLOCK_M * pitch_f;
 #pragma unroll
             for (int i = 0; i < 8; ++i) { s_gn[tid * 16 + i] = cs[i]; s_gn[tid * 16 + 8 + i] = cq[i]; }
             __syncthreads();
@@ -412,6 +593,9 @@
                 for (int r = 0; r < R; ++r) a += s_gn[(r * groups + c8) * 16 + k];
                 if (col < col_valid) dst[(size_t)(k >> 3) * p.N + n0 + col] = a;
             }
+        }
+        if constexpr (OP == 0 && !PAIR) {
+            if (p.norm_kind != 0) norm_epilogue(p, stage, pitch_f, m0, n0, row_begin, valid);
         }
     }
     if (p.split_k > 1 && p.gn_part == nullptr) cluster_sync_all();
@@ -705,16 +889,7 @@
     const int te = ew * 32 + lane;
     int* cnt_in = p.cnt + tile;
     int* cnt_out = p.cnt + p.num_tiles + tile;
-    if (te == 0) {
-        atomicAdd(cnt_in, 1);
-        int seen;
-        long long t0 = clock64();
-        do {
-            asm volatile("ld.acquire.gpu.global.s32 %0, [%1];" : "=r"(seen) : "l"(cnt_in) : "memory");
-            if (clock64() - t0 > 4000000000LL) { printf("b200sd: split-K arrival wait timed out (unit %d)\n", unit); __trap(); }
-        } while (seen < p.split);
-        __threadfence();
-    }
+    if (te == 0) grid_arrive_wait(cnt_in, p.split, "split-K", unit);
     ptx::named_bar_sync(1, kEpiWarps * 32);
     const int rpc = BLOCK_M / p.split;
     const int groups = p.block_n >> 2;
@@ -777,14 +952,7 @@
         }
     }
     ptx::named_bar_sync(1, kEpiWarps * 32);
-    if (te == 0) {
-        __threadfence();
-        if (atomicAdd(cnt_out, 1) == p.split - 1) {
-            *cnt_out = 0;
-            *cnt_in = 0;
-            __threadfence();
-        }
-    }
+    if (te == 0) grid_depart(cnt_in, cnt_out, p.split);
 }
 
 __global__ void __launch_bounds__(kPersistThreads, 1) gemm_persist_kernel(const __grid_constant__ PParams p) {
@@ -1119,27 +1287,34 @@
     return B200SD_OK;
 }
 
-int launch_gemm(KParams& p, int m_tiles, int n_tiles, int grid_z, bool cluster, b200sd_stream_t stream) {
+int gemm_stages(KParams& p, long total_ctas, size_t* smem_bytes) {
     const int sms = b200sd_num_sms();
     const int bn = p.block_n;
-    if (p.pair) m_tiles = (m_tiles + 1) & ~1;
     const int stage_bytes = kABytes + ((bn * BLOCK_K * 2) >> (p.pair ? 1 : 0));
-    const long total_ctas = (long)m_tiles * n_tiles * grid_z;
     int stages;
     if (total_ctas <= sms || bn > 160) stages = (200 * 1024) / stage_bytes;
     else stages = (108 * 1024) / stage_bytes;
     if (stages > kMaxStages) stages = kMaxStages;
     if (stages > p.kb_per_split && total_ctas <= sms) stages = p.kb_per_split;
-    const int min_stages = ceil_div(BLOCK_M * (bn + 4) * (int)sizeof(float), stage_bytes);
+    size_t scratch = p.gn_part ? (size_t)kNumThreads * 16 * sizeof(float) : 0;
+    if (p.norm_kind == B200SD_NORM_LAYER) scratch = std::max(scratch, (size_t)BLOCK_M * sizeof(float2));
+    if (p.norm_kind == B200SD_NORM_GROUP) scratch = std::max(scratch, (size_t)(4 * p.gn_fold + 12) * bn * sizeof(float));
+    p.norm_smem = (uint32_t)(BLOCK_M * (bn + 4) * sizeof(float));
+    const int min_stages = ceil_div(p.norm_smem + (int)scratch, stage_bytes);
     if (stages < min_stages) stages = min_stages;
     if (stages < 2) stages = 2;
     p.stages = stages;
-    B200SD_REQUIRE((size_t)stages * stage_bytes >= (size_t)BLOCK_M * (bn + 4) * sizeof(float), "gemm: smem ring smaller than the epilogue staging tile");
-    const size_t smem_bytes = (size_t)stages * stage_bytes + 1024  + 256  + 3072 ;
-    B200SD_REQUIRE(smem_bytes <= 227 * 1024, "gemm: smem budget exceeded (%zu B)", smem_bytes);
-
+    *smem_bytes = (size_t)stages * stage_bytes + 1024  + 256  + 3072 ;
+    B200SD_REQUIRE(*smem_bytes <= 227 * 1024, "gemm: smem budget exceeded (%zu B)", *smem_bytes);
+    return B200SD_OK;
+}
+
+int launch_gemm(KParams& p, int m_tiles, int n_tiles, int grid_z, bool cluster, b200sd_stream_t stream) {
+    if (p.pair) m_tiles = (m_tiles + 1) & ~1;
+    size_t smem_bytes = 0;
     {
-        const int rc = configure_gemm_kernels();
+        int rc = gemm_stages(p, (long)m_tiles * n_tiles * grid_z, &smem_bytes);
+        if (!rc) rc = configure_gemm_kernels();
         if (rc) return rc;
     }
     cudaLaunchConfig_t cfg = {};
@@ -1147,14 +1322,19 @@
     cfg.blockDim = dim3(kNumThreads);
     cfg.dynamicSmemBytes = smem_bytes;
     cfg.stream = static_cast<cudaStream_t>(stream);
-    cudaLaunchAttribute attr[1];
+    cudaLaunchAttribute attr[2];
+    cfg.attrs = attr;
     if ((cluster && grid_z > 1) || p.pair) {
-        attr[0].id = cudaLaunchAttributeClusterDimension;
-        attr[0].val.clusterDim.x = p.pair ? 2 : 1;
-        attr[0].val.clusterDim.y = 1;
-        attr[0].val.clusterDim.z = p.pair ? 1 : grid_z;
-        cfg.attrs = attr;
-        cfg.numAttrs = 1;
+        attr[cfg.numAttrs].id = cudaLaunchAttributeClusterDimension;
+        attr[cfg.numAttrs].val.clusterDim.x = p.pair ? 2 : 1;
+        attr[cfg.numAttrs].val.clusterDim.y = 1;
+        attr[cfg.numAttrs].val.clusterDim.z = p.pair ? 1 : grid_z;
+        ++cfg.numAttrs;
+    }
+    if (p.norm_kind != 0) {
+        attr[cfg.numAttrs].id = cudaLaunchAttributeCooperative;
+        attr[cfg.numAttrs].val.cooperative = 1;
+        ++cfg.numAttrs;
     }
     B200SD_CUDA(cudaLaunchKernelEx(&cfg, gemm_entry(p.pair, p.b_mode), p));
     g_b200sd_launches.fetch_add(1, std::memory_order_relaxed);
@@ -1313,6 +1493,64 @@
     return B200SD_OK;
 }
 
+static bool norm_plan(const b200sd_gemm_args* a, KParams& p, int m_tiles, int n_tiles, size_t* ws_bytes) {
+    if (a->norm_kind != B200SD_NORM_LAYER && a->norm_kind != B200SD_NORM_GROUP) return false;
+    if (p.persist || p.pair || a->epilogue != B200SD_EPI_LINEAR || a->out_dtype != B200SD_F32 ||
+        (a->residual && a->residual_dtype != B200SD_F32))
+        return false;
+    const long ctas = (long)m_tiles * n_tiles * p.split_k;
+    if (ctas > b200sd_num_sms()) return false;
+    p.norm_kind = a->norm_kind;
+    p.ld_norm = a->ld_norm > 0 ? a->ld_norm : a->N;
+    p.eps = a->eps;
+    p.silu = a->silu;
+    size_t floats = 0;
+    if (p.norm_kind == B200SD_NORM_LAYER) {
+        if (n_tiles > kMaxLnTiles) return false;
+        p.dep_mtiles = 1;
+        p.n_tiles = n_tiles;
+        floats = (size_t)m_tiles * p.rows_valid * n_tiles * 2;
+    } else {
+        const int hw = a->rows_per_image;
+        if (!a->gn_part || hw <= 0 || a->groups <= 0 || a->N % a->groups != 0 || a->M % hw != 0) return false;
+        p.cpg = a->N / a->groups;
+        if (p.block_n % p.cpg != 0) return false;
+        int ppi = 0, total = 0;
+        if (b200sd_gemm_gn_layout(a, hw, &ppi, &total) != B200SD_OK || ppi <= 0) return false;
+        if (hw % p.rows_valid == 0) p.dep_mtiles = hw / p.rows_valid;
+        else if (p.rows_valid % hw == 0 && p.rows_valid / hw <= 2) p.dep_mtiles = 1;
+        else return false;
+        if (m_tiles % p.dep_mtiles != 0) return false;
+        int G, slabs, ppc, R, threads, nq;
+        if (!b200sd_gn_parts_shape(a->N, a->groups, a->M / hw, hw, &G, &slabs, &ppc, &R, &threads, &nq)) return false;
+        p.hw = hw;
+        p.gn_ppi = ppi;
+        p.gn_fold = nq;
+    }
+    size_t smem = 0;
+    if (gemm_stages(p, ctas, &smem) != B200SD_OK) return false;
+    const size_t counters = (((size_t)2 * (m_tiles / p.dep_mtiles) * sizeof(int)) + 255) & ~(size_t)255;
+    *ws_bytes = counters + floats * sizeof(float);
+    return true;
+}
+
+extern "C" int b200sd_gemm_norm_query(const b200sd_gemm_args* a, int* supported, size_t* ws_bytes) {
+    B200SD_REQUIRE(a && supported && ws_bytes, "gemm_norm_query: null argument");
+    KParams p;
+    memset(&p, 0, sizeof(p));
+    p.M = a->M;
+    p.N = a->N;
+    p.num_k_blocks = a->K / BLOCK_K;
+    p.conv = a->conv_taps == 9;
+    p.gn_part = a->gn_part;
+    int m_tiles = 0, n_tiles = 0;
+    const int rc = gemm_tiling(a, p, &m_tiles, &n_tiles);
+    if (rc) return rc;
+    *ws_bytes = 0;
+    *supported = norm_plan(a, p, m_tiles, n_tiles, ws_bytes) ? 1 : 0;
+    return B200SD_OK;
+}
+
 extern "C" int b200sd_gemm(const b200sd_gemm_args* a, b200sd_stream_t stream) {
     B200SD_REQUIRE(a != nullptr, "gemm: null args");
     B200SD_REQUIRE(a->a0 && a->w && a->out, "gemm: null operand pointer");
@@ -1368,6 +1606,23 @@
     B200SD_REQUIRE(!a->gn_part || (a->out_dtype == B200SD_F32 && a->epilogue == B200SD_EPI_LINEAR &&
                                    (!a->residual || a->residual_dtype == B200SD_F32)),
                    "gemm: gn_part needs fp32 output, the linear epilogue and no bf16 residual");
+    if (a->norm_kind != B200SD_NORM_NONE) {
+        B200SD_REQUIRE(a->norm_out && a->gamma && a->beta && a->norm_ws, "gemm: the norm epilogue needs norm_out, gamma, beta and norm_ws");
+        B200SD_REQUIRE((reinterpret_cast<uintptr_t>(a->norm_out) & 15) == 0 && a->ld_norm % 8 == 0 &&
+                           (reinterpret_cast<uintptr_t>(a->norm_ws) & 255) == 0,
+                       "gemm: norm_out must be 16-byte aligned with ld_norm %% 8 == 0, norm_ws 256-byte aligned");
+        size_t ws_bytes = 0;
+        if (!norm_plan(a, p, m_tiles, n_tiles, &ws_bytes)) {
+            b200sd_set_error("gemm: no norm epilogue for M=%d N=%d K=%d (see b200sd_gemm_norm_query)", a->M, a->N, a->K);
+            return B200SD_ERR_UNSUPPORTED;
+        }
+        p.norm_out = static_cast<bf16*>(a->norm_out);
+        p.gamma = a->gamma;
+        p.beta = a->beta;
+        p.norm_cnt = static_cast<int*>(a->norm_ws);
+        const size_t counters = (((size_t)2 * (m_tiles / p.dep_mtiles) * sizeof(int)) + 255) & ~(size_t)255;
+        p.ln_part = reinterpret_cast<float2*>(static_cast<char*>(a->norm_ws) + counters);
+    }
 
     if (!p.conv) {
         const uint64_t dimsA[2] = {(uint64_t)C0, (uint64_t)a->M};
diff --git a/stable-diffusion-for-book-cover-generation_b200/csrc/norm.cu b/stable-diffusion-for-book-cover-generation_b200/csrc/norm.cu
--- a/stable-diffusion-for-book-cover-generation_b200/csrc/norm.cu
+++ b/stable-diffusion-for-book-cover-generation_b200/csrc/norm.cu
@@ -583,6 +583,31 @@
     return b200sd_layernorm_split(x, gamma, beta, out, nullptr, rows, C, eps, in_dtype, stream);
 }
 
+bool b200sd_gn_parts_shape(int C, int groups, int batch, int hw, int* G_out, int* slabs_out, int* ppc_out, int* R_out,
+                           int* threads_out, int* fold_ways) {
+    if (groups <= 0 || C % groups != 0 || batch <= 0 || hw <= 0) return false;
+    const int cpg = C / groups;
+    int G = 1;
+    while ((G * cpg) % 8 != 0 && G < groups) G *= 2;
+    while (G * 2 <= groups && groups % (G * 2) == 0 && G * cpg < 32) G *= 2;
+    const int Cg = G * cpg;
+    if ((Cg % 8) != 0 || groups % G != 0 || Cg / 8 > 512) return false;
+    const int VC = Cg / 8, sets = groups / G;
+    int slabs = ceil_div(b200sd_num_sms() * 2, batch * sets);
+    if (slabs > hw / 32) slabs = hw / 32;
+    if (slabs < 1) slabs = 1;
+    const int ppc = ceil_div(hw, slabs);
+    slabs = ceil_div(hw, ppc);
+    int R = 256 / VC;
+    if (R < 1) R = 1;
+    if (R > ppc) R = ppc;
+    int threads = ((VC * R + 31) / 32) * 32;
+    if (threads < 64) threads = 64;
+    *G_out = G; *slabs_out = slabs; *ppc_out = ppc; *R_out = R; *threads_out = threads;
+    *fold_ways = std::max(1, threads / (2 * Cg));
+    return true;
+}
+
 extern "C" int b200sd_groupnorm_silu_parts(const void* x0, const void* x1, int C0, int C1, const float* part0, int ppi0, int ld0,
                                            const float* part1, int ppi1, int ld1, const float* gamma, const float* beta, void* out,
                                            void* raw_out, float* stats_out, int batch, int hw, int groups, float eps, int silu,
@@ -594,23 +619,9 @@
     B200SD_REQUIRE(batch > 0 && hw > 0 && groups > 0 && groups <= kMaxGroups && C % groups == 0, "groupnorm_parts: bad shape");
     B200SD_REQUIRE(C0 % 8 == 0 && C1 % 8 == 0, "groupnorm_parts: channel counts must be multiples of 8");
     B200SD_REQUIRE(in_dtype == B200SD_BF16 || in_dtype == B200SD_F32, "groupnorm_parts: bad input dtype");
-    const int cpg = C / groups;
-    int G = 1;
-    while ((G * cpg) % 8 != 0 && G < groups) G *= 2;
-    while (G * 2 <= groups && groups % (G * 2) == 0 && G * cpg < 32) G *= 2;
-    const int Cg = G * cpg;
-    if ((Cg % 8) != 0 || groups % G != 0 || Cg / 8 > 512) return B200SD_ERR_UNSUPPORTED;
-    const int VC = Cg / 8, sets = groups / G;
-    int slabs = ceil_div(b200sd_num_sms() * 2, batch * sets);
-    if (slabs > hw / 32) slabs = hw / 32;
-    if (slabs < 1) slabs = 1;
-    const int ppc = ceil_div(hw, slabs);
-    slabs = ceil_div(hw, ppc);
-    int R = 256 / VC;
-    if (R < 1) R = 1;
-    if (R > ppc) R = ppc;
-    int threads = ((VC * R + 31) / 32) * 32;
-    if (threads < 64) threads = 64;
+    int G, slabs, ppc, R, threads, nq;
+    if (!b200sd_gn_parts_shape(C, groups, batch, hw, &G, &slabs, &ppc, &R, &threads, &nq)) return B200SD_ERR_UNSUPPORTED;
+    const int Cg = G * (C / groups), sets = groups / G;
     const size_t smem = ((size_t)4 * Cg + (size_t)std::max(threads, 2 * Cg)) * sizeof(float);
     cudaStream_t s = static_cast<cudaStream_t>(stream);
     if (in_dtype == B200SD_F32)
diff --git a/stable-diffusion-for-book-cover-generation_b200/engine.py b/stable-diffusion-for-book-cover-generation_b200/engine.py
--- a/stable-diffusion-for-book-cover-generation_b200/engine.py
+++ b/stable-diffusion-for-book-cover-generation_b200/engine.py
@@ -7,8 +7,8 @@
 
 
 class Engine(Builder):
-    def __init__(self, model, N, H, W, S_ctx, device, io=None):
-        super().__init__(device)
+    def __init__(self, model, N, H, W, S_ctx, device, io=None, norm_epilogue=("layer", "group")):
+        super().__init__(device, norm_epilogue)
         self.model, self.N, self.H, self.W, self.S = model, N, H, W, S_ctx
         self._io = io
         cfg = model.config
@@ -113,7 +113,7 @@
             self.groupnorm(P, x, None, wa["gn_g"], wa["gn_b"], t, N, h * w, 1e-6, False)
             hs = pool.get(M, Cc, F32)
             self.gemm(P, t, wa["w_in"], hs, bias=wa["b_in"])
-            P.append(lambda: ops.layernorm(hs, wa["ln1_g"], wa["ln1_b"], t), "layernorm")
+            self.layernorm(P, hs, wa["ln1_g"], wa["ln1_b"], t)
             qkv = pool.get(M, 3 * Cc)
             self.gemm(P, t, wa["w_qkv"], qkv)
             P.append(lambda: ops.attention(qkv, qkv, qkv, t, N, self.heads, h * w, h * w, d, scale, ldq=3 * Cc,
@@ -121,7 +121,7 @@
                      "attention", 4.0 * N * self.heads * (h * w) * (h * w) * d, f"self-attn S{h * w} d{d}")
             pool.put(qkv)
             self.gemm(P, t, wa["w_o1"], hs, bias=wa["b_o1"], residual=hs)
-            P.append(lambda: ops.layernorm(hs, wa["ln2_g"], wa["ln2_b"], t), "layernorm")
+            self.layernorm(P, hs, wa["ln2_g"], wa["ln2_b"], t)
             q = pool.get(M, Cc)
             self.gemm(P, t, wa["w_q2"], q)
             P.append(lambda: ops.attention(q, kv, kv, t, N, self.heads, h * w, self.S, d, scale, ldq=Cc, ldk=2 * Cc,
@@ -129,7 +129,7 @@
                      "attention", 4.0 * N * self.heads * (h * w) * self.S * d, f"cross-attn S{h * w} d{d}")
             pool.put(q)
             self.gemm(P, t, wa["w_o2"], hs, bias=wa["b_o2"], residual=hs)
-            P.append(lambda: ops.layernorm(hs, wa["ln3_g"], wa["ln3_b"], t), "layernorm")
+            self.layernorm(P, hs, wa["ln3_g"], wa["ln3_b"], t)
             ff = pool.get(M, 4 * Cc)
             self.gemm(P, t, wa["w_ff1"], ff, bias=wa["b_ff1"], epilogue=ops.EPI_GEGLU, block_n=wa["ff_tile"])
             self.gemm(P, ff, wa["w_ff2"], t, bias=wa["b_ff2"], residual=hs)
diff --git a/stable-diffusion-for-book-cover-generation_b200/ops.py b/stable-diffusion-for-book-cover-generation_b200/ops.py
--- a/stable-diffusion-for-book-cover-generation_b200/ops.py
+++ b/stable-diffusion-for-book-cover-generation_b200/ops.py
@@ -8,6 +8,7 @@
 
 F32, BF16 = 0, 1
 EPI_LINEAR, EPI_GEGLU = 0, 1
+NORM_LAYER, NORM_GROUP = 1, 2
 
 
 def _up16(*ts):
@@ -261,6 +262,24 @@
     return GnParts(buf, ppi.value, args.N)
 
 
+def gemm_attach_norm(args, kind, norm_out, gamma, beta, eps, *, silu=False, groups=32, hw=0):
+    _chk(norm_out, gamma, beta)
+    saved = (args.norm_kind, args.norm_out, args.ld_norm, args.gamma, args.beta, args.eps, args.silu, args.groups, args.rows_per_image)
+    args.norm_kind, args.norm_out, args.ld_norm = kind, _p(norm_out), norm_out.shape[-1]
+    args.gamma, args.beta, args.eps, args.silu, args.groups = _p(gamma), _p(beta), float(eps), int(silu), groups
+    if kind == NORM_GROUP:
+        args.rows_per_image = hw
+    ok, ws_bytes = C.c_int(0), C.c_size_t(0)
+    check(lib().b200sd_gemm_norm_query(C.byref(args), C.byref(ok), C.byref(ws_bytes)), "gemm_norm_query")
+    if not ok.value:
+        (args.norm_kind, args.norm_out, args.ld_norm, args.gamma, args.beta, args.eps, args.silu, args.groups,
+         args.rows_per_image) = saved
+        return None
+    ws = torch.zeros(max(256, ws_bytes.value), dtype=torch.uint8, device=norm_out.device)
+    args.norm_ws = ws.data_ptr()
+    return ws
+
+
 def groupnorm_silu_parts(x0, x1, parts0, parts1, gamma, beta, out, batch, hw, groups=32, eps=1e-5, silu=True, raw_out=None,
                          stats_out=None):
     _chk(x0, x1, gamma, beta, out, raw_out, stats_out)
diff --git a/stable-diffusion-for-book-cover-generation_b200/plan.py b/stable-diffusion-for-book-cover-generation_b200/plan.py
--- a/stable-diffusion-for-book-cover-generation_b200/plan.py
+++ b/stable-diffusion-for-book-cover-generation_b200/plan.py
@@ -67,10 +67,12 @@
 
 class Builder:
 
-    def __init__(self, device):
+    def __init__(self, device, norm_epilogue=()):
         self.device = device
         self._keep = []
         self._gn_parts = {}
+        self._norm_epilogue = frozenset(norm_epilogue)
+        self._last_gemm = {}
 
     def gemm(self, plan, a0, w, out, *, rowbias_ptr=None, gn_hw=0, kind=None, name=None, **kw):
         args = ops.gemm(a0, w, out, launch=False, **kw)
@@ -86,6 +88,7 @@
         k = "conv3x3" if args.conv_taps == 9 else "gemm"
         plan.append(lambda a=args: ops.gemm_run(a), kind or k, 2.0 * args.M * args.N * args.K,
                     name or f"{k} M{args.M} N{args.N} K{args.K}")
+        self._last_gemm[id(plan)] = (len(plan) - 1, id(out), args)
 
     def dgrad(self, plan, dy, w, out, *, name=None, **kw):
         args = ops.gemm_dgrad(dy, w, out, launch=False, **kw)
@@ -104,6 +107,9 @@
     def groupnorm(self, plan, x, skip, g, b, out, batch, hw, eps, silu, *, groups=32, raw_out=None, stats_out=None):
         p0 = self._gn_parts.get(id(x))
         p1 = self._gn_parts.get(id(skip)) if skip is not None else None
+        if (p0 is not None and skip is None and raw_out is None and stats_out is None and
+                self._fuse_norm(plan, x, "group", out, g, b, eps, silu=silu, groups=groups, hw=hw)):
+            return
         Cc = x.shape[-1] + (skip.shape[-1] if skip is not None else 0)
         if p0 is not None and (skip is None or p1 is not None) and ops.gn_parts_supported(Cc, groups):
             self._keep.append((p0, p1))
@@ -112,6 +118,25 @@
         else:
             plan.append(lambda: ops.groupnorm_silu(x, skip, g, b, out, batch, hw, groups, eps, silu, raw_out=raw_out,
                                                    stats_out=stats_out), "groupnorm")
+
+    def layernorm(self, plan, x, g, b, out, eps=1e-5):
+        if not self._fuse_norm(plan, x, "layer", out, g, b, eps):
+            plan.append(lambda: ops.layernorm(x, g, b, out, eps), "layernorm")
+
+    def _fuse_norm(self, plan, x, which, out, g, b, eps, **kw):
+        last = self._last_gemm.get(id(plan))
+        if which not in self._norm_epilogue or last is None:
+            return False
+        i, out_id, args = last
+        if out_id != id(x) or any(m[0] != "tap" for m in plan.meta[i + 1:]):
+            return False
+        ws = ops.gemm_attach_norm(args, ops.NORM_LAYER if which == "layer" else ops.NORM_GROUP, out, g, b, eps, **kw)
+        if ws is None:
+            return False
+        self._keep.append((out, g, b, ws))
+        kind, flops, name = plan.meta[i]
+        plan.meta[i] = (kind, flops, f"{name} + {which}norm")
+        return True
 
 
 def profile_plan(plan, device, iters=5):
```

Result: slower. 184.3, median of 6 (-9.5%).
